# letitiabanana/PnP-OVSS

Measured on AMD Instinct MI355X. Metric: images/sec (336^2, drop_iter=4, blur+CRF), higher is better.
Workload: dtype bf16x3

## Files before the change

### include/pnp_hip.h

```cpp
#ifndef PNP_HIP_H
#define PNP_HIP_H

#include <stddef.h>
#include <stdint.h>

#ifdef __cplusplus
extern "C" {
#endif

typedef struct pnp_engine pnp_engine;

typedef struct pnp_config {
    int32_t img_size, patch, vit_dim, vit_depth, vit_heads, vit_mlp_ratio;
    float vit_ln_eps;
    int32_t txt_hidden, txt_layers, txt_heads, txt_inter;
    float txt_ln_eps;
    int32_t vocab, max_pos, enc_token_id;
    int32_t max_batch;
    int32_t max_text_len;
    int32_t stash_layer;
    int32_t compute_bf16;
    int32_t device;
} pnp_config;

int pnp_create(const pnp_config* cfg, pnp_engine** out);
int pnp_create_shared(const pnp_config* cfg, pnp_engine* donor, pnp_engine** out);
void pnp_destroy(pnp_engine* e);
const char* pnp_last_error(const pnp_engine* e);
size_t pnp_workspace_bytes(const pnp_config* cfg);
size_t pnp_allocated_bytes(const pnp_engine* e);

int pnp_load_weight(pnp_engine* e, const char* name, const float* data, const int64_t* shape, int32_t ndim,
                    int32_t on_device);
int pnp_finalize_weights(pnp_engine* e);

int pnp_vit_forward(pnp_engine* e, const float* d_images, const uint8_t* d_dropped, int32_t B, void* stream);
int pnp_cross_kv(pnp_engine* e, int32_t B, void* stream);
int pnp_text_forward_xattn(pnp_engine* e, const int64_t* d_ids, const int64_t* d_mask, int32_t ld, int32_t B,
                           int32_t L, float* d_logits, void* stream);
int pnp_xattn_grad(pnp_engine* e, int32_t B, int32_t L, void* stream);
int pnp_xattn_grad_layer(pnp_engine* e, int32_t B, int32_t L, int32_t layer, void* stream);
int pnp_gradcam_gather(pnp_engine* e, const int64_t* d_mask, int32_t ld, int32_t B, int32_t L, int32_t head,
                       float* d_out, void* stream);
int pnp_compute_gradcam(pnp_engine* e, const float* d_images, const uint8_t* d_dropped, const int64_t* d_ids,
                        const int64_t* d_mask, int32_t ld, int32_t B, int32_t L, int32_t head, float* d_out,
                        float* d_logits, void* stream);

int pnp_compute_gradcam_layer(pnp_engine* e, const float* d_images, const uint8_t* d_dropped, const int64_t* d_ids,
                              const int64_t* d_mask, int32_t ld, int32_t B, int32_t L, int32_t layer, int32_t head,
                              float* d_out, float* d_logits, void* stream);

int pnp_drop_step(pnp_engine* e, const float* d_gradcam, float* d_g0, float* d_agg, uint8_t* d_dropped,
                  int32_t* d_picks, int32_t iter, int32_t B, int32_t T, int32_t npick, int32_t max_picks,
                  void* stream);
int pnp_drop_loop(pnp_engine* e, const float* d_images, const int64_t* d_ids, const int64_t* d_mask, int32_t ld,
                  int32_t B, int32_t L, int32_t head, int32_t drop_iter, int32_t npick, float* d_g0, float* d_agg,
                  int32_t* d_picks, float* d_logits, void* stream);

int pnp_drop_loop_layer(pnp_engine* e, const float* d_images, const int64_t* d_ids, const int64_t* d_mask, int32_t ld,
                        int32_t B, int32_t L, int32_t layer, int32_t head, int32_t drop_iter, int32_t npick, float* d_g0,
                        float* d_agg, int32_t* d_picks, float* d_logits, void* stream);

typedef struct pnp_post_batch {
    int32_t B;
    const int32_t* H;
    const int32_t* W;
    const int32_t* n_classes;
    const int32_t* has_bg;
    const int32_t* img_cls_off;
    const int32_t* cls_off;
    const int32_t* tok_idx;
    const int32_t* cls_div;
    const int32_t* lut;
    int32_t lut_stride;
    const uint8_t* d_rgb;
    const float* d_gt;
    const double* blur_wts;
    const int32_t* blur_wt_off;
} pnp_post_batch;

int pnp_post_reserve(pnp_engine* e, int32_t max_batch, int64_t max_total_pixels, int32_t max_pixels_per_image,
                     int32_t max_channels, int32_t crf_chunk);
int pnp_post_prepare(pnp_engine* e, const pnp_post_batch* batch, int32_t want_crf, void* stream);
int pnp_merge_tokens(pnp_engine* e, const float* d_gradcam, int32_t T, void* stream);
int pnp_threshold_upsample(pnp_engine* e, float threshold, int32_t scale01, void* stream);
int pnp_blur_minmax(pnp_engine* e, void* stream);
int pnp_densecrf(pnp_engine* e, int32_t iters, float pos_w, float pos_xy, float bi_w, float bi_xy, float bi_rgb,
                 void* stream);
int pnp_remap_hist(pnp_engine* e, int32_t from_crf, uint8_t* d_labels, unsigned long long* d_hist, int32_t n_class,
                   void* stream);
int pnp_postprocess(pnp_engine* e, const float* d_gradcam, int32_t T, float threshold, int32_t scale01, int32_t mode,
                    uint8_t* d_labels, unsigned long long* d_hist, int32_t n_class, void* stream);

int pnp_postprocess_pair(pnp_engine* e, const float* d_gradcam_1drop, const float* d_gradcam_ndrop, int32_t T, float threshold,
                         int32_t scale01_mask, uint8_t* d_labels_1drop, unsigned long long* d_hist_1drop, uint8_t* d_labels_ndrop,
                         unsigned long long* d_hist_ndrop, int32_t n_class, void* stream);

typedef struct pnp_pre_image {
    int64_t src_off;
    int64_t tmp_off;
    int32_t H, W;
    int32_t kx_off, kx_size;
    int32_t ky_off, ky_size;
} pnp_pre_image;
int pnp_preprocess_images(const uint8_t* d_rgb, const pnp_pre_image* d_desc, int32_t B, int32_t S, int32_t max_H,
                          const int32_t* d_coef, uint8_t* d_tmp, const float* mean3, const float* std3, float* d_out,
                          void* stream);

typedef struct pnp_jpeg_image {
    int64_t data_off;
    int64_t coef_off[3];
    int64_t plane_off[3];
    int64_t rgb_off;
    int32_t data_len, H, W, ncomp, hmax, vmax, mcux, mcuy;
    int32_t h[3], v[3], tq[3], td[3], ta[3], bx[3], by[3];
    int32_t tab, pad[2];
} pnp_jpeg_image;
typedef struct pnp_jpeg_tables {
    uint8_t counts[4][16];
    uint8_t vals[4][256];
    int32_t quant[4][64];
} pnp_jpeg_tables;
typedef struct pnp_jpeg_segment {
    int64_t byte_off;
    int64_t clean_off;
    int32_t image, mcu0, nmcu;
    int32_t raw_len;
    int32_t clean_cap;
    int32_t sub_bits;
    int32_t pad[2];
} pnp_jpeg_segment;
int pnp_jpeg_decode(const uint8_t* d_data, const pnp_jpeg_image* d_images, const pnp_jpeg_tables* d_tables,
                    const pnp_jpeg_segment* d_segments, int32_t n_images, int32_t n_segments, uint8_t* d_clean, int32_t* d_seg_bits,
                    int16_t* d_coef, int64_t coef_elems, uint8_t* d_planes, uint8_t* d_rgb, int32_t max_blocks_per_image,
                    int32_t max_pixels_per_image, int32_t* d_err, void* stream);

int pnp_get_buffer(pnp_engine* e, const char* name, void** d_ptr, size_t* bytes);
int pnp_profile_enable(pnp_engine* e, int32_t on);
int pnp_profile_read(pnp_engine* e, int64_t* launches, double* flops, double* ms);
int pnp_profile_read_stage(pnp_engine* e, int32_t stage, int64_t* launches, double* work, double* ms);
int pnp_set_tuning(const char* key, int32_t value);
int pnp_streamk_status(pnp_engine* e, int64_t* launches, uint32_t* gave_up);
int pnp_op_gemm(int32_t bf16, const void* d_A, int32_t lda, const void* d_B, int32_t ldb, int32_t M, int32_t N, int32_t K,
                const float* d_bias, const float* d_resid, int32_t ldr, float* d_out_f32, int32_t ldo, int32_t gelu,
                void* stream);
int pnp_op_gemm_ex(int32_t bf16, const void* d_A, int32_t lda, const void* d_B, int32_t ldb, int32_t M, int32_t N, int32_t K,
                   const float* d_bias, const float* d_resid, int32_t ldr, float* d_out_f32, int32_t ldo, void* d_out_t,
                   int32_t ldo_t, int32_t mode, void* stream);
int pnp_op_gemm_tokcols(int32_t bf16, const void* d_A, int32_t lda, const void* d_B, int32_t ldb, int32_t M, int32_t N,
                        int32_t K, const float* d_bias_rows, void* d_out_t, int32_t ldo_t, int32_t col_div,
                        int32_t col_pad, void* stream);
int pnp_op_split(const float* d_in, void* d_hi, void* d_lo, int64_t n, void* stream);
int pnp_op_gemm_x3(const void* d_A_hi, const void* d_A_lo, int32_t lda, const void* d_B_hi, const void* d_B_lo, int32_t ldb,
                   int32_t M, int32_t N, int32_t K, const float* d_bias, int32_t bias_on_rows, const float* d_resid, int32_t ldr,
                   float* d_out_f32, int32_t ldo, void* d_out_hi, void* d_out_lo, int32_t ldo_t, int32_t gelu, int32_t col_div,
                   int32_t col_pad, void* stream);
int pnp_op_gemm_x3a(const float* d_A, int32_t lda, const void* d_B_hi, const void* d_B_lo, int32_t ldb, int32_t M, int32_t N,
                    int32_t K, const float* d_bias, const float* d_resid, int32_t ldr, float* d_out_f32, int32_t ldo, int32_t mode,
                    float* d_aux, int32_t ld_aux, void* stream);
int pnp_op_vit_attention(int32_t bf16, const void* d_qk, int32_t ld_qk, int32_t D, const void* d_vt, int32_t ld_vt,
                         int32_t n_pad, void* d_ctx, int32_t B, int32_t heads, int32_t N, float scale, void* stream);
int pnp_op_vit_attention_x3(const void* d_qkv_hi, const void* d_qkv_lo, int32_t ld_qkv, int32_t D, void* d_ctx_hi, void* d_ctx_lo,
                            int32_t B, int32_t heads, int32_t N, float scale, void* stream);
int pnp_op_layernorm(const float* d_x, const float* d_w, const float* d_b, float eps, int32_t rows, int32_t D,
                     float* d_y, void* stream);
int pnp_op_xattn(int32_t bf16, int32_t mode, const void* d_nat, int32_t ld_nat, const void* d_tr, int32_t ld_tr,
                 int32_t n_pad, const void* d_x, int32_t ldx, void* d_out, int32_t ldo, float* d_probs, int32_t n_stride,
                 int32_t B, int32_t L, int32_t N, int32_t heads, void* stream);
int pnp_dbg_gemm_stamps(uint64_t* host_out, int32_t max_blocks);
int pnp_op_cast(int32_t to_bf16, const float* d_in, void* d_out, int64_t n, void* stream);
int pnp_op_sort_pairs(uint64_t* d_keys_in, uint64_t* d_keys_out, uint32_t* d_vals_in, uint32_t* d_vals_out, int64_t n,
                      int32_t begin_bit, int32_t end_bit, const size_t* h_seg_off, int32_t n_seg, void* stream);
int pnp_op_scan_i32(const int32_t* d_in, int32_t* d_out, int64_t n, int32_t inclusive, void* stream);

#ifdef __cplusplus
}
#endif
#endif
```

### pnp-ovss_amd/csrc/engine.hip

```cpp
#include <hip/hip_runtime.h>

#include <cmath>
#include <cstdarg>
#include <cstring>
#include <map>
#include <memory>
#include <string>
#include <vector>

#include "../../include/pnp_hip.h"
#include "common.h"
#include "kernels.h"

using namespace pnp;

namespace {

struct Buf {
    void* p = nullptr;
    size_t bytes = 0;
};

struct TextLayerW {
    void *qkv_w = nullptr, *so_w = nullptr, *cq_w = nullptr, *co_w = nullptr, *i_w = nullptr, *o_w = nullptr;
    float *qkv_b = nullptr, *so_b = nullptr, *sln_w = nullptr, *sln_b = nullptr, *cq_b = nullptr, *co_b = nullptr,
          *cln_w = nullptr, *cln_b = nullptr, *i_b = nullptr, *o_b = nullptr, *oln_w = nullptr, *oln_b = nullptr;
    void *o_wT = nullptr, *i_wT = nullptr, *co_wT = nullptr, *cq_wT = nullptr, *so_wT = nullptr, *qkv_wT = nullptr;
};

struct TextLayerA {
    void* qkv = nullptr;
    float* Ps = nullptr;
    float *a_hat = nullptr, *a_rstd = nullptr, *a_out = nullptr;
    void* a_outT = nullptr;
    void* qc = nullptr;
    float* Pc = nullptr;
    float *c_hat = nullptr, *c_rstd = nullptr, *c_out = nullptr;
    void* c_outT = nullptr;
    float* u = nullptr;
    float *o_hat = nullptr, *o_rstd = nullptr, *h_out = nullptr;
    void* h_outT = nullptr;
};

struct VitLayerW {
    float *n1w, *n1b, *n2w, *n2b, *qkv_b, *proj_b, *fc1_b, *fc2_b;
    void *qkv_w, *proj_w, *fc1_w, *fc2_w;
};

struct WeightStore {
    int device = 0;
    std::vector<void*> allocs;
    size_t bytes = 0;
    ~WeightStore() {
        (void)hipSetDevice(device);
        for (void* p : allocs) (void)hipFree(p);
    }
};

}

struct pnp_engine {
    pnp_config c{};
    std::shared_ptr<WeightStore> wstore;
    bool to_store = false;
    bool shares_weights = false;
    int bf = 0;
    int x3 = 0;
    size_t esz = 4;
    int P = 0, PP = 0, N = 0, Npad = 0, D = 0, H = 0, I = 0, TL = 0, nh = 0, Nst = 0, SL = 0;
    char err[512] = {0};
    std::vector<void*> allocs;
    size_t alloc_bytes = 0;
    std::map<std::string, Buf> named;
    std::map<std::string, bool> loaded;
    bool finalized = false;

    float *cls = nullptr, *pos = nullptr, *patch_b = nullptr, *vnorm_w = nullptr, *vnorm_b = nullptr;
    void* patch_w = nullptr;
    std::vector<VitLayerW> vit;
    float *word = nullptr, *tpos = nullptr, *eln_w = nullptr, *eln_b = nullptr, *itm_w = nullptr, *itm_b = nullptr;
    std::vector<TextLayerW> txt;
    void *ck_w = nullptr, *cv_w = nullptr;
    float *ck_b = nullptr, *cv_b = nullptr;
    std::vector<Buf> staging;

    int ldq = 0;
    float* x0 = nullptr;
    struct { const float* images = nullptr; const int64_t* ids = nullptr; const int64_t* mask = nullptr; int B = 0, L = 0, ld = 0;
             bool vit = false, text = false; } reuse;
    void *patches = nullptr, *xn = nullptr, *qk = nullptr, *vt = nullptr, *ctx = nullptr, *h1 = nullptr, *embT = nullptr;
    float *x = nullptr, *emb32 = nullptr;
    void *Knat = nullptr, *Vnat = nullptr, *Kt = nullptr, *Vt = nullptr;
    std::vector<TextLayerA> ta;
    float *temb = nullptr, *h0 = nullptr, *tmp = nullptr;
    void *h0T = nullptr, *ctx_s = nullptr, *ctx_c = nullptr, *g = nullptr;
    float *dh = nullptr, *d_pre = nullptr, *dc = nullptr, *d_cpre = nullptr, *da = nullptr, *d_apre = nullptr,
          *dctx_s = nullptr, *dS = nullptr, *dPc = nullptr;
    void *d_preT = nullptr, *dg = nullptr, *d_cpreT = nullptr, *dctxc = nullptr, *dqc = nullptr, *d_apreT = nullptr,
         *dqkv = nullptr;
    int grad_layer = -1;
    float* G = nullptr;
    uint8_t* dropped = nullptr;
    float* logits_scratch = nullptr;

    struct Post {
        bool reserved = false, prepared = false, has_crf = false;
        int groups_cap = 1;
        int maxB = 0, maxK = 0, max_pix_img = 0, chunk = 0;
        int64_t max_total_pix = 0;
        int B = 0, Cmax = 0, Kmax = 0, maxHW = 0;
        int64_t total_pix = 0;
        std::vector<PostDesc> desc, desc_pair;
        PostDesc* d_desc = nullptr;
        PostDesc* d_desc_pair = nullptr;
        int32_t *d_img_cls_off = nullptr, *d_cls_off = nullptr, *d_tok_idx = nullptr, *d_cls_div = nullptr, *d_lut = nullptr;
        int lut_stride = 0;
        size_t* d_label_off = nullptr;
        double* d_wts = nullptr;
        int32_t* d_wt_off = nullptr;
        float *merged = nullptr, *thr = nullptr, *maps = nullptr, *maps2 = nullptr, *maps3 = nullptr, *stats = nullptr;
        float *unary = nullptr, *Q = nullptr, *va = nullptr, *vb = nullptr, *vga = nullptr, *vgb = nullptr, *norm[2] = {nullptr, nullptr};
        int Kpmax = 0, Kpmax_pair = 0, maxH = 0, maxW = 0, max_radius = 0, maxKp = 0;
        size_t valg_cap = 0;
        std::vector<int> gauss_sig;
        const uint8_t* d_rgb = nullptr;
        const float* d_gt = nullptr;
        CrfLattice lat[2]{};
        uint64_t *keys_a = nullptr, *keys_b = nullptr;
        uint32_t* vals_a = nullptr;
        int *n1k = nullptr, *n2k = nullptr;
        int *head = nullptr, *incl = nullptr, *range_err = nullptr;
        int range_err_host = 0;
        int lat_points[2] = {0, 0};
        std::vector<size_t> h_label_off;
        std::vector<int32_t> h_wt_off;
        std::vector<double> h_wts;
        void* sort_tmp = nullptr;
        size_t sort_tmp_bytes = 0;
        size_t cap[2] = {0, 0};
        size_t val_cap = 0;
        int lut_cap = 0, cls_cap = 0, tok_cap = 0, wts_cap = 0;
        bool maps_in_2 = false;
    } post;

    GemmProfile* gemm_prof = nullptr;
    StreamKWs sk_ws;
    struct StageProfile {
        bool on = false;
        std::vector<hipEvent_t> ev0, ev1;
        int used = 0;
        long long launches = 0;
        double work = 0;
        double lattice = 0;
    } crf_prof;
};

namespace {

int fail(pnp_engine* e, int code, const char* fmt, ...) {
// ... 6 lines not shown

#define HIPCHK(e, call)                                                                      \
    do {                                                                                     \
        hipError_t _s = (call);                                                              \
        if (_s != hipSuccess) return fail(e, PNP_ERR_HIP, "%s: %s", #call, hipGetErrorString(_s)); \
    } while (0)
#define KCHK(e, call)                                                         \
    do {                                                                      \
        int _r = (call);                                                      \
        if (_r != PNP_OK) return fail(e, _r, "%s failed (%d): %s", #call, _r, hipGetErrorString(hipGetLastError())); \
    } while (0)

template <typename T>
int dalloc(pnp_engine* e, T** out, size_t count, bool zero = false) {
    void* p = nullptr;
    const size_t bytes = (count * sizeof(T) + 255) / 256 * 256;
    if (hipMalloc(&p, bytes ? bytes : 256) != hipSuccess) return fail(e, PNP_ERR_NOMEM, "hipMalloc(%zu) failed", bytes);
    if (zero && hipMemset(p, 0, bytes ? bytes : 256) != hipSuccess) return fail(e, PNP_ERR_HIP, "hipMemset failed");
    if (e->to_store && e->wstore) {
        e->wstore->allocs.push_back(p);
        e->wstore->bytes += bytes;
    } else {
        e->allocs.push_back(p);
    }
    e->alloc_bytes += bytes;
    *out = reinterpret_cast<T*>(p);
    return PNP_OK;
}
int dalloc_t(pnp_engine* e, void** out, size_t count, bool zero = false) {
    char* p = nullptr;
    int r = dalloc<char>(e, &p, count * e->esz, zero);
    *out = p;
    return r;
}

bool ends_with(const std::string& s, const char* suf) {
    const size_t n = strlen(suf);
    return s.size() >= n && s.compare(s.size() - n, n, suf) == 0;
}

__global__ void transpose_cast_kernel_f32(const float* __restrict__ in, float* __restrict__ out, int rows, int cols) {
    __shared__ float t[32][33];
    const int bx = blockIdx.x * 32, by = blockIdx.y * 32;
    for (int i = threadIdx.y; i < 32; i += 8) {
        const int r = by + i, c = bx + threadIdx.x;
        t[i][threadIdx.x] = (r < rows && c < cols) ? in[(size_t)r * cols + c] : 0.f;
    }
    __syncthreads();
    for (int i = threadIdx.y; i < 32; i += 8) {
        const int c = bx + i, r = by + threadIdx.x;
        if (r < rows && c < cols) out[(size_t)c * rows + r] = t[threadIdx.x][i];
    }
}

__global__ void feat_to_tok_kernel(const float* __restrict__ src, int ld_src, int n_pad, float* __restrict__ dst, int R, int N) {
    __shared__ float t[32][33];
    const int b = blockIdx.z, r0 = blockIdx.x * 32, t0 = blockIdx.y * 32;
    for (int i = threadIdx.y; i < 32; i += 8) {
        const int r = r0 + i, tok = t0 + threadIdx.x;
        t[i][threadIdx.x] = (r < R && tok < N) ? src[(size_t)r * ld_src + (size_t)b * n_pad + tok] : 0.f;
    }
    __syncthreads();
    for (int i = threadIdx.y; i < 32; i += 8) {
        const int tok = t0 + i, r = r0 + threadIdx.x;
        if (r < R && tok < N) dst[((size_t)b * N + tok) * R + r] = t[threadIdx.x][i];
    }
}
__global__ void tok_to_feat_kernel(const float* __restrict__ src, int ld_src, float* __restrict__ dst, int ld_dst, int n_pad, int R, int N) {
    __shared__ float t[32][33];
    const int b = blockIdx.z, r0 = blockIdx.x * 32, t0 = blockIdx.y * 32;
    for (int i = threadIdx.y; i < 32; i += 8) {
        const int tok = t0 + i, r = r0 + threadIdx.x;
        t[i][threadIdx.x] = (r < R && tok < N) ? src[((size_t)b * N + tok) * ld_src + r] : 0.f;
    }
    __syncthreads();
    for (int i = threadIdx.y; i < 32; i += 8) {
        const int r = r0 + i, tok = t0 + threadIdx.x;
        if (r < R && tok < N) dst[(size_t)r * ld_dst + (size_t)b * n_pad + tok] = t[threadIdx.x][i];
    }
}

__global__ void embed_reuse_kernel(const float* __restrict__ x0, const uint8_t* __restrict__ dropped, const float* __restrict__ bias,
                                   const float* __restrict__ pos, float* __restrict__ x, int rows, int N, int D4) {
    const size_t total = (size_t)rows * D4;
    for (size_t i = (size_t)blockIdx.x * blockDim.x + threadIdx.x; i < total; i += (size_t)gridDim.x * blockDim.x) {
        const int m = (int)(i / D4), c = (int)(i - (size_t)m * D4);
        const int b = m / N, t = m - b * N;
        f32x4 v;
        if (t > 0 && dropped[(size_t)b * (N - 1) + (t - 1)]) {
            const f32x4 bv = reinterpret_cast<const f32x4*>(bias)[c];
            const f32x4 pv = reinterpret_cast<const f32x4*>(pos)[(size_t)t * D4 + c];
#pragma unroll
            for (int e = 0; e < 4; e++) v[e] = __fadd_rn(__fadd_rn(0.0f, bv[e]), pv[e]);
        } else {
            v = reinterpret_cast<const f32x4*>(x0)[i];
        }
        reinterpret_cast<f32x4*>(x)[i] = v;
    }
}

int make_weight(pnp_engine* e, const float* src32, int rows, int cols, bool transpose, void** out, bool split = false) {
    KCHK(e, dalloc_t(e, out, (size_t)rows * cols));
    const float* s = src32;
    float* tmp = nullptr;
    if (transpose) {
        HIPCHK(e, hipMalloc((void**)&tmp, (size_t)rows * cols * 4));
        hipLaunchKernelGGL(transpose_cast_kernel_f32, dim3((cols + 31) / 32, (rows + 31) / 32), dim3(32, 8), 0, 0, src32, tmp,
                           rows, cols);
        s = tmp;
    }
    int r = split ? split_f32(s, *out, (char*)*out + (size_t)rows * cols * 2, (size_t)rows * cols, 0)
                  : cast_f32(e->bf, s, *out, (size_t)rows * cols, 0);
    hipError_t st = hipDeviceSynchronize();
    if (tmp) (void)hipFree(tmp);
    if (r != PNP_OK || st != hipSuccess) return fail(e, PNP_ERR_HIP, "weight conversion failed");
    return PNP_OK;
}

GemmArgs G_(const void* A, int lda, const void* B, int ldb, int M, int N, int K) {
    GemmArgs g;
    g.A = A; g.lda = lda; g.B = B; g.ldb = ldb; g.M = M; g.N = N; g.K = K;
    return g;
}

int egemm(pnp_engine* e, int bf, GemmArgs g, hipStream_t s) {
    g.prof = e->gemm_prof;
    g.sk = e->sk_ws.part ? &e->sk_ws : nullptr;
    return gemm_nt(bf, g, s);
}

int tgemm(pnp_engine* e, GemmArgs g, hipStream_t s) {
    if (e->x3) {
        g.a_f32 = 1;
        g.B_lo = (const char*)g.B + (size_t)g.N * g.K * 2;
    }
    return egemm(e, e->bf, g, s);
}

const char* kVitNames[] = {"norm1.weight", "norm1.bias", "attn.qkv.weight", "attn.qkv.bias", "attn.proj.weight",
                           "attn.proj.bias", "norm2.weight", "norm2.bias", "mlp.fc1.weight", "mlp.fc1.bias",
                           "mlp.fc2.weight", "mlp.fc2.bias"};

}


extern "C" size_t pnp_workspace_bytes(const pnp_config* c) {
    if (!c) return 0;
    const size_t es = c->compute_bf16 == 1 ? 2 : 4;
    const size_t P = c->img_size / c->patch, N = P * P + 1, Npad = (N + 63) / 64 * 64, D = c->vit_dim, H = c->txt_hidden,
                 I = c->txt_inter, TL = c->txt_layers, B = c->max_batch, L = c->max_text_len;
    const size_t M = B * N, R = B * L;
    size_t w = (size_t)c->vit_depth * (12 * D * D) * es + TL * (4 * H * H + 2 * H * D + 2 * H * I) * es * 2 +
               ((size_t)c->vocab + c->max_pos) * H * 4;
    size_t a = M * (768 + D * 2 + 3 * D + 64 + D + 4 * D) * es + M * D * 12 + D * B * Npad * es + M * TL * H * es * 2 +
               2 * TL * H * B * Npad * es;
    size_t t = TL * (R * (3 * H + 2 * H) * es + R * (H * 8 + I) * 4 + B * (H / 64) * L * (L + Npad) * 4) + R * I * (4 + es) * 2 +
               R * H * 64;
    return w + a + t + (64u << 20);
}

extern "C" const char* pnp_last_error(const pnp_engine* e) { return e ? e->err : "null engine"; }

extern "C" void pnp_destroy(pnp_engine* e) {
    if (!e) return;
    (void)hipSetDevice(e->c.device);
    (void)hipDeviceSynchronize();
    for (void* p : e->allocs) (void)hipFree(p);
    for (auto& b : e->staging) if (b.p) (void)hipFree(b.p);
    if (e->gemm_prof) {
        for (int i = 0; i < e->gemm_prof->created; i++) {
            (void)hipEventDestroy(e->gemm_prof->ev0[i]);
            (void)hipEventDestroy(e->gemm_prof->ev1[i]);
        }
        delete e->gemm_prof;
    }
    for (hipEvent_t ev : e->crf_prof.ev0) (void)hipEventDestroy(ev);
    for (hipEvent_t ev : e->crf_prof.ev1) (void)hipEventDestroy(ev);
    streamk_ws_destroy(&e->sk_ws);
    delete e;
}

static int create_impl(const pnp_config* cfg, pnp_engine* donor, pnp_engine** out);
extern "C" int pnp_create(const pnp_config* cfg, pnp_engine** out) { return create_impl(cfg, nullptr, out); }
extern "C" int pnp_create_shared(const pnp_config* cfg, pnp_engine* donor, pnp_engine** out) {
    if (!donor) return PNP_ERR_ARG;
    return create_impl(cfg, donor, out);
}
static int create_impl(const pnp_config* cfg, pnp_engine* donor, pnp_engine** out) {
    if (!cfg || !out) return PNP_ERR_ARG;
    pnp_engine* e = new pnp_engine();
    *out = e;
    e->c = *cfg;
    if (donor) {
        const pnp_config& d = donor->c;
        if (!donor->finalized) return fail(e, PNP_ERR_STATE, "pnp_create_shared: the donor's weights are not finalized");
        if (d.device != cfg->device || d.compute_bf16 != cfg->compute_bf16 || d.img_size != cfg->img_size || d.patch != cfg->patch ||
            d.vit_dim != cfg->vit_dim || d.vit_depth != cfg->vit_depth || d.vit_heads != cfg->vit_heads ||
            d.vit_mlp_ratio != cfg->vit_mlp_ratio || d.txt_hidden != cfg->txt_hidden || d.txt_layers != cfg->txt_layers ||
            d.txt_heads != cfg->txt_heads || d.txt_inter != cfg->txt_inter || d.vocab != cfg->vocab || d.max_pos != cfg->max_pos ||
            d.vit_ln_eps != cfg->vit_ln_eps || d.txt_ln_eps != cfg->txt_ln_eps)
            return fail(e, PNP_ERR_ARG, "pnp_create_shared: device, compute mode and model geometry must equal the donor's");
        if (cfg->stash_layer < d.stash_layer)
            return fail(e, PNP_ERR_ARG, "pnp_create_shared: stash_layer %d below the donor's %d (its transposed backward weights "
                        "exist for layers >= %d only)", cfg->stash_layer, d.stash_layer, d.stash_layer);
    }
    const pnp_config& c = e->c;
    if (c.compute_bf16 < 0 || c.compute_bf16 > 2) return fail(e, PNP_ERR_ARG, "compute_bf16 must be 0 (fp32), 1 (bf16) or 2 (split-bf16)");
    e->bf = c.compute_bf16 == 1 ? 1 : 0;
    e->x3 = c.compute_bf16 == 2 ? 1 : 0;
    e->esz = e->bf ? 2 : 4;
    if (c.patch != 16) return fail(e, PNP_ERR_ARG, "patch must be 16");
    if (c.img_size % 16 || c.img_size <= 0) return fail(e, PNP_ERR_ARG, "img_size must be a positive multiple of 16");
    if (c.vit_dim != c.vit_heads * 64 || c.txt_hidden != c.txt_heads * 64)
        return fail(e, PNP_ERR_ARG, "head_dim must be 64 (vit_dim=%d heads=%d, txt_hidden=%d heads=%d)", c.vit_dim,
                    c.vit_heads, c.txt_hidden, c.txt_heads);
    if (c.vit_dim % 128 || c.txt_hidden % 128 || c.txt_inter % 128 || (c.vit_dim * c.vit_mlp_ratio) % 128)
        return fail(e, PNP_ERR_ARG, "widths must be multiples of 128");
    if (c.vit_dim > 1024 || c.txt_hidden > 1024) return fail(e, PNP_ERR_ARG, "LayerNorm width > 1024 unsupported");
    if (c.max_text_len < 5 || c.max_text_len > 512 || c.max_text_len > c.max_pos)
        return fail(e, PNP_ERR_ARG, "max_text_len must be in [5, min(512, max_pos = %d)]", c.max_pos);
    if (c.stash_layer < 0 || c.stash_layer >= c.txt_layers) return fail(e, PNP_ERR_ARG, "stash_layer out of range");
    if (c.max_batch <= 0) return fail(e, PNP_ERR_ARG, "max_batch must be positive");
    HIPCHK(e, hipSetDevice(c.device));
    e->P = c.img_size / 16;
    e->PP = e->P * e->P;
    e->N = e->PP + 1;
    e->Npad = (e->N + 63) / 64 * 64;
    e->Nst = e->Npad;
    e->D = c.vit_dim;
    e->H = c.txt_hidden;
    e->I = c.txt_inter;
    e->TL = c.txt_layers;
    e->nh = c.txt_heads;
    e->SL = c.stash_layer;
    if ((e->N + 15) / 16 > 160) return fail(e, PNP_ERR_ARG, "too many image tokens (%d) for the cross-attention kernel", e->N);
    const size_t B = c.max_batch, M = B * e->N, D = e->D, H = e->H, I = e->I, L = c.max_text_len, R = B * L, TL = e->TL;
    const size_t ldv = B * e->Npad;
    e->vit.resize(c.vit_depth);
    e->txt.resize(TL);
    e->ta.resize(TL);
    if (e->x3) {
        const int n_cu = device_cu_count();
        if (!n_cu || streamk_ws_create(&e->sk_ws, n_cu) != PNP_OK) return fail(e, PNP_ERR_HIP, "stream-K workspace allocation failed");
        e->alloc_bytes += (size_t)n_cu * 256 * 256 * 4;
    }
    KCHK(e, dalloc_t(e, &e->patches, B * e->PP * 768));
    KCHK(e, dalloc(e, &e->x, M * D));
    KCHK(e, dalloc(e, &e->x0, M * D));
    KCHK(e, dalloc_t(e, &e->xn, M * D));
    e->ldq = 3 * (int)D + 64;
    KCHK(e, dalloc_t(e, &e->qk, M * (size_t)e->ldq));
    KCHK(e, dalloc_t(e, &e->vt, D * ldv, true));
    KCHK(e, dalloc_t(e, &e->ctx, M * D));
    KCHK(e, dalloc_t(e, &e->h1, M * D * c.vit_mlp_ratio));
    KCHK(e, dalloc_t(e, &e->embT, M * D));
    KCHK(e, dalloc(e, &e->emb32, M * D));
    const int nVn = e->TL - e->SL, nKt = e->TL - e->SL - 1;
    KCHK(e, dalloc_t(e, &e->Knat, M * TL * H));
    KCHK(e, dalloc_t(e, &e->Vnat, M * (size_t)nVn * H));
    KCHK(e, dalloc_t(e, &e->Vt, TL * H * ldv, true));
    if (nKt > 0) KCHK(e, dalloc_t(e, &e->Kt, (size_t)nKt * H * ldv, true));
    KCHK(e, dalloc(e, &e->temb, R * H));
    KCHK(e, dalloc(e, &e->h0, R * H));
    KCHK(e, dalloc_t(e, &e->h0T, R * H));
    KCHK(e, dalloc(e, &e->tmp, R * H));
    KCHK(e, dalloc_t(e, &e->ctx_s, R * H));
    KCHK(e, dalloc_t(e, &e->ctx_c, R * H));
    KCHK(e, dalloc_t(e, &e->g, R * I));
    for (size_t i = 0; i < TL; i++) {
        TextLayerA& a = e->ta[i];
        KCHK(e, dalloc_t(e, &a.qkv, R * 3 * H));
        KCHK(e, dalloc(e, &a.a_hat, R * H));
        KCHK(e, dalloc(e, &a.a_rstd, R));
        KCHK(e, dalloc(e, &a.a_out, R * H));
        KCHK(e, dalloc_t(e, &a.a_outT, R * H));
        KCHK(e, dalloc_t(e, &a.qc, R * H));
        KCHK(e, dalloc(e, &a.c_hat, R * H));
        KCHK(e, dalloc(e, &a.c_rstd, R));
        KCHK(e, dalloc(e, &a.c_out, R * H));
        KCHK(e, dalloc_t(e, &a.c_outT, R * H));
        KCHK(e, dalloc(e, &a.u, R * I));
        KCHK(e, dalloc(e, &a.o_hat, R * H));
        KCHK(e, dalloc(e, &a.o_rstd, R));
        KCHK(e, dalloc(e, &a.h_out, R * H));
        KCHK(e, dalloc_t(e, &a.h_outT, R * H));
        if ((int)i >= e->SL) {
            KCHK(e, dalloc(e, &a.Ps, B * e->nh * L * L));
            KCHK(e, dalloc(e, &a.Pc, B * e->nh * L * (size_t)e->Nst, true));
        }
    }
    KCHK(e, dalloc(e, &e->dh, R * H));
    KCHK(e, dalloc(e, &e->d_pre, R * H));
    KCHK(e, dalloc_t(e, &e->d_preT, R * H));
    KCHK(e, dalloc_t(e, &e->dg, R * I));
    KCHK(e, dalloc(e, &e->dc, R * H));
    KCHK(e, dalloc(e, &e->d_cpre, R * H));
    KCHK(e, dalloc_t(e, &e->d_cpreT, R * H));
    KCHK(e, dalloc_t(e, &e->dctxc, R * H));
    KCHK(e, dalloc_t(e, &e->dqc, R * H));
    KCHK(e, dalloc(e, &e->da, R * H));
    KCHK(e, dalloc(e, &e->d_apre, R * H));
    KCHK(e, dalloc_t(e, &e->d_apreT, R * H));
    KCHK(e, dalloc(e, &e->dctx_s, R * H));
    KCHK(e, dalloc(e, &e->dS, B * e->nh * L * L));
    KCHK(e, dalloc(e, &e->dPc, B * e->nh * L * (size_t)e->Nst, true));
    KCHK(e, dalloc_t(e, &e->dqkv, R * 3 * H));
    KCHK(e, dalloc(e, &e->G, B * L * (size_t)e->PP));
    KCHK(e, dalloc(e, &e->dropped, B * (size_t)e->PP, true));
    KCHK(e, dalloc(e, &e->logits_scratch, B * 2));
    if (donor) {
        e->wstore = donor->wstore;
        e->shares_weights = true;
        e->cls = donor->cls; e->pos = donor->pos; e->patch_b = donor->patch_b; e->vnorm_w = donor->vnorm_w; e->vnorm_b = donor->vnorm_b;
        e->word = donor->word; e->tpos = donor->tpos; e->eln_w = donor->eln_w; e->eln_b = donor->eln_b;
        e->itm_w = donor->itm_w; e->itm_b = donor->itm_b; e->ck_b = donor->ck_b; e->cv_b = donor->cv_b;
        e->patch_w = donor->patch_w; e->ck_w = donor->ck_w; e->cv_w = donor->cv_w;
        e->vit = donor->vit;
        e->txt = donor->txt;
        e->finalized = true;
        return PNP_OK;
    }
    e->wstore = std::make_shared<WeightStore>();
    e->wstore->device = c.device;
    e->to_store = true;
    KCHK(e, dalloc(e, &e->cls, D));
    KCHK(e, dalloc(e, &e->pos, (size_t)e->N * D));
    KCHK(e, dalloc(e, &e->patch_b, D));
    KCHK(e, dalloc(e, &e->vnorm_w, D));
    KCHK(e, dalloc(e, &e->vnorm_b, D));
    KCHK(e, dalloc(e, &e->word, (size_t)c.vocab * H));
    KCHK(e, dalloc(e, &e->tpos, (size_t)c.max_pos * H));
    KCHK(e, dalloc(e, &e->eln_w, H));
    KCHK(e, dalloc(e, &e->eln_b, H));
    KCHK(e, dalloc(e, &e->itm_w, 2 * H));
    KCHK(e, dalloc(e, &e->itm_b, 2));
    KCHK(e, dalloc(e, &e->ck_b, TL * H));
    KCHK(e, dalloc(e, &e->cv_b, TL * H));
    for (auto& v : e->vit) {
        KCHK(e, dalloc(e, &v.n1w, D)); KCHK(e, dalloc(e, &v.n1b, D)); KCHK(e, dalloc(e, &v.n2w, D)); KCHK(e, dalloc(e, &v.n2b, D));
        KCHK(e, dalloc(e, &v.qkv_b, 3 * D)); KCHK(e, dalloc(e, &v.proj_b, D));
        KCHK(e, dalloc(e, &v.fc1_b, D * c.vit_mlp_ratio)); KCHK(e, dalloc(e, &v.fc2_b, D));
        v.qkv_w = v.proj_w = v.fc1_w = v.fc2_w = nullptr;
    }
    for (auto& t : e->txt) {
        KCHK(e, dalloc(e, &t.qkv_b, 3 * H)); KCHK(e, dalloc(e, &t.so_b, H)); KCHK(e, dalloc(e, &t.sln_w, H)); KCHK(e, dalloc(e, &t.sln_b, H));
        KCHK(e, dalloc(e, &t.cq_b, H)); KCHK(e, dalloc(e, &t.co_b, H)); KCHK(e, dalloc(e, &t.cln_w, H)); KCHK(e, dalloc(e, &t.cln_b, H));
        KCHK(e, dalloc(e, &t.i_b, I)); KCHK(e, dalloc(e, &t.o_b, H)); KCHK(e, dalloc(e, &t.oln_w, H)); KCHK(e, dalloc(e, &t.oln_b, H));
    }
    e->to_store = false;
    return PNP_OK;
}


namespace {

struct Slot {
    float* small = nullptr;
    size_t small_off = 0;
    bool gemm = false;
    int rows = 0, cols = 0;
};

bool resolve(pnp_engine* e, const std::string& n, Slot& s) {
    const int D = e->D, H = e->H, I = e->I;
    auto small = [&](float* p, int count, size_t off = 0) { s.small = p; s.small_off = off; s.rows = 1; s.cols = count; return true; };
    auto gemm = [&](int r, int c) { s.gemm = true; s.rows = r; s.cols = c; return true; };
    if (n == "visual_encoder.cls_token") return small(e->cls, D);
    if (n == "visual_encoder.pos_embed") return small(e->pos, e->N * D);
    if (n == "visual_encoder.patch_embed.proj.weight") return gemm(D, 768);
    if (n == "visual_encoder.patch_embed.proj.bias") return small(e->patch_b, D);
    if (n == "visual_encoder.norm.weight") return small(e->vnorm_w, D);
    if (n == "visual_encoder.norm.bias") return small(e->vnorm_b, D);
    if (n == "text_encoder.embeddings.word_embeddings.weight") return small(e->word, e->c.vocab * H);
    if (n == "text_encoder.embeddings.position_embeddings.weight") return small(e->tpos, e->c.max_pos * H);
    if (n == "text_encoder.embeddings.LayerNorm.weight") return small(e->eln_w, H);
    if (n == "text_encoder.embeddings.LayerNorm.bias") return small(e->eln_b, H);
    if (n == "itm_head.weight") return small(e->itm_w, 2 * H);
    if (n == "itm_head.bias") return small(e->itm_b, 2);
    int li = -1;
    char rest[128];
    if (sscanf(n.c_str(), "visual_encoder.blocks.%d.%127s", &li, rest) == 2 && li >= 0 && li < e->c.vit_depth) {
        VitLayerW& v = e->vit[li];
        const std::string r(rest);
        const int F = D * e->c.vit_mlp_ratio;
        if (r == "norm1.weight") return small(v.n1w, D);
        if (r == "norm1.bias") return small(v.n1b, D);
        if (r == "norm2.weight") return small(v.n2w, D);
        if (r == "norm2.bias") return small(v.n2b, D);
        if (r == "attn.qkv.bias") return small(v.qkv_b, 3 * D);
        if (r == "attn.proj.bias") return small(v.proj_b, D);
        if (r == "mlp.fc1.bias") return small(v.fc1_b, F);
        if (r == "mlp.fc2.bias") return small(v.fc2_b, D);
        if (r == "attn.qkv.weight") return gemm(3 * D, D);
        if (r == "attn.proj.weight") return gemm(D, D);
        if (r == "mlp.fc1.weight") return gemm(F, D);
        if (r == "mlp.fc2.weight") return gemm(D, F);
        return false;
    }
    if (sscanf(n.c_str(), "text_encoder.encoder.layer.%d.%127s", &li, rest) == 2 && li >= 0 && li < e->TL) {
        TextLayerW& t = e->txt[li];
        const std::string r(rest);
        if (r == "attention.self.query.bias") return small(t.qkv_b, H, 0);
        if (r == "attention.self.key.bias") return small(t.qkv_b, H, H);
        if (r == "attention.self.value.bias") return small(t.qkv_b, H, 2 * H);
        if (r == "attention.output.dense.bias") return small(t.so_b, H);
// ... 47 lines not shown
    }
    e->loaded[name] = true;
    return PNP_OK;
}

extern "C" int pnp_finalize_weights(pnp_engine* e) {
    if (!e) return PNP_ERR_ARG;
    if (e->finalized) return PNP_OK;
    HIPCHK(e, hipSetDevice(e->c.device));
    e->to_store = true;
    struct StoreOff { pnp_engine* e; ~StoreOff() { e->to_store = false; } } store_off{e};
    const int D = e->D, H = e->H, I = e->I, TL = e->TL;
    auto stage = [&](const std::string& n) -> const float* {
        auto it = e->named.find("stage:" + n);
        return it == e->named.end() ? nullptr : (const float*)it->second.p;
    };
#define NEED(ptr, nm)                                                         \
    const float* ptr = stage(nm);                                             \
    if (!ptr) return fail(e, PNP_ERR_STATE, "missing weight %s", std::string(nm).c_str());
    {
        const char* smalls[] = {"visual_encoder.cls_token", "visual_encoder.pos_embed", "visual_encoder.patch_embed.proj.bias",
                                "visual_encoder.norm.weight", "visual_encoder.norm.bias",
                                "text_encoder.embeddings.word_embeddings.weight", "text_encoder.embeddings.position_embeddings.weight",
                                "text_encoder.embeddings.LayerNorm.weight", "text_encoder.embeddings.LayerNorm.bias",
                                "itm_head.weight", "itm_head.bias"};
        for (const char* s : smalls)
            if (!e->loaded.count(s)) return fail(e, PNP_ERR_STATE, "missing weight %s", s);
    }
    {
        NEED(pw, "visual_encoder.patch_embed.proj.weight");
        KCHK(e, make_weight(e, pw, D, 768, false, &e->patch_w));
    }
    const int F = D * e->c.vit_mlp_ratio;
    for (int i = 0; i < e->c.vit_depth; i++) {
        const std::string b = "visual_encoder.blocks." + std::to_string(i) + ".";
        for (const char* k : kVitNames)
            if (!e->loaded.count(b + k)) return fail(e, PNP_ERR_STATE, "missing weight %s%s", b.c_str(), k);
        NEED(w0, b + "attn.qkv.weight");
        NEED(w1, b + "attn.proj.weight");
        NEED(w2, b + "mlp.fc1.weight");
        NEED(w3, b + "mlp.fc2.weight");
        KCHK(e, make_weight(e, w0, 3 * D, D, false, &e->vit[i].qkv_w, e->x3));
        KCHK(e, make_weight(e, w1, D, D, false, &e->vit[i].proj_w, e->x3));
        KCHK(e, make_weight(e, w2, F, D, false, &e->vit[i].fc1_w, e->x3));
        KCHK(e, make_weight(e, w3, D, F, false, &e->vit[i].fc2_w, e->x3));
    }
    KCHK(e, dalloc_t(e, &e->ck_w, (size_t)TL * H * D));
    KCHK(e, dalloc_t(e, &e->cv_w, (size_t)TL * H * D));
    for (int i = 0; i < TL; i++) {
        const std::string b = "text_encoder.encoder.layer." + std::to_string(i) + ".";
        TextLayerW& t = e->txt[i];
        const char* req[] = {"attention.self.query.bias", "attention.self.key.bias", "attention.self.value.bias",
                             "attention.output.dense.bias", "attention.output.LayerNorm.weight", "attention.output.LayerNorm.bias",
                             "crossattention.self.query.bias", "crossattention.self.key.bias", "crossattention.self.value.bias",
                             "crossattention.output.dense.bias", "crossattention.output.LayerNorm.weight",
                             "crossattention.output.LayerNorm.bias", "intermediate.dense.bias", "output.dense.bias",
                             "output.LayerNorm.weight", "output.LayerNorm.bias"};
        for (const char* k : req)
            if (!e->loaded.count(b + k)) return fail(e, PNP_ERR_STATE, "missing weight %s%s", b.c_str(), k);
        NEED(wq, b + "attention.self.query.weight");
        NEED(wk, b + "attention.self.key.weight");
        NEED(wv, b + "attention.self.value.weight");
        NEED(wso, b + "attention.output.dense.weight");
        NEED(wcq, b + "crossattention.self.query.weight");
        NEED(wck, b + "crossattention.self.key.weight");
        NEED(wcv, b + "crossattention.self.value.weight");
        NEED(wco, b + "crossattention.output.dense.weight");
        NEED(wi, b + "intermediate.dense.weight");
        NEED(wo, b + "output.dense.weight");
        float* fused = nullptr;
        HIPCHK(e, hipMalloc((void**)&fused, (size_t)3 * H * H * 4));
        HIPCHK(e, hipMemcpy(fused, wq, (size_t)H * H * 4, hipMemcpyDeviceToDevice));
        HIPCHK(e, hipMemcpy(fused + (size_t)H * H, wk, (size_t)H * H * 4, hipMemcpyDeviceToDevice));
        HIPCHK(e, hipMemcpy(fused + (size_t)2 * H * H, wv, (size_t)H * H * 4, hipMemcpyDeviceToDevice));
        int r = make_weight(e, fused, 3 * H, H, false, &t.qkv_w, e->x3);
        if (r == PNP_OK && i > e->SL) r = make_weight(e, fused, 3 * H, H, true, &t.qkv_wT, e->x3);
        (void)hipFree(fused);
        if (r != PNP_OK) return r;
        KCHK(e, make_weight(e, wso, H, H, false, &t.so_w, e->x3));
        KCHK(e, make_weight(e, wcq, H, H, false, &t.cq_w, e->x3));
        KCHK(e, make_weight(e, wco, H, H, false, &t.co_w, e->x3));
        KCHK(e, make_weight(e, wi, I, H, false, &t.i_w, e->x3));
        KCHK(e, make_weight(e, wo, H, I, false, &t.o_w, e->x3));
        if (e->x3) {
            const size_t half = (size_t)TL * H * D * 2, off = (size_t)i * H * D * 2;
            KCHK(e, split_f32(wck, (char*)e->ck_w + off, (char*)e->ck_w + half + off, (size_t)H * D, 0));
            KCHK(e, split_f32(wcv, (char*)e->cv_w + off, (char*)e->cv_w + half + off, (size_t)H * D, 0));
        } else {
            KCHK(e, cast_f32(e->bf, wck, (char*)e->ck_w + (size_t)i * H * D * e->esz, (size_t)H * D, 0));
            KCHK(e, cast_f32(e->bf, wcv, (char*)e->cv_w + (size_t)i * H * D * e->esz, (size_t)H * D, 0));
        }
        if (i >= e->SL) {
            KCHK(e, make_weight(e, wo, H, I, true, &t.o_wT, e->x3));
            KCHK(e, make_weight(e, wi, I, H, true, &t.i_wT, e->x3));
            KCHK(e, make_weight(e, wco, H, H, true, &t.co_wT, e->x3));
        }
        if (i > e->SL) {
            KCHK(e, make_weight(e, wcq, H, H, true, &t.cq_wT, e->x3));
            KCHK(e, make_weight(e, wso, H, H, true, &t.so_wT, e->x3));
        }
    }
#undef NEED
    HIPCHK(e, hipDeviceSynchronize());
    for (auto& b : e->staging) if (b.p) (void)hipFree(b.p);
    e->staging.clear();
    for (auto it = e->named.begin(); it != e->named.end();) {
        if (it->first.rfind("stage:", 0) == 0) it = e->named.erase(it);
        else ++it;
    }
    e->finalized = true;
    return PNP_OK;
}


static int vit_forward_impl(pnp_engine* e, const float* d_images, const uint8_t* d_dropped, int32_t B, void* stream, int embed);
extern "C" int pnp_vit_forward(pnp_engine* e, const float* d_images, const uint8_t* d_dropped, int32_t B, void* stream) {
    if (e) e->reuse.vit = false;
    return vit_forward_impl(e, d_images, d_dropped, B, stream, 0);
}
static int vit_forward_impl(pnp_engine* e, const float* d_images, const uint8_t* d_dropped, int32_t B, void* stream, int embed) {
    if (!e || !d_images) return PNP_ERR_ARG;
    if (!e->finalized) return fail(e, PNP_ERR_STATE, "weights not finalized");
    if (B <= 0 || B > e->c.max_batch) return fail(e, PNP_ERR_ARG, "batch %d out of range (max %d)", B, e->c.max_batch);
    hipStream_t s = (hipStream_t)stream;
    const int D = e->D, N = e->N, M = B * N, F = D * e->c.vit_mlp_ratio, bf = e->bf;
    const int ldv = e->c.max_batch * e->Npad;
    if (embed == 2 && !(e->reuse.vit && e->reuse.images == d_images && e->reuse.B == B)) embed = 0;
    if (embed == 2 && d_dropped) {
        hipLaunchKernelGGL(embed_reuse_kernel, dim3(2048), dim3(256), 0, s, (const float*)e->x0, d_dropped, (const float*)e->patch_b,
                           (const float*)e->pos, e->x, M, N, D / 4);
        if (hipGetLastError() != hipSuccess) return fail(e, PNP_ERR_HIP, "embed_reuse launch");
    } else {
    KCHK(e, patchify(bf, d_images, d_dropped, e->patches, B, e->c.img_size, e->P, s));
    KCHK(e, cls_rows(e->cls, e->pos, e->x, B, N, D, s));
    {
        GemmArgs g = G_(e->patches, 768, e->patch_w, 768, B * e->PP, D, 768);
        g.bias = e->patch_b; g.resid = e->pos; g.ldr = D; g.out_f32 = e->x; g.ldo = D; g.row_div = e->PP;
        KCHK(e, egemm(e, bf, g, s));
    }
    if (embed == 1) {
        HIPCHK(e, hipMemcpyAsync(e->x0, e->x, (size_t)M * D * sizeof(float), hipMemcpyDeviceToDevice, s));
        e->reuse.images = d_images;
        e->reuse.B = B;
        e->reuse.vit = true;
    }
    }
    const float scale = 1.0f / sqrtf(64.f);
    if (e->x3) {
        const size_t cap = (size_t)e->c.max_batch * N;
        void* const xn_lo = (char*)e->xn + cap * D * 2;
        void* const ctx_lo = (char*)e->ctx + cap * D * 2;
        void* const h1_lo = (char*)e->h1 + cap * F * 2;
        void* const qk_lo = (char*)e->qk + cap * e->ldq * 2;
        for (int l = 0; l < e->c.vit_depth; l++) {
            const VitLayerW& w = e->vit[l];
            const char* const qkv_lo = (const char*)w.qkv_w + (size_t)3 * D * D * 2;
            KCHK(e, layernorm(1, e->x, w.n1w, w.n1b, e->c.vit_ln_eps, M, D, nullptr, e->xn, nullptr, nullptr, s, xn_lo));
            {
                GemmArgs g = G_(e->xn, D, w.qkv_w, D, M, 3 * D, D);
                g.A_lo = xn_lo; g.B_lo = qkv_lo;
                g.bias = w.qkv_b; g.out_t = e->qk; g.out_lo = qk_lo; g.ldo_t = e->ldq;
                KCHK(e, egemm(e, 1, g, s));
            }
            KCHK(e, vit_attention_x3(e->qk, qk_lo, e->ldq, D, e->ctx, ctx_lo, B, e->c.vit_heads, N, scale, s));
            {
                GemmArgs g = G_(e->ctx, D, w.proj_w, D, M, D, D);
                g.A_lo = ctx_lo; g.B_lo = (const char*)w.proj_w + (size_t)D * D * 2;
                g.bias = w.proj_b; g.resid = e->x; g.ldr = D; g.out_f32 = e->x; g.ldo = D;
                KCHK(e, egemm(e, 1, g, s));
            }
            KCHK(e, layernorm(1, e->x, w.n2w, w.n2b, e->c.vit_ln_eps, M, D, nullptr, e->xn, nullptr, nullptr, s, xn_lo));
            {
                GemmArgs g = G_(e->xn, D, w.fc1_w, D, M, F, D);
                g.A_lo = xn_lo; g.B_lo = (const char*)w.fc1_w + (size_t)F * D * 2;
                g.bias = w.fc1_b; g.mode = GEMM_EPI_GELU; g.out_t = e->h1; g.out_lo = h1_lo; g.ldo_t = F;
                KCHK(e, egemm(e, 1, g, s));
            }
            {
                GemmArgs g = G_(e->h1, F, w.fc2_w, F, M, D, F);
                g.A_lo = h1_lo; g.B_lo = (const char*)w.fc2_w + (size_t)D * F * 2;
                g.bias = w.fc2_b; g.resid = e->x; g.ldr = D; g.out_f32 = e->x; g.ldo = D;
                KCHK(e, egemm(e, 1, g, s));
            }
        }
        KCHK(e, layernorm(1, e->x, e->vnorm_w, e->vnorm_b, e->c.vit_ln_eps, M, D, e->emb32, e->embT, nullptr, nullptr, s,
                          (char*)e->embT + cap * D * 2));
        return pnp_cross_kv(e, B, stream);
    }
    for (int l = 0; l < e->c.vit_depth; l++) {
        const VitLayerW& w = e->vit[l];
        KCHK(e, layernorm(bf, e->x, w.n1w, w.n1b, e->c.vit_ln_eps, M, D, nullptr, e->xn, nullptr, nullptr, s));
        if (bf) {
            GemmArgs g = G_(e->xn, D, w.qkv_w, D, M, 3 * D, D);
            g.bias = w.qkv_b; g.out_t = e->qk; g.ldo_t = e->ldq;
            KCHK(e, egemm(e, bf, g, s));
            KCHK(e, vit_attention(bf, e->qk, e->ldq, D, (const char*)e->qk + (size_t)2 * D * e->esz, e->ldq, e->Npad, e->ctx, B,
                                  e->c.vit_heads, N, scale, s));
        } else {
        {
            GemmArgs g = G_(e->xn, D, w.qkv_w, D, M, 2 * D, D);
            g.bias = w.qkv_b; g.out_t = e->qk; g.ldo_t = 2 * D;
            KCHK(e, egemm(e, bf, g, s));
        }
        {
            GemmArgs g = G_((const char*)w.qkv_w + (size_t)2 * D * D * e->esz, D, e->xn, D, D, M, D);
            g.bias = w.qkv_b + 2 * D; g.bias_on_rows = 1; g.out_t = e->vt; g.ldo_t = ldv; g.col_div = N; g.col_pad = e->Npad;
            KCHK(e, egemm(e, bf, g, s));
        }
        KCHK(e, vit_attention(bf, e->qk, 2 * D, D, e->vt, ldv, e->Npad, e->ctx, B, e->c.vit_heads, N, scale, s));
        }
        {
            GemmArgs g = G_(e->ctx, D, w.proj_w, D, M, D, D);
            g.bias = w.proj_b; g.resid = e->x; g.ldr = D; g.out_f32 = e->x; g.ldo = D;
            KCHK(e, egemm(e, bf, g, s));
        }
        KCHK(e, layernorm(bf, e->x, w.n2w, w.n2b, e->c.vit_ln_eps, M, D, nullptr, e->xn, nullptr, nullptr, s));
        {
            GemmArgs g = G_(e->xn, D, w.fc1_w, D, M, F, D);
            g.bias = w.fc1_b; g.mode = GEMM_EPI_GELU; g.out_t = e->h1; g.ldo_t = F;
            KCHK(e, egemm(e, bf, g, s));
        }
        {
            GemmArgs g = G_(e->h1, F, w.fc2_w, F, M, D, F);
            g.bias = w.fc2_b; g.resid = e->x; g.ldr = D; g.out_f32 = e->x; g.ldo = D;
            KCHK(e, egemm(e, bf, g, s));
        }
    }
    KCHK(e, layernorm(bf, e->x, e->vnorm_w, e->vnorm_b, e->c.vit_ln_eps, M, D, e->emb32, e->embT, nullptr, nullptr, s));
    return pnp_cross_kv(e, B, stream);
}

extern "C" int pnp_cross_kv(pnp_engine* e, int32_t B, void* stream) {
    if (!e) return PNP_ERR_ARG;
    if (!e->finalized) return fail(e, PNP_ERR_STATE, "weights not finalized");
    if (B <= 0 || B > e->c.max_batch) return fail(e, PNP_ERR_ARG, "batch %d out of range (max %d)", B, e->c.max_batch);
    hipStream_t s = (hipStream_t)stream;
    const int D = e->D, N = e->N, M = B * N, bf = e->bf;
    const int ldv = e->c.max_batch * e->Npad;
    const int H = e->H, TL = e->TL, SL = e->SL;
    if (e->x3) {
        const size_t cap = (size_t)e->c.max_batch * N, whalf = (size_t)TL * H * D * 2;
        const void* const emb_lo = (const char*)e->embT + cap * D * 2;
        const char *ck = (const char*)e->ck_w, *cv = (const char*)e->cv_w;
        {
            GemmArgs g = G_(e->embT, D, ck, D, M, TL * H, D);
            g.A_lo = emb_lo; g.B_lo = ck + whalf;
            g.bias = e->ck_b; g.out_f32 = (float*)e->Knat; g.ldo = TL * H;
            KCHK(e, egemm(e, 1, g, s));
        }
        {
            GemmArgs g = G_(cv, D, e->embT, D, TL * H, M, D);
            g.A_lo = cv + whalf; g.B_lo = emb_lo;
            g.bias = e->cv_b; g.bias_on_rows = 1; g.out_f32 = (float*)e->Vt; g.ldo = ldv; g.col_div = N; g.col_pad = e->Npad;
            KCHK(e, egemm(e, 1, g, s));
        }
        {
            const int nVn = TL - SL, R = nVn * H;
            hipLaunchKernelGGL(feat_to_tok_kernel, dim3((R + 31) / 32, (N + 31) / 32, B), dim3(32, 8), 0, s,
                               (const float*)e->Vt + (size_t)SL * H * ldv, ldv, e->Npad, (float*)e->Vnat, R, N);
            const int nKt = TL - SL - 1;
            if (nKt > 0)
                hipLaunchKernelGGL(tok_to_feat_kernel, dim3((nKt * H + 31) / 32, (N + 31) / 32, B), dim3(32, 8), 0, s,
                                   (const float*)e->Knat + (size_t)(SL + 1) * H, TL * H, (float*)e->Kt, ldv, e->Npad, nKt * H, N);
            if (hipGetLastError() != hipSuccess) return fail(e, PNP_ERR_HIP, "cross K / V layout kernels failed to launch");
        }
        return PNP_OK;
    }
    {
        GemmArgs g = G_(e->embT, D, e->ck_w, D, M, TL * H, D);
        g.bias = e->ck_b; g.out_t = e->Knat; g.ldo_t = TL * H;
        KCHK(e, egemm(e, bf, g, s));
    }
    {
        GemmArgs g = G_(e->cv_w, D, e->embT, D, TL * H, M, D);
        g.bias = e->cv_b; g.bias_on_rows = 1; g.out_t = e->Vt; g.ldo_t = ldv; g.col_div = N; g.col_pad = e->Npad;
        KCHK(e, egemm(e, bf, g, s));
    }
    {
        const int nVn = TL - SL;
        GemmArgs g = G_(e->embT, D, (const char*)e->cv_w + (size_t)SL * H * D * e->esz, D, M, nVn * H, D);
        g.bias = e->cv_b + (size_t)SL * H; g.out_t = e->Vnat; g.ldo_t = nVn * H;
        KCHK(e, egemm(e, bf, g, s));
    }
    if (TL - SL - 1 > 0) {
        const int nKt = TL - SL - 1;
        GemmArgs g = G_((const char*)e->ck_w + (size_t)(SL + 1) * H * D * e->esz, D, e->embT, D, nKt * H, M, D);
        g.bias = e->ck_b + (size_t)(SL + 1) * H; g.bias_on_rows = 1; g.out_t = e->Kt; g.ldo_t = ldv; g.col_div = N; g.col_pad = e->Npad;
        KCHK(e, egemm(e, bf, g, s));
    }
    return PNP_OK;
}

static int text_forward_impl(pnp_engine* e, const int64_t* d_ids, const int64_t* d_mask, int32_t ld, int32_t B, int32_t L,
                             float* d_logits, void* stream, bool reuse_prefix);
extern "C" int pnp_text_forward_xattn(pnp_engine* e, const int64_t* d_ids, const int64_t* d_mask, int32_t ld, int32_t B,
                                      int32_t L, float* d_logits, void* stream) {
    if (e) e->reuse.text = false;
    return text_forward_impl(e, d_ids, d_mask, ld, B, L, d_logits, stream, false);
}
static int text_forward_impl(pnp_engine* e, const int64_t* d_ids, const int64_t* d_mask, int32_t ld, int32_t B, int32_t L,
                             float* d_logits, void* stream, bool reuse_prefix) {
    if (!e || !d_ids || !d_mask) return PNP_ERR_ARG;
    if (!e->finalized) return fail(e, PNP_ERR_STATE, "weights not finalized");
    if (B <= 0 || B > e->c.max_batch || L < 5 || L > e->c.max_text_len || ld < L)
        return fail(e, PNP_ERR_ARG, "text batch %d x %d (ld %d) out of range (max %d x %d)", B, L, ld, e->c.max_batch, e->c.max_text_len);
    hipStream_t s = (hipStream_t)stream;
    const int H = e->H, I = e->I, TL = e->TL, R = B * L, bf = e->bf, N = e->N, D = e->D;
    const int ldv = e->c.max_batch * e->Npad;
    (void)D;
    if (reuse_prefix && !(e->reuse.text && e->reuse.ids == d_ids && e->reuse.mask == d_mask && e->reuse.B == B && e->reuse.L == L &&
                          e->reuse.ld == ld))
        reuse_prefix = false;
    if (!reuse_prefix) {
        KCHK(e, text_embed(d_ids, ld, e->word, e->tpos, e->temb, B, L, H, e->c.enc_token_id, e->c.vocab, s));
        KCHK(e, layernorm(bf, e->temb, e->eln_w, e->eln_b, e->c.txt_ln_eps, R, H, e->h0, e->h0T, nullptr, nullptr, s));
    }
    const float* h = e->h0;
// ... 579 lines not shown
    lout.lut = p.d_lut;
    lout.lut_stride = p.lut_stride;
    lout.label_off = p.d_label_off;
    int r = crf_iterate(e, p.d_desc_pair, p.Kpmax_pair, 10, 7.0f, 10.0f, s, lout);
    if (r) return r;
    for (int grp = 0; grp < 2; grp++) {
        uint8_t* lab = grp == 0 ? d_labels_1drop : d_labels_ndrop;
        unsigned long long* hist = grp == 0 ? d_hist_1drop : d_hist_ndrop;
        if (hist && p.d_gt) KCHK(e, confusion_hist(lab, p.d_gt, p.d_desc, p.d_label_off, hist, n_class, p.B, p.maxHW, s));
    }
    return PNP_OK;
}


extern "C" int pnp_get_buffer(pnp_engine* e, const char* name, void** d_ptr, size_t* bytes) {
    if (!e || !name || !d_ptr || !bytes) return PNP_ERR_ARG;
    const std::string n(name);
    const size_t B = e->c.max_batch, L = e->c.max_text_len;
    auto& p = e->post;
    auto set = [&](void* ptr, size_t b) { *d_ptr = ptr; *bytes = b; return PNP_OK; };
    if (n == "image_embeds") return set(e->emb32, B * e->N * (size_t)e->D * 4);
    if (n == "image_embeds_t") return set(e->embT, B * e->N * (size_t)e->D * e->esz);
    if (n == "x") return set(e->x, B * e->N * (size_t)e->D * 4);
    if (n == "P") return set(e->ta[e->grad_layer >= 0 ? e->grad_layer : e->SL].Pc, B * e->nh * L * (size_t)e->Nst * 4);
    if (n == "dP") return set(e->dPc, B * e->nh * L * (size_t)e->Nst * 4);
    if (n == "h_last") return set(e->ta[e->TL - 1].h_out, B * L * (size_t)e->H * 4);
    if (n == "dropped") return set(e->dropped, B * (size_t)e->PP);
    if (n == "P_last" && e->ta[e->TL - 1].Pc) return set(e->ta[e->TL - 1].Pc, B * e->nh * L * (size_t)e->Nst * 4);
    if (n == "Kt" && e->Kt) return set(e->Kt, (size_t)(e->TL - e->SL - 1) * e->H * B * e->Npad * e->esz);
    if (n == "Vt") return set(e->Vt, (size_t)e->TL * e->H * B * e->Npad * e->esz);
    if (n == "dq_xattn") return set(e->dqc, B * L * (size_t)e->H * e->esz);
    if (n == "dctx_xattn") return set(e->dctxc, B * L * (size_t)e->H * e->esz);
    if (p.reserved) {
        const size_t mk = (size_t)p.max_total_pix * p.maxK * 4;
        const size_t mq = (size_t)p.max_total_pix * p.maxKp * 4;
        if (n == "merged") return set(p.merged, (size_t)p.maxB * p.maxK * e->PP * 4);
        if (n == "maps") return set(p.maps_in_2 ? p.maps2 : p.maps, mk);
        if (n == "maps_pre_blur") return set(p.maps, mk);
        if (n == "unary") return set(p.unary, mq);
        if (n == "crf_q") return set(p.Q, mq);
        if (n == "crf_idbase_gauss") return set(p.lat[0].idbase, ((size_t)p.maxB + 1) * 4);
        if (n == "crf_idbase_bilateral") return set(p.lat[1].idbase, ((size_t)p.maxB + 1) * 4);
        if (n == "crf_norm_gauss") return set(p.norm[0], (size_t)p.max_total_pix * 4);
        if (n == "crf_norm_bilateral") return set(p.norm[1], (size_t)p.max_total_pix * 4);
        if (n == "crf_offset_gauss") return set(p.lat[0].offset, (size_t)p.max_total_pix * 3 * 4);
        if (n == "crf_offset_bilateral") return set(p.lat[1].offset, (size_t)p.max_total_pix * 6 * 4);
        if (n == "crf_nbr8_gauss") return set(p.lat[0].nbr8, (size_t)(p.lat[0].D1 / 2) * p.lat[0].cap * sizeof(CrfNbr8));
        if (n == "crf_nbr8_bilateral") return set(p.lat[1].nbr8, (size_t)(p.lat[1].D1 / 2) * p.lat[1].cap * sizeof(CrfNbr8));
    }
    return fail(e, PNP_ERR_ARG, "unknown buffer %s", name);
}

extern "C" size_t pnp_allocated_bytes(const pnp_engine* e) { return e ? e->alloc_bytes : 0; }

extern "C" int pnp_profile_enable(pnp_engine* e, int32_t on) {
    if (!e) return PNP_ERR_ARG;
    if (!e->gemm_prof) {
        if (!on) {
            e->crf_prof.on = false;
            return PNP_OK;
        }
        e->gemm_prof = new GemmProfile();
    }
    GemmProfile& pf = *e->gemm_prof;
    pf.on = on != 0;
    pf.period = on > 1 ? on : 1;
    pf.seq = 0;
    pf.used = 0;
    pf.launches = 0;
    pf.flops = 0;
    e->crf_prof.on = on != 0;
    e->crf_prof.used = 0;
    e->crf_prof.launches = 0;
    e->crf_prof.work = 0;
    e->crf_prof.lattice = 0;
    return PNP_OK;
}

extern "C" int pnp_profile_read_stage(pnp_engine* e, int32_t stage, int64_t* launches, double* work, double* ms) {
    if (!e || !launches || !work || !ms) return PNP_ERR_ARG;
    if (stage == 0) return pnp_profile_read(e, launches, work, ms);
    if (stage != 1 && stage != 2) return fail(e, PNP_ERR_ARG, "unknown profile stage %d", stage);
    auto& pf = e->crf_prof;
    double total = 0;
    for (int i = 0; i < pf.used; i++) {
        HIPCHK(e, hipEventSynchronize(pf.ev1[i]));
        float t = 0;
        HIPCHK(e, hipEventElapsedTime(&t, pf.ev0[i], pf.ev1[i]));
        total += t;
    }
    *launches = pf.launches;
    *work = stage == 1 ? pf.work : pf.lattice;
    *ms = total;
    return PNP_OK;
}

extern "C" int pnp_profile_read(pnp_engine* e, int64_t* launches, double* flops, double* ms) {
    if (!e || !launches || !flops || !ms) return PNP_ERR_ARG;
    if (!e->gemm_prof) {
        *launches = 0; *flops = 0; *ms = 0;
        return PNP_OK;
    }
    GemmProfile& pf = *e->gemm_prof;
    double total = 0;
    for (int i = 0; i < pf.used; i++) {
        HIPCHK(e, hipEventSynchronize(pf.ev1[i]));
        float t = 0;
        HIPCHK(e, hipEventElapsedTime(&t, pf.ev0[i], pf.ev1[i]));
        total += t;
    }
    *launches = pf.launches;
    *flops = pf.flops;
    *ms = total;
    return PNP_OK;
}

extern "C" int pnp_op_gemm(int32_t bf, const void* d_A, int32_t lda, const void* d_B, int32_t ldb, int32_t M, int32_t N,
                           int32_t K, const float* d_bias, const float* d_resid, int32_t ldr, float* d_out_f32, int32_t ldo,
                           int32_t gelu, void* stream) {
    GemmArgs g = G_(d_A, lda, d_B, ldb, M, N, K);
    g.bias = d_bias; g.resid = d_resid; g.ldr = ldr; g.out_f32 = d_out_f32; g.ldo = ldo;
    g.mode = gelu ? GEMM_EPI_GELU : GEMM_EPI_LINEAR;
    return gemm_nt(bf, g, (hipStream_t)stream);
}

extern "C" int pnp_op_gemm_ex(int32_t bf, const void* d_A, int32_t lda, const void* d_B, int32_t ldb, int32_t M, int32_t N,
                              int32_t K, const float* d_bias, const float* d_resid, int32_t ldr, float* d_out_f32, int32_t ldo,
                              void* d_out_t, int32_t ldo_t, int32_t mode, void* stream) {
    GemmArgs g = G_(d_A, lda, d_B, ldb, M, N, K);
    g.bias = d_bias; g.resid = d_resid; g.ldr = ldr; g.out_f32 = d_out_f32; g.ldo = ldo; g.out_t = d_out_t; g.ldo_t = ldo_t;
    g.mode = mode ? GEMM_EPI_GELU : GEMM_EPI_LINEAR;
    return gemm_nt(bf, g, (hipStream_t)stream);
}

extern "C" int pnp_op_split(const float* d_in, void* d_hi, void* d_lo, int64_t n, void* stream) {
    if (!d_in || !d_hi || !d_lo || n <= 0) return PNP_ERR_ARG;
    return split_f32(d_in, d_hi, d_lo, (size_t)n, (hipStream_t)stream);
}

extern "C" int pnp_op_gemm_x3(const void* d_A_hi, const void* d_A_lo, int32_t lda, const void* d_B_hi, const void* d_B_lo,
                              int32_t ldb, int32_t M, int32_t N, int32_t K, const float* d_bias, int32_t bias_on_rows,
                              const float* d_resid, int32_t ldr, float* d_out_f32, int32_t ldo, void* d_out_hi, void* d_out_lo,
                              int32_t ldo_t, int32_t gelu, int32_t col_div, int32_t col_pad, void* stream) {
    if (!d_A_hi || !d_A_lo || !d_B_hi || !d_B_lo) return PNP_ERR_ARG;
    GemmArgs g = G_(d_A_hi, lda, d_B_hi, ldb, M, N, K);
    g.A_lo = d_A_lo; g.B_lo = d_B_lo;
    g.bias = d_bias; g.bias_on_rows = bias_on_rows; g.resid = d_resid; g.ldr = ldr; g.out_f32 = d_out_f32; g.ldo = ldo;
    g.out_t = d_out_hi; g.out_lo = d_out_lo; g.ldo_t = ldo_t; g.col_div = col_div; g.col_pad = col_pad;
    g.mode = gelu ? GEMM_EPI_GELU : GEMM_EPI_LINEAR;
    g.sk = streamk_mode() ? streamk_ws_default() : nullptr;
    return gemm_nt(1, g, (hipStream_t)stream);
}

extern "C" int pnp_set_tuning(const char* key, int32_t value) {
    if (!key) return PNP_ERR_ARG;
    if (!strcmp(key, "streamk")) {
        if (value < 0 || value > 2) return PNP_ERR_ARG;
        set_streamk_mode(value);
        return PNP_OK;
    }
    return PNP_ERR_ARG;
}

extern "C" int pnp_streamk_status(pnp_engine* e, int64_t* launches, uint32_t* gave_up) {
    if (!launches || !gave_up) return PNP_ERR_ARG;
    StreamKWs* ws = e ? &e->sk_ws : streamk_ws_default();
    *launches = ws ? ws->launches : 0;
    *gave_up = 0;
    if (!ws || !ws->part) return PNP_OK;
    if (e) HIPCHK(e, hipSetDevice(e->c.device));
    if (hipDeviceSynchronize() != hipSuccess) return PNP_ERR_HIP;
    return streamk_ws_timeouts(ws, gave_up);
}

extern "C" int pnp_op_gemm_x3a(const float* d_A, int32_t lda, const void* d_B_hi, const void* d_B_lo, int32_t ldb, int32_t M,
                               int32_t N, int32_t K, const float* d_bias, const float* d_resid, int32_t ldr, float* d_out_f32,
                               int32_t ldo, int32_t mode, float* d_aux, int32_t ld_aux, void* stream) {
    if (!d_A || !d_B_hi || !d_B_lo || !d_out_f32 || mode < 0 || mode > 2) return PNP_ERR_ARG;
    GemmArgs g = G_(d_A, lda, d_B_hi, ldb, M, N, K);
    g.B_lo = d_B_lo; g.a_f32 = 1;
    g.bias = d_bias; g.resid = d_resid; g.ldr = ldr; g.out_f32 = d_out_f32; g.ldo = ldo;
    g.mode = mode; g.aux = d_aux; g.ld_aux = ld_aux;
    return gemm_nt(0, g, (hipStream_t)stream);
}

extern "C" int pnp_op_gemm_tokcols(int32_t bf, const void* d_A, int32_t lda, const void* d_B, int32_t ldb, int32_t M, int32_t N,
                                   int32_t K, const float* d_bias_rows, void* d_out_t, int32_t ldo_t, int32_t col_div,
                                   int32_t col_pad, void* stream) {
    if (!d_out_t || col_div < 0 || (col_div > 0 && col_pad < col_div)) return PNP_ERR_ARG;
    GemmArgs g = G_(d_A, lda, d_B, ldb, M, N, K);
    g.bias = d_bias_rows; g.bias_on_rows = 1; g.out_t = d_out_t; g.ldo_t = ldo_t; g.col_div = col_div; g.col_pad = col_pad;
    return gemm_nt(bf, g, (hipStream_t)stream);
}

extern "C" int pnp_op_vit_attention(int32_t bf, const void* d_qk, int32_t ld_qk, int32_t D, const void* d_vt, int32_t ld_vt,
                                    int32_t n_pad, void* d_ctx, int32_t B, int32_t heads, int32_t N, float scale, void* stream) {
    if (!d_qk || !d_vt || !d_ctx || B <= 0 || heads <= 0 || N <= 0) return PNP_ERR_ARG;
    return vit_attention(bf, d_qk, ld_qk, D, d_vt, ld_vt, n_pad, d_ctx, B, heads, N, scale, (hipStream_t)stream);
}

extern "C" int pnp_op_vit_attention_x3(const void* d_qkv_hi, const void* d_qkv_lo, int32_t ld_qkv, int32_t D, void* d_ctx_hi,
                                       void* d_ctx_lo, int32_t B, int32_t heads, int32_t N, float scale, void* stream) {
    if (B <= 0 || heads <= 0 || N <= 0 || ld_qkv < 3 * D) return PNP_ERR_ARG;
    return vit_attention_x3(d_qkv_hi, d_qkv_lo, ld_qkv, D, d_ctx_hi, d_ctx_lo, B, heads, N, scale, (hipStream_t)stream);
}

extern "C" int pnp_op_layernorm(const float* d_x, const float* d_w, const float* d_b, float eps, int32_t rows, int32_t D,
                                float* d_y, void* stream) {
    return layernorm(0, d_x, d_w, d_b, eps, rows, D, d_y, nullptr, nullptr, nullptr, (hipStream_t)stream);
}

extern "C" int pnp_op_xattn(int32_t bf16, int32_t mode, const void* d_nat, int32_t ld_nat, const void* d_tr, int32_t ld_tr,
                            int32_t n_pad, const void* d_x, int32_t ldx, void* d_out, int32_t ldo, float* d_probs,
                            int32_t n_stride, int32_t B, int32_t L, int32_t N, int32_t heads, void* stream) {
    if (!d_nat || !d_x || !d_probs || mode < 0 || mode > 2 || (mode != 2 && (!d_tr || !d_out))) return PNP_ERR_ARG;
    if (B <= 0 || L <= 0 || N <= 0 || heads <= 0) return PNP_ERR_ARG;
    return xattn(bf16, mode, d_nat, ld_nat, d_tr, ld_tr, n_pad, d_x, ldx, d_out, ldo, d_probs, n_stride, B, L, N, heads,
                 (hipStream_t)stream);
}

extern "C" int pnp_dbg_gemm_stamps(uint64_t* host_out, int32_t max_blocks) {
    return gemm_read_stamps((unsigned long long*)host_out, max_blocks);
}

extern "C" int pnp_preprocess_images(const uint8_t* d_rgb, const pnp_pre_image* d_desc, int32_t B, int32_t S, int32_t max_H,
                                     const int32_t* d_coef, uint8_t* d_tmp, const float* mean3, const float* std3,
                                     float* d_out, void* stream) {
    if (!d_rgb || !d_desc || !d_coef || !d_tmp || !mean3 || !std3 || !d_out) return PNP_ERR_ARG;
    static_assert(sizeof(pnp_pre_image) == 40, "pnp_pre_image layout is part of the ABI");
    return preprocess_images(d_rgb, d_desc, B, S, max_H, d_coef, d_tmp, mean3, std3, d_out, (hipStream_t)stream);
}

extern "C" int pnp_jpeg_decode(const uint8_t* d_data, const pnp_jpeg_image* d_images, const pnp_jpeg_tables* d_tables,
                               const pnp_jpeg_segment* d_segments, int32_t n_images, int32_t n_segments, uint8_t* d_clean,
                               int32_t* d_seg_bits, int16_t* d_coef, int64_t coef_elems, uint8_t* d_planes, uint8_t* d_rgb,
                               int32_t max_blocks_per_image, int32_t max_pixels_per_image, int32_t* d_err, void* stream) {
    if (!d_data || !d_images || !d_tables || !d_segments || !d_clean || !d_seg_bits || !d_coef || !d_planes || !d_rgb || !d_err ||
        coef_elems <= 0)
        return PNP_ERR_ARG;
    static_assert(sizeof(pnp_jpeg_image) == sizeof(JpegImage) && sizeof(pnp_jpeg_tables) == sizeof(JpegTables) &&
                      sizeof(pnp_jpeg_segment) == sizeof(JpegSegment), "JPEG descriptor layouts are part of the ABI");
    return jpeg_decode(d_data, reinterpret_cast<const JpegImage*>(d_images), reinterpret_cast<const JpegTables*>(d_tables),
                       reinterpret_cast<const JpegSegment*>(d_segments), n_images, n_segments, d_clean, d_seg_bits, d_coef,
                       (size_t)coef_elems, d_planes, d_rgb, max_blocks_per_image, max_pixels_per_image, d_err, (hipStream_t)stream);
}

extern "C" int pnp_op_sort_pairs(uint64_t* d_keys_in, uint64_t* d_keys_out, uint32_t* d_vals_in, uint32_t* d_vals_out, int64_t n,
                                 int32_t begin_bit, int32_t end_bit, const size_t* h_seg_off, int32_t n_seg, void* stream) {
    if (n < 0 || (n && (!d_keys_in || !d_keys_out || !d_vals_in || !d_vals_out))) return PNP_ERR_ARG;
    if (!n) return PNP_OK;
    const size_t tb = sort_temp_bytes((size_t)n);
    void* temp = nullptr;
    if (hipMalloc(&temp, tb) != hipSuccess) return PNP_ERR_NOMEM;
    int r = radix_sort_pairs(d_keys_in, d_keys_out, d_vals_in, d_vals_out, (size_t)n, begin_bit, end_bit, h_seg_off, n_seg, temp, tb, (hipStream_t)stream);
    if (hipStreamSynchronize((hipStream_t)stream) != hipSuccess && r == PNP_OK) r = PNP_ERR_HIP;
    (void)hipFree(temp);
    return r;
}
extern "C" int pnp_op_scan_i32(const int32_t* d_in, int32_t* d_out, int64_t n, int32_t inclusive, void* stream) {
    if (n < 0 || (n && (!d_in || !d_out))) return PNP_ERR_ARG;
    if (!n) return PNP_OK;
    const size_t tb = sort_temp_bytes((size_t)n);
    void* temp = nullptr;
    if (hipMalloc(&temp, tb) != hipSuccess) return PNP_ERR_NOMEM;
    int r = device_scan_i32(d_in, d_out, (size_t)n, inclusive != 0, temp, tb, (hipStream_t)stream);
    if (hipStreamSynchronize((hipStream_t)stream) != hipSuccess && r == PNP_OK) r = PNP_ERR_HIP;
    (void)hipFree(temp);
    return r;
}

extern "C" int pnp_op_cast(int32_t to_bf16, const float* d_in, void* d_out, int64_t n, void* stream) {
    return cast_f32(to_bf16, d_in, d_out, (size_t)n, (hipStream_t)stream);
}
```

### pnp-ovss_amd/csrc/gemm.h

```cpp
#pragma once
#include <hip/hip_runtime.h>

namespace pnp {

enum { GEMM_EPI_LINEAR = 0, GEMM_EPI_GELU = 1, GEMM_EPI_GELU_GRAD = 2 };

struct GemmProfile;

struct StreamKWs {
    float* part = nullptr;
    unsigned* flag = nullptr;
    int wgs = 0;
    long long launches = 0;
};
int streamk_ws_create(StreamKWs* ws, int wgs);
void streamk_ws_destroy(StreamKWs* ws);
int streamk_ws_timeouts(StreamKWs* ws, unsigned* out);
StreamKWs* streamk_ws_default();
void set_streamk_mode(int mode);
int streamk_mode();

struct GemmArgs {
    const void* A = nullptr;
    const void* B = nullptr;
    int M = 0, N = 0, K = 0, lda = 0, ldb = 0;
    int Nvalid = 0;
    int mode = GEMM_EPI_LINEAR;
    const float* bias = nullptr;
    int bias_on_rows = 0;
    const float* resid = nullptr;
    int ldr = 0;
    float* out_f32 = nullptr;
    int ldo = 0;
    void* out_t = nullptr;
    int ldo_t = 0;
    float* aux = nullptr;
    int ld_aux = 0;
    const void* A_lo = nullptr;
    const void* B_lo = nullptr;
    void* out_lo = nullptr;
    int a_f32 = 0;
    int row_div = 0;
    int col_div = 0, col_pad = 0;
    struct GemmProfile* prof = nullptr;
    StreamKWs* sk = nullptr;
    float* sk_part = nullptr;
    unsigned* sk_flag = nullptr;
    unsigned* sk_tmo = nullptr;
    int sk_full = 0, sk_upw = 0;
    unsigned long long* stamps = nullptr;
    int ablate = 0;
};

int gemm_nt(int dtype_bf16, GemmArgs g, hipStream_t s);

struct GemmProfile {
    bool on = false;
    static constexpr int kMax = 8192;
    hipEvent_t ev0[kMax], ev1[kMax];
    int created = 0, used = 0;
    int period = 1;
    long long seq = 0;
    long long launches = 0;
    double flops = 0;
};
int gemm_read_stamps(unsigned long long* host_out, int max_blocks);

}
```

### pnp-ovss_amd/csrc/gemm.hip

```cpp
#include <stdlib.h>

#include <type_traits>

#include "common.h"
#include "gemm.h"
#include "gemm_wide.h"

namespace pnp {

struct RowCtx {
    int orow;
    const float* resid_row;
    float bias_row;
};

__device__ __forceinline__ RowCtx row_ctx(const GemmArgs& g, int m) {
    RowCtx rc;
    rc.orow = m;
    rc.resid_row = nullptr;
    if (g.row_div > 0) {
        const int b = m / g.row_div, p = m - b * g.row_div;
        rc.orow = b * (g.row_div + 1) + 1 + p;
        if (g.resid) rc.resid_row = g.resid + (size_t)(1 + p) * g.ldr;
    } else if (g.resid) {
// ... 471 lines not shown
                if (g.bias && m < g.M) brow[j] = g.bias[m];
            }
        }
        const int next = tile + gridDim.x;
        if (next < ntiles) {
            set_tile(next, m0, n0);
#pragma unroll
            for (int i = 0; i < NDMA; i++) issue_one(0, i);
        }

        if constexpr (EPI == WIDE_TOKCOLS_BF16) {
            constexpr int HROW = 68;
            bf16* const stgh = reinterpret_cast<bf16*>(smem + 65536) + wave * (64 * HROW);
            const bool pairs = (g.col_div & 1) == 0;
            const int tl0 = pairs ? 2 * l32 : lane;
            const int tok = en0 + wn * 64 + tl0;
            size_t ocol = tok;
            if (g.col_div > 0) {
                const int b = tok / g.col_div;
                int tl = tok - b * g.col_div;
                ocol = (size_t)b * g.col_pad + tl;
            }
            bf16* const ocolp = reinterpret_cast<bf16*>(g.out_t) + ocol;
            const bool tv = tok < g.Nvalid;
#pragma unroll
            for (int half = 0; half < 2; half++) {
                const int mbase = em0 + wm * 128 + half * 64;
#pragma unroll
                for (int jj = 0; jj < 2; jj++)
#pragma unroll
                    for (int i = 0; i < TN; i++)
#pragma unroll
                        for (int gq = 0; gq < 4; gq++) {
                            const f32x16& a = acc[i][half * 2 + jj];
                            const float br = brow[half * 2 + jj];
                            const bf16x4 pk = {(bf16)(a[gq * 4] + br), (bf16)(a[gq * 4 + 1] + br), (bf16)(a[gq * 4 + 2] + br),
                                               (bf16)(a[gq * 4 + 3] + br)};
                            *reinterpret_cast<bf16x4*>(stgh + (jj * 32 + l32) * HROW + i * 32 + gq * 8 + hi * 4) = pk;
                        }
                if (pairs) {
                    uint32_t sv[32];
#pragma unroll
                    for (int it = 0; it < 32; it++) sv[it] = *reinterpret_cast<const uint32_t*>(stgh + (it * 2 + hi) * HROW + tl0);
#pragma unroll
                    for (int it = 0; it < 32; it++) {
                        const int m = mbase + it * 2 + hi;
                        if (tv && m < g.M) *reinterpret_cast<uint32_t*>(ocolp + (size_t)m * g.ldo_t) = sv[it];
                    }
                } else {
#pragma unroll 8
                    for (int row = 0; row < 64; row++) {
                        const bf16 v = stgh[row * HROW + lane];
                        if (tv && mbase + row < g.M) ocolp[(size_t)(mbase + row) * g.ldo_t] = v;
                    }
                }
            }
        } else if constexpr (EPI == WIDE_BF16 || EPI == WIDE_GELU_BF16) {
            constexpr int HROW = 68;
            bf16* const stgh = reinterpret_cast<bf16*>(smem + 65536) + wave * (64 * HROW);
            const bool full = (em0 + BM <= g.M) && (en0 + BN <= g.Nvalid);
            bf16* const obase = reinterpret_cast<bf16*>(g.out_t) + (size_t)(em0 + wm * 128 + (lane >> 4)) * g.ldo_t + n;
#pragma unroll
            for (int half = 0; half < 2; half++) {
#pragma unroll
                for (int jj = 0; jj < 2; jj++)
#pragma unroll
                    for (int i = 0; i < TN; i++)
#pragma unroll
                        for (int gq = 0; gq < 4; gq++) {
                            const f32x16& a = acc[i][half * 2 + jj];
                            f32x4 v = {a[gq * 4], a[gq * 4 + 1], a[gq * 4 + 2], a[gq * 4 + 3]};
                            v += bacc[i][gq];
                            if constexpr (EPI == WIDE_GELU_BF16) {
#pragma unroll
                                for (int e = 0; e < 4; e++) v[e] = gelu_logistic_fit(v[e]);
                            }
                            const bf16x4 pk = {(bf16)v[0], (bf16)v[1], (bf16)v[2], (bf16)v[3]};
                            *reinterpret_cast<bf16x4*>(stgh + (jj * 32 + l32) * HROW + i * 32 + gq * 8 + hi * 4) = pk;
                        }
                bf16x4 sv[16];
#pragma unroll
                for (int it = 0; it < 16; it++)
                    sv[it] = *reinterpret_cast<const bf16x4*>(stgh + (it * 4 + (lane >> 4)) * HROW + (lane & 15) * 4);
                if (full) {
#pragma unroll
                    for (int it = 0; it < 16; it++)
                        *reinterpret_cast<bf16x4*>(obase + (size_t)(half * 64 + it * 4) * g.ldo_t) = sv[it];
                } else {
#pragma unroll
                    for (int it = 0; it < 16; it++) {
                        const int m = em0 + wm * 128 + half * 64 + it * 4 + (lane >> 4);
                        if (m < g.M && nv) *reinterpret_cast<bf16x4*>(obase + (size_t)(half * 64 + it * 4) * g.ldo_t) = sv[it];
                    }
                }
            }
        } else {
            constexpr bool kResid = EPI == WIDE_RESID_F32;
            const bool full = (em0 + BM <= g.M) && (en0 + BN <= g.Nvalid);
            const float* const rbase = kResid ? g.resid + (size_t)(em0 + wm * 128 + (lane >> 4)) * g.ldr + n : nullptr;
            float* const obase = g.out_f32 + (size_t)(em0 + wm * 128 + (lane >> 4)) * g.ldo + n;
            f32x4 rw[8];
#pragma unroll
            for (int qd = 0; qd < 4; qd++) {
                f32x4* const rcur = (qd & 1) ? rw : rv;
                f32x4* const rnxt = (qd & 1) ? rv : rw;
#pragma unroll
                for (int i = 0; i < TN; i++)
#pragma unroll
                    for (int gq = 0; gq < 4; gq++) {
                        const f32x16& a = acc[i][qd];
                        const f32x4 v = {a[gq * 4], a[gq * 4 + 1], a[gq * 4 + 2], a[gq * 4 + 3]};
                        *reinterpret_cast<f32x4*>(stg + l32 * SROW + i * 32 + gq * 8 + hi * 4) = v;
                    }
                if (kResid && qd < 3) {
#pragma unroll
                    for (int it = 0; it < 8; it++) {
                        const int m = em0 + wm * 128 + (qd + 1) * 32 + it * 4 + (lane >> 4);
                        rnxt[it] = (full || (m < g.M && nv)) ? *reinterpret_cast<const f32x4*>(rbase + (size_t)((qd + 1) * 32 + it * 4) * g.ldr) : bv;
                    }
                }
                f32x4 sv[8];
#pragma unroll
                for (int it = 0; it < 8; it++)
                    sv[it] = *reinterpret_cast<const f32x4*>(stg + (it * 4 + (lane >> 4)) * SROW + (lane & 15) * 4);
#pragma unroll
                for (int it = 0; it < 8; it++) {
                    f32x4 v = sv[it] + bv;
                    if constexpr (kResid) v += rcur[it];
                    const int m = em0 + wm * 128 + qd * 32 + it * 4 + (lane >> 4);
                    if (full || (m < g.M && nv)) *reinterpret_cast<f32x4*>(obase + (size_t)(qd * 32 + it * 4) * g.ldo) = v;
                }
            }
        }
        if (tile == (int)blockIdx.x) stamp(1);
        if (next >= ntiles) break;
        tile = next;
        drain32 = EPI != WIDE_TOKCOLS_BF16 && (em0 + BM <= g.M) && (en0 + BN <= g.Nvalid);
    }
    if (g.stamps) {
        asm volatile("s_waitcnt vmcnt(0)" ::: "memory");
        stamp(3);
    }
}

static int wide_epilogue_kind(const GemmArgs& g) {
    if (g.aux || g.row_div) return -1;
    if (g.A_lo || g.B_lo) {
        if (!g.A_lo || !g.B_lo) return -1;
        if (g.mode == GEMM_EPI_LINEAR && !g.resid && g.out_f32 && !g.out_t && (g.bias_on_rows || !g.bias) && (g.col_div > 0 || g.bias_on_rows))
            return WIDE_TOKCOLS_F32;
        if (g.col_div || g.bias_on_rows || (g.Nvalid & 3)) return -1;
        if (g.mode == GEMM_EPI_LINEAR && g.resid && g.out_f32 && !g.out_t) return WIDE_RESID_F32;
        if (g.mode == GEMM_EPI_LINEAR && !g.resid && g.out_f32 && !g.out_t) return WIDE_BIAS_F32;
        if (g.mode == GEMM_EPI_GELU && !g.resid && g.out_t && g.out_lo && !g.out_f32) return WIDE_GELU_SPLIT;
        if (g.mode == GEMM_EPI_LINEAR && !g.resid && g.out_t && g.out_lo && !g.out_f32) return WIDE_SPLIT;
        return -1;
    }
    if (g.mode == GEMM_EPI_LINEAR && !g.resid && g.out_t && !g.out_f32 && (g.bias_on_rows || !g.bias) && (g.col_div > 0 || g.bias_on_rows))
        return WIDE_TOKCOLS_BF16;
    if (g.col_div || g.bias_on_rows || (g.Nvalid & 3)) return -1;
    if (g.mode == GEMM_EPI_LINEAR && !g.resid && g.out_t && !g.out_f32) return WIDE_BF16;
    if (g.mode == GEMM_EPI_GELU && !g.resid && g.out_t && !g.out_f32) return WIDE_GELU_BF16;
    if (g.mode == GEMM_EPI_LINEAR && g.resid && g.out_f32 && !g.out_t) return WIDE_RESID_F32;
    return -1;
}

template <int EPI>
static int launch_wide(const GemmArgs& g, hipStream_t s) {
    const int nbm = (g.M + 255) / 256, nbn = g.N / 256;
    const int n_cu = device_cu_count();
    if (!n_cu) return PNP_ERR_HIP;
    static std::atomic<uint32_t> opted{0};
    if (lds_opt_in(opted, reinterpret_cast<const void*>(gemm_nt_wide_kernel<EPI>), kWideSmem) != PNP_OK) return PNP_ERR_HIP;
    const int ntiles = nbm * nbn;
    int cap = n_cu;
#ifdef PNP_DEV
    if (getenv("PNP_GEMM_GRID")) cap = atoi(getenv("PNP_GEMM_GRID"));
#endif
    const int grid = ntiles > cap ? cap : ntiles;
    hipLaunchKernelGGL((gemm_nt_wide_kernel<EPI>), dim3(grid), dim3(512), kWideSmem, s, g);
    return hipGetLastError() == hipSuccess ? PNP_OK : PNP_ERR_HIP;
}

template <int NW, int KS, int NS = 4>
__global__ __launch_bounds__(NW * 64) void gemm_nt_small_x3_kernel(const GemmArgs g) {
    constexpr int BM = 64, BN = 64, ROWB = 64 * KS, ARR = 64 * ROWB, SLOT = 4 * ARR;
    constexpr int LEAD = NS - 1;
    static_assert(NS == 3 || NS == 4, "ring depth");
    constexpr int WN = NW / 2, TN = 2 / (NW / 4);
    constexpr int EPT = 32 * KS / NW;
    constexpr int PROWS = 1024 / ROWB;
    constexpr int BP = 2 * (64 / PROWS) / NW;
    constexpr int VMI = (EPT + 3) / 4 + BP;
    extern __shared__ __attribute__((aligned(16))) char smem[];
    const int tid = threadIdx.x;
    const int lane = tid & 63, wave = __builtin_amdgcn_readfirstlane(tid >> 6);
    const int r = lane & 15, q = lane >> 4;
    const int wm = wave / WN, wn = wave % WN;
    const int nbm = (g.M + BM - 1) / BM, nbn = g.N / BN;
    int bm, bn;
    tile_coords<16>(blockIdx.x, nbm, nbn, bm, bn);
    const int m0 = bm * BM, n0 = bn * BN;
    const int nk = g.K / (32 * KS);
    auto swz = [](int row) { return KS == 1 ? ((-(row >> 2)) & 3) : ((row >> 1) & 7); };

    const int a_row = tid / NW, a_e = (tid % NW) * EPT;
    int a_gr = m0 + a_row;
    a_gr = a_gr < g.M ? a_gr : g.M - 1;
    const float* a_src = reinterpret_cast<const float*>(g.A) + (size_t)a_gr * g.lda + a_e;
    const char* Bh = reinterpret_cast<const char*>(g.B);
    const char* Bl = reinterpret_cast<const char*>(g.B_lo);
    constexpr int PPA = 64 / PROWS, LPR = ROWB / 16;
    uint32_t b_off[BP];
#pragma unroll
    for (int i = 0; i < BP; i++) {
        const int p = wave * BP + i;
        const int row = (p % PPA) * PROWS + lane / LPR;
        int gr = n0 + row;
        gr = gr < g.Nvalid ? gr : g.Nvalid - 1;
        const int c = (lane % LPR) ^ swz(row);
        b_off[i] = (uint32_t)gr * (uint32_t)g.ldb * 2 + c * 16;
    }
    auto issue_b = [&](int kt) {
        char* st = smem + (kt % NS) * SLOT + 2 * ARR;
        const uint32_t koff = (uint32_t)kt * ROWB;
#pragma unroll
        for (int i = 0; i < BP; i++) {
            const int p = wave * BP + i;
            const char* base = p < PPA ? Bh : Bl;
            __builtin_amdgcn_global_load_lds((const __attribute__((address_space(1))) void*)(base + (size_t)(b_off[i] + koff)),
                                             (__attribute__((address_space(3))) void*)(st + (p / PPA) * ARR + (p % PPA) * 1024), 16, 0, 0);
        }
    };
    typedef __attribute__((ext_vector_type(EPT))) float fvec;
    fvec ra[2];
    auto load_a = [&](int kt) { ra[kt & 1] = *reinterpret_cast<const fvec*>(a_src + (size_t)kt * (32 * KS)); };
    auto store_a = [&](int kt) {
        char* st = smem + (kt % NS) * SLOT + a_row * ROWB;
        if constexpr (EPT >= 8) {
#pragma unroll
            for (int c8 = 0; c8 < EPT / 8; c8++) {
                bf16x8 h, l;
#pragma unroll
                for (int e = 0; e < 8; e++) {
                    h[e] = (bf16)ra[kt & 1][c8 * 8 + e];
                    l[e] = (bf16)(ra[kt & 1][c8 * 8 + e] - (float)h[e]);
                }
                const int off = (((a_e >> 3) + c8) ^ swz(a_row)) << 4;
                *reinterpret_cast<bf16x8*>(st + off) = h;
                *reinterpret_cast<bf16x8*>(st + ARR + off) = l;
            }
        } else {
            bf16x4 h, l;
#pragma unroll
            for (int e = 0; e < 4; e++) {
                h[e] = (bf16)ra[kt & 1][e];
                l[e] = (bf16)(ra[kt & 1][e] - (float)h[e]);
            }
            const int off = (((a_e >> 3) ^ swz(a_row)) << 4) + (a_e & 7) * 2;
            *reinterpret_cast<bf16x4*>(st + off) = h;
            *reinterpret_cast<bf16x4*>(st + ARR + off) = l;
        }
    };

    f32x4 acc[TN][2];
#pragma unroll
    for (int i = 0; i < TN; i++)
#pragma unroll
        for (int j = 0; j < 2; j++) acc[i][j] = f32x4{0.f, 0.f, 0.f, 0.f};

    const int fa_row = (wm * 32 + r) * ROWB, fb_row = 2 * ARR + (wn * 16 * TN + r) * ROWB;
    const int fsw = swz(r);

    load_a(0);
    issue_b(0);
    store_a(0);
    if (nk > 1) {
        load_a(1);
        issue_b(1);
    }
    if (LEAD > 2 && nk > 2) {
        load_a(2);
        issue_b(2);
    }
    auto iter = [&](int kt, auto rest) {
        constexpr int REST = decltype(rest)::value;
        if constexpr (REST >= 2 && LEAD == 3) PNP_WAIT_VM_LGKM(BP + VMI);
        else if constexpr (REST >= 1) PNP_WAIT_VM_LGKM(BP);
        else PNP_WAIT_VM_LGKM(0);
        __builtin_amdgcn_s_barrier();
        const char* st = smem + (kt % NS) * SLOT;
        bf16x8 ah[KS][2], al[KS][2], bh[KS][TN], bl[KS][TN];
#pragma unroll
        for (int ks = 0; ks < KS; ks++) {
            const int co = ((ks * 4 + q) ^ fsw) << 4;
#pragma unroll
            for (int j = 0; j < 2; j++) {
                ah[ks][j] = *reinterpret_cast<const bf16x8*>(st + fa_row + j * 16 * ROWB + co);
                al[ks][j] = *reinterpret_cast<const bf16x8*>(st + ARR + fa_row + j * 16 * ROWB + co);
            }
#pragma unroll
            for (int i = 0; i < TN; i++) {
                bh[ks][i] = *reinterpret_cast<const bf16x8*>(st + fb_row + i * 16 * ROWB + co);
                bl[ks][i] = *reinterpret_cast<const bf16x8*>(st + ARR + fb_row + i * 16 * ROWB + co);
            }
        }
// ... 295 lines not shown
```

### pnp-ovss_amd/csrc/gemm_wide.h

```cpp
#pragma once
#include "common.h"
#include "gemm.h"

namespace pnp {

template <int GM>
__device__ __forceinline__ void tile_coords(int bid, int nbm, int nbn, int& bm, int& bn) {
    const int nwg = nbm * nbn;
    const int qd = nwg >> 3, rm = nwg & 7, x = bid & 7, i = bid >> 3;
    const int id = (x < rm ? x * (qd + 1) : rm * (qd + 1) + (x - rm) * qd) + i;
    const int per_group = GM * nbn;
    const int rg = id / per_group, rem = id - rg * per_group;
    const int rows = (nbm - rg * GM) < GM ? (nbm - rg * GM) : GM;
    bn = rem / rows;
    bm = rg * GM + (rem - bn * rows);
}

__device__ __forceinline__ void tile_coords_rt(int gm, int bid, int nbm, int nbn, int& bm, int& bn) {
    const int nwg = nbm * nbn;
    const int qd = nwg >> 3, rm = nwg & 7, x = bid & 7, i = bid >> 3;
    const int id = (x < rm ? x * (qd + 1) : rm * (qd + 1) + (x - rm) * qd) + i;
    const int per_group = gm * nbn;
    const int rg = id / per_group, rem = id - rg * per_group;
    const int rows = (nbm - rg * gm) < gm ? (nbm - rg * gm) : gm;
    bn = rem / rows;
    bm = rg * gm + (rem - bn * rows);
}

#define PNP_WAIT_VM_LGKM(n) asm volatile("s_waitcnt vmcnt(%0) lgkmcnt(0)" ::"n"(n) : "memory")
#define PNP_WAIT_VM(n) asm volatile("s_waitcnt vmcnt(%0)" ::"n"(n) : "memory")

enum { WIDE_BF16 = 0, WIDE_GELU_BF16 = 1, WIDE_RESID_F32 = 2, WIDE_TOKCOLS_BF16 = 3, WIDE_BIAS_F32 = 4, WIDE_TOKCOLS_F32 = 5,
       WIDE_GELU_SPLIT = 6, WIDE_SPLIT = 7 };
constexpr int kWideStageRow = 68;
constexpr int kWideStageBytes = 8 * 32 * kWideStageRow * 4;
constexpr int kWideSmem = 65536 + kWideStageBytes;

int launch_x3_wide(int epi, const GemmArgs& g, hipStream_t s);

}
```

### pnp-ovss_amd/csrc/gemm_x3.hip

```cpp
#include <stdlib.h>

#include <mutex>
#include <type_traits>

#include "common.h"
#include "gemm.h"
#include "gemm_wide.h"

#ifdef PNP_EPI_NT
#define PNP_EPI_STORE(ptr, val) __builtin_nontemporal_store((val), (ptr))
#else
#define PNP_EPI_STORE(ptr, val) (*(ptr) = (val))
#endif

namespace pnp {

typedef __attribute__((ext_vector_type(4))) uint32_t frag16;

__device__ __forceinline__ void x3_half(f32x4& c0, f32x4& c1, const frag16& ah, const frag16& al, const frag16& bh0, const frag16& bh1,
                                        const frag16& bl0, const frag16& bl1) {
    asm volatile(
        "v_mfma_f32_16x16x32_bf16 %0, %6, %2, %0\n\t"
        "v_mfma_f32_16x16x32_bf16 %1, %7, %2, %1\n\t"
        "v_mfma_f32_16x16x32_bf16 %0, %4, %3, %0\n\t"
        "v_mfma_f32_16x16x32_bf16 %1, %5, %3, %1\n\t"
        "v_mfma_f32_16x16x32_bf16 %0, %4, %2, %0\n\t"
        "v_mfma_f32_16x16x32_bf16 %1, %5, %2, %1"
        : "+v"(c0), "+v"(c1)
        : "v"(ah), "v"(al), "v"(bh0), "v"(bh1), "v"(bl0), "v"(bl1));
}

typedef __attribute__((ext_vector_type(4))) uint32_t u32x4;
typedef __attribute__((address_space(1))) uint32_t gu32;
#ifdef PNP_SK_PLAIN
#define PNP_SK_AUX 0
#else
#define PNP_SK_AUX 16
#endif

template <int EPI, bool SK>
__global__ __launch_bounds__(512) void gemm_nt_x3_kernel(const GemmArgs g) {
    constexpr int BM = 256, BN = 256, SLOT = 65536, ARR = 16384;
    constexpr int JM = 8, IN = 4;
    constexpr int NDMA = 8;
    constexpr int kDrain = (EPI == WIDE_GELU_SPLIT || EPI == WIDE_SPLIT) ? 32 : 24;
    constexpr int SROW = kWideStageRow;
    extern __shared__ __attribute__((aligned(16))) char smem[];

    const int tid = threadIdx.x;
    const int lane = tid & 63, wave = __builtin_amdgcn_readfirstlane(tid >> 6);
    const int r = lane & 15, q = lane >> 4;
    const int wm = wave >> 2, wn = wave & 3;
    const int nbm = (g.M + BM - 1) / BM, nbn = g.N / BN;
    const int ntiles = nbm * nbn;
    const int nk = g.K / 32;
    const char* Ab = reinterpret_cast<const char*>(g.A);
    const char* Bb = reinterpret_cast<const char*>(g.B);
    const char* Alo = reinterpret_cast<const char*>(g.A_lo);
    const char* Blo = reinterpret_cast<const char*>(g.B_lo);

    uint32_t soff[4];
    auto set_tile = [&](int tile, int& m0, int& n0, int lane) {
        int bm, bn;
#ifdef PNP_DEV
        if (g.ablate >= 100) {
            if (g.ablate == 100) {
                bm = tile / nbn;
                bn = tile - bm * nbn;
            } else {
                tile_coords_rt(g.ablate - 100, tile, nbm, nbn, bm, bn);
            }
        } else
#endif
        tile_coords<4>(tile, nbm, nbn, bm, bn);
        m0 = bm * BM;
        n0 = bn * BN;
        const uint32_t lda_b = (uint32_t)g.lda * 2, ldb_b = (uint32_t)g.ldb * 2;
        const int c = (lane & 3) ^ ((-(lane >> 4)) & 3);
#pragma unroll
        for (int i = 0; i < 2; i++) {
            const int row = (wave * 2 + i) * 16 + (lane >> 2);
            int gr = m0 + row;
            gr = gr < g.M ? gr : g.M - 1;
            soff[i] = (uint32_t)gr * lda_b + c * 16;
            gr = n0 + row;
            gr = gr < g.Nvalid ? gr : g.Nvalid - 1;
            soff[2 + i] = (uint32_t)gr * ldb_b + c * 16;
        }
    };
    auto issue_one = [&](int kt, int i, uint32_t on) {
#ifdef PNP_X3_ABLATE
        if (kt >= 2) return;
#endif
        const int op = i >> 2, rg = (i >> 1) & 1, lo = i & 1;
        const char* base = op ? (lo ? Blo : Bb) : (lo ? Alo : Ab);
        const int d = (kt & 1) * SLOT + op * (2 * ARR) + lo * ARR + (wave * 2 + rg) * 1024;
        const uint32_t lds = (uint32_t)(uintptr_t)(__attribute__((address_space(3))) char*)(smem + d);
        uint32_t voff;
        uint64_t saved;
        asm volatile(
            "s_mov_b64 %1, exec\n\t"
            "s_cmp_lg_u32 %6, 0\n\t"
            "s_cselect_b64 exec, exec, 0\n\t"
            "v_add_u32 %0, %3, %2\n\t"
            "s_mov_b32 m0, %5\n\t"
            "s_nop 0\n\t"
            "global_load_lds_dwordx4 %0, %4\n\t"
            "s_mov_b64 exec, %1"
            : "=&v"(voff), "=&s"(saved)
            : "v"(soff[op * 2 + rg]), "s"((uint32_t)kt * 64), "s"(base), "s"(lds), "s"(on)
            : "memory", "scc");
    };
    auto stamp_sk = [&](int slot) {
        if (g.stamps && tid == 0) {
            g.stamps[((size_t)gridDim.x + blockIdx.x) * 8 + slot] = __builtin_readcyclecounter();
            g.stamps[((size_t)gridDim.x + blockIdx.x) * 8 + 4 + slot] = wall_clock64();
        }
    };
    auto stamp = [&](int slot) {
        if (g.stamps && tid == 0) {
            g.stamps[(size_t)blockIdx.x * 8 + slot] = __builtin_readcyclecounter();
            g.stamps[(size_t)blockIdx.x * 8 + 4 + slot] = wall_clock64();
        }
    };

    const int fo = r * 64 + ((q ^ ((-(r >> 2)) & 3)) << 4);
    int fa_off[2], fb_off[2];
    fa_off[0] = wm * (128 * 64) + fo;
    fb_off[0] = 2 * ARR + wn * (64 * 64) + fo;
    fa_off[1] = fa_off[0] + SLOT;
    fb_off[1] = fb_off[0] + SLOT;
    asm volatile("" : "+v"(fa_off[1]), "+v"(fb_off[1]));
    float* const stg = reinterpret_cast<float*>(smem + SLOT) + wave * (32 * SROW);

    const int bid = blockIdx.x;
    enum { kWhole = 0, kProduce = 1, kOwn = 2 };
    auto get_work = [&](int wi, int& t, int& k0, int& k1, int& kind) {
        const int grid = gridDim.x;
        const int full = SK ? g.sk_full : ntiles;
        t = bid + wi * grid;
        if (t < full) {
            k0 = 0;
            k1 = nk;
            kind = kWhole;
            return true;
        }
        if constexpr (SK) {
            const int j = wi - g.sk_full / grid;
            const int nk2 = nk >> 1;
            const int T = (ntiles - full) * nk2;
            const int u0 = bid * g.sk_upw;
            const int u1 = u0 + g.sk_upw < T ? u0 + g.sk_upw : T;
            if (u0 >= u1 || j > 1) return false;
            const int ta = u0 / nk2, bnd = (ta + 1) * nk2;
            const bool owns = u1 >= bnd, two = u1 > bnd;
            if (j == 0 && (two || !owns)) {
                t = full + ta + (two ? 1 : 0);
                k0 = two ? 0 : 2 * (u0 - ta * nk2);
                k1 = 2 * (u1 - (two ? bnd : ta * nk2));
                kind = kProduce;
                return true;
            }
            if (owns && (j == 0 || two)) {
                t = full + ta;
                k0 = 2 * (u0 - ta * nk2);
                k1 = nk;
                kind = k0 ? kOwn : kWhole;
                return true;
            }
        }
        return false;
    };
    int wi = 0, tile, k0, k1, kind;
    if (!get_work(0, tile, k0, k1, kind)) return;
    int m0, n0;
    bool drain32 = false;
    stamp(0);
    set_tile(tile, m0, n0, lane);
#pragma unroll
    for (int i = 0; i < NDMA; i++) issue_one(k0, i, 1u);

    for (;;) {
        f32x4 acc[JM][IN];
#pragma unroll
        for (int j = 0; j < JM; j++)
#pragma unroll
            for (int i = 0; i < IN; i++) acc[j][i] = f32x4{0.f, 0.f, 0.f, 0.f};

        frag16 ah[4], al[4], bh[2][IN], bl[2][IN];
        auto rd_a = [&](int slot, int s, int jm) {
#if defined(PNP_X3_ABLATE) && PNP_X3_ABLATE >= 4
            return;
#endif
            const char* p = smem + fa_off[s] + jm * 1024;
            ah[slot] = *reinterpret_cast<const frag16*>(p);
            al[slot] = *reinterpret_cast<const frag16*>(p + ARR);
        };
        auto rd_b = [&](int set, int s, int in) {
// ... 11 lines not shown
#pragma unroll
        for (int i = 0; i < NDMA; i++) issue_one(k0 + 1, i, 1u);
        rd_a(0, 0, 0);
        rd_a(1, 0, 1);
        rd_a(2, 0, 2);
#pragma unroll
        for (int i = 0; i < IN; i++) rd_b(0, 0, i);

        auto slab = [&](int kt, auto par) {
            constexpr int S = decltype(par)::value;
            const uint32_t head = __builtin_amdgcn_readfirstlane((kt >= k0 + 1 && kt + 1 < k1) ? 1 : 0);
            const uint32_t tail = __builtin_amdgcn_readfirstlane((kt + 2 < k1) ? 1 : 0);
#pragma unroll
            for (int j = 0; j < JM; j++) {
                x3_half(acc[j][0], acc[j][1], ah[j & 3], al[j & 3], bh[S][0], bh[S][1], bl[S][0], bl[S][1]);
                if (j + 3 < JM) {
                    rd_a((j + 3) & 3, S, j + 3);
                    if (j < 2) issue_one(kt + 1, 4 + 2 * j, head);
                } else {
                    if (j == JM - 3) {
#if !defined(PNP_X3_ABLATE) || PNP_X3_ABLATE < 3
                        __builtin_amdgcn_s_waitcnt(0x0070);
                        __builtin_amdgcn_s_barrier();
#endif
                    }
                    rd_a((j + 3) & 3, S ^ 1, j + 3 - JM);
                    if (j == JM - 2) rd_b(S ^ 1, S ^ 1, 1);
                    if (j == JM - 1) rd_b(S ^ 1, S ^ 1, 3);
                    if (j == JM - 3) issue_one(kt + 2, 0, tail);
                    if (j == JM - 2) issue_one(kt + 2, 2, tail);
                }
                x3_half(acc[j][2], acc[j][3], ah[j & 3], al[j & 3], bh[S][2], bh[S][3], bl[S][2], bl[S][3]);
                if (j < 2) issue_one(kt + 1, 5 + 2 * j, head);
                if (j == JM - 3) {
                    rd_b(S ^ 1, S ^ 1, 0);
                    issue_one(kt + 2, 1, tail);
                }
                if (j == JM - 2) {
                    rd_b(S ^ 1, S ^ 1, 2);
                    issue_one(kt + 2, 3, tail);
                }
            }
        };
        constexpr std::integral_constant<int, 0> s0{};
        constexpr std::integral_constant<int, 1> s1{};
        for (int kt = k0; kt < k1; kt += 2) {
            slab(kt, s0);
            slab(kt + 1, s1);
        }
        asm volatile("s_nop 15\n\ts_nop 15" ::: "memory");
        if (wi == 0) stamp(2);

        __syncthreads();
        int ntile, nk0, nk1, nkind;
        const bool have_next = get_work(wi + 1, ntile, nk0, nk1, nkind);
        auto request_next = [&]() {
            if (have_next) {
                set_tile(ntile, m0, n0, lane);
#pragma unroll
                for (int i = 0; i < NDMA; i++) issue_one(nk0, i, 1u);
            }
        };
        if constexpr (SK) {
            if (kind == kProduce) {
                stamp_sk(0);
                request_next();
                const __amdgpu_buffer_rsrc_t rs = __builtin_amdgcn_make_buffer_rsrc(g.sk_part + (size_t)bid * (BM * BN), 0, BM * BN * 4, 0x00020000);
#if !defined(PNP_SK_ABLATE) || PNP_SK_ABLATE < 1 || PNP_SK_ABLATE == 3
                {
                    int voff = tid * 16;
#pragma unroll
                    for (int j = 0; j < JM; j++)
#pragma unroll
                        for (int i = 0; i < IN; i++) {
                            __builtin_amdgcn_raw_buffer_store_b128(__builtin_bit_cast(u32x4, acc[j][i]), rs, voff, 0, PNP_SK_AUX);
                            voff += 8192;
                            asm volatile("" : "+v"(voff));
                        }
                }
#endif
#ifdef PNP_SK_PLAIN
                asm volatile("s_waitcnt vmcnt(0)" ::: "memory");
                __syncthreads();
                if (tid == 0) {
                    __builtin_amdgcn_fence(__ATOMIC_RELEASE, "agent");
                    asm volatile("s_waitcnt vmcnt(0)" ::: "memory");
                }
#endif
                asm volatile("s_waitcnt vmcnt(0)" ::: "memory");
                __syncthreads();
                if (tid == 0) __hip_atomic_store((gu32*)(g.sk_flag + bid), 1u, __ATOMIC_RELAXED, __HIP_MEMORY_SCOPE_AGENT);
                stamp_sk(1);
            }
            if (kind == kOwn) {
                const int np = ((k0 >> 1) + g.sk_upw - 1) / g.sk_upw;
                stamp_sk(2);
                for (int pj = 1; pj <= np; pj++) {
                    const int src = bid - pj;
                    if (wave == 0) {
                        gu32* const fl = (gu32*)(g.sk_flag + src);
                        uint32_t spins = 0;
#if defined(PNP_SK_ABLATE) && PNP_SK_ABLATE >= 2
                        while (false) {
#else
                        while (__hip_atomic_load(fl, __ATOMIC_RELAXED, __HIP_MEMORY_SCOPE_AGENT) != 1u) {
#endif
                            __builtin_amdgcn_s_sleep(8);
                            if (++spins > (1u << 22)) {
                                if (lane == 0) __hip_atomic_store((gu32*)g.sk_tmo, 1u + (uint32_t)bid, __ATOMIC_RELAXED, __HIP_MEMORY_SCOPE_AGENT);
                                break;
                            }
                        }
                        if (lane == 0) __hip_atomic_store(fl, 0u, __ATOMIC_RELAXED, __HIP_MEMORY_SCOPE_AGENT);
                    }
                    __syncthreads();
                    const __amdgpu_buffer_rsrc_t rs = __builtin_amdgcn_make_buffer_rsrc(g.sk_part + (size_t)src * (BM * BN), 0, BM * BN * 4, 0x00020000);
#ifdef PNP_SK_PLAIN
                    if (tid == 0) {
                        __builtin_amdgcn_fence(__ATOMIC_ACQUIRE, "agent");
                        asm volatile("s_waitcnt vmcnt(0)" ::: "memory");
                    }
                    __syncthreads();
#endif
#if !defined(PNP_SK_ABLATE) || PNP_SK_ABLATE < 1 || PNP_SK_ABLATE == 4
                    int voff = tid * 16;
#pragma unroll
                    for (int grp = 0; grp < 4; grp++) {
                        u32x4 t[8];
#pragma unroll
                        for (int x = 0; x < 8; x++) {
                            t[x] = __builtin_amdgcn_raw_buffer_load_b128(rs, voff, 0, PNP_SK_AUX);
                            voff += 8192;
                            asm volatile("" : "+v"(voff));
                        }
#pragma unroll
                        for (int x = 0; x < 8; x++) acc[(grp * 8 + x) / IN][(grp * 8 + x) % IN] += __builtin_bit_cast(f32x4, t[x]);
                    }
#endif
                }
                stamp_sk(3);
            }
        }
        bool next_drain = false;
        if (!SK || kind != kProduce) {
        int etid = tid;
        asm volatile("" : "+v"(etid));
        const int lane = etid & 63, r = lane & 15, q = lane >> 4;
        const int em0 = m0, en0 = n0;
        const int n = en0 + wn * 64 + (lane & 15) * 4;
        const bool nv = n < g.Nvalid;
        f32x4 bv = {0.f, 0.f, 0.f, 0.f};
        f32x4 rv[8];
        f32x4 bacc[IN];
        if constexpr (EPI == WIDE_GELU_SPLIT || EPI == WIDE_SPLIT) {
#pragma unroll
            for (int i = 0; i < IN; i++) {
                const int nn = en0 + wn * 64 + i * 16 + q * 4;
                bacc[i] = (g.bias && nn < g.Nvalid) ? *reinterpret_cast<const f32x4*>(g.bias + nn) : bv;
            }
        }
        if constexpr (EPI == WIDE_BIAS_F32 || EPI == WIDE_RESID_F32) {
            if (g.bias && nv) bv = *reinterpret_cast<const f32x4*>(g.bias + n);
        }
        if constexpr (EPI == WIDE_RESID_F32) {
            const int mrow0 = em0 + wm * 128 + (lane >> 4);
#pragma unroll
            for (int it = 0; it < 8; it++) {
                const int m = mrow0 + it * 4;
                rv[it] = (m < g.M && nv) ? *reinterpret_cast<const f32x4*>(g.resid + (size_t)m * g.ldr + n) : bv;
            }
        }
        float brow[JM] = {0.f, 0.f, 0.f, 0.f, 0.f, 0.f, 0.f, 0.f};
        if constexpr (EPI == WIDE_TOKCOLS_F32) {
#pragma unroll
            for (int j = 0; j < JM; j++) {
                const int m = em0 + wm * 128 + j * 16 + r;
                if (g.bias && m < g.M) brow[j] = g.bias[m];
            }
        }

        if constexpr (EPI == WIDE_TOKCOLS_F32) {
            const int l32 = lane & 31, hi = lane >> 5;
            const bool pairs = (g.col_div & 1) == 0;
            const int tl0 = pairs ? 2 * l32 : lane;
            const int tok = en0 + wn * 64 + tl0;
            size_t ocol = tok;
            if (g.col_div > 0) {
                const int b = tok / g.col_div;
                const int tl = tok - b * g.col_div;
                ocol = (size_t)b * g.col_pad + tl;
            }
            float* const ocolp = g.out_f32 + ocol;
            const bool tv = tok < g.Nvalid;
#pragma unroll
            for (int qd = 0; qd < 4; qd++) {
                const int mbase = em0 + wm * 128 + qd * 32;
#pragma unroll
                for (int j2 = 0; j2 < 2; j2++)
#pragma unroll
                    for (int i = 0; i < IN; i++) {
                        const float br = brow[qd * 2 + j2];
                        const f32x4 v = acc[qd * 2 + j2][i] + br;
                        *reinterpret_cast<f32x4*>(stg + (j2 * 16 + r) * SROW + i * 16 + q * 4) = v;
                    }
                if (qd == 0) request_next();
                if (pairs) {
                    f32x2 sv[16];
#pragma unroll
                    for (int it = 0; it < 16; it++) sv[it] = *reinterpret_cast<const f32x2*>(stg + (it * 2 + hi) * SROW + tl0);
#pragma unroll
                    for (int it = 0; it < 16; it++) {
                        const int m = mbase + it * 2 + hi;
                        if (tv && m < g.M) *reinterpret_cast<f32x2*>(ocolp + (size_t)m * g.ldo) = sv[it];
                    }
                } else {
#pragma unroll 8
                    for (int row = 0; row < 32; row++) {
                        const float v = stg[row * SROW + lane];
                        if (tv && mbase + row < g.M) ocolp[(size_t)(mbase + row) * g.ldo] = v;
                    }
                }
            }
        } else if constexpr (EPI == WIDE_GELU_SPLIT || EPI == WIDE_SPLIT) {
            constexpr int HROW = 68;
            bf16* const stgh = reinterpret_cast<bf16*>(smem + SLOT) + wave * (64 * HROW);
            const bool full = (em0 + BM <= g.M) && (en0 + BN <= g.Nvalid);
#pragma unroll
            for (int half = 0; half < 2; half++) {
#pragma unroll
                for (int j4 = 0; j4 < 4; j4++)
#pragma unroll
                    for (int i = 0; i < IN; i++)
#pragma unroll
                        for (int e = 0; e < 4; e += 2) {
                            f32x4& a = acc[half * 4 + j4][i];
                            pnp_f32x2 v = {a[e] + bacc[i][e], a[e + 1] + bacc[i][e + 1]};
                            if constexpr (EPI == WIDE_GELU_SPLIT) v = gelu_erf_fast2(v);
                            a[e] = v[0];
                            a[e + 1] = v[1];
                        }
                if (half == 0) request_next();
#pragma unroll
                for (int part = 0; part < 2; part++) {
                    bf16* const obase = reinterpret_cast<bf16*>(part ? g.out_lo : g.out_t) + (size_t)(em0 + wm * 128 + (lane >> 4)) * g.ldo_t + n;
#pragma unroll
                    for (int j4 = 0; j4 < 4; j4++)
#pragma unroll
                        for (int i = 0; i < IN; i++) {
                            const f32x4& a = acc[half * 4 + j4][i];
                            bf16x4 pk;
#pragma unroll
                            for (int e = 0; e < 4; e++) {
                                const float v = a[e];
                                const bf16 h = (bf16)v;
                                pk[e] = part ? (bf16)(v - (float)h) : h;
                            }
                            *reinterpret_cast<bf16x4*>(stgh + (j4 * 16 + r) * HROW + i * 16 + q * 4) = pk;
                        }
                    bf16x4 sv[16];
#pragma unroll
                    for (int it = 0; it < 16; it++)
                        sv[it] = *reinterpret_cast<const bf16x4*>(stgh + (it * 4 + (lane >> 4)) * HROW + (lane & 15) * 4);
#pragma unroll
                    for (int it = 0; it < 16; it++) {
                        const int m = em0 + wm * 128 + half * 64 + it * 4 + (lane >> 4);
                        if (full || (m < g.M && nv)) PNP_EPI_STORE(reinterpret_cast<bf16x4*>(obase + (size_t)(half * 64 + it * 4) * g.ldo_t), sv[it]);
                    }
                }
            }
        } else {
            constexpr bool kResid = EPI == WIDE_RESID_F32;
            const bool full = (em0 + BM <= g.M) && (en0 + BN <= g.Nvalid);
            const float* const rbase = kResid ? g.resid + (size_t)(em0 + wm * 128 + (lane >> 4)) * g.ldr + n : nullptr;
            float* const obase = g.out_f32 + (size_t)(em0 + wm * 128 + (lane >> 4)) * g.ldo + n;
            f32x4 rw[8];
#pragma unroll
            for (int qd = 0; qd < 4; qd++) {
                f32x4* const rcur = (qd & 1) ? rw : rv;
                f32x4* const rnxt = (qd & 1) ? rv : rw;
#pragma unroll
                for (int j2 = 0; j2 < 2; j2++)
#pragma unroll
                    for (int i = 0; i < IN; i++)
                        *reinterpret_cast<f32x4*>(stg + (j2 * 16 + r) * SROW + i * 16 + q * 4) = acc[qd * 2 + j2][i];
                if (kResid && qd < 3) {
#pragma unroll
                    for (int it = 0; it < 8; it++) {
                        const int m = em0 + wm * 128 + (qd + 1) * 32 + it * 4 + (lane >> 4);
                        rnxt[it] = (full || (m < g.M && nv)) ? *reinterpret_cast<const f32x4*>(rbase + (size_t)((qd + 1) * 32 + it * 4) * g.ldr) : bv;
                    }
                }
                f32x4 sv[8];
#pragma unroll
                for (int it = 0; it < 8; it++)
                    sv[it] = *reinterpret_cast<const f32x4*>(stg + (it * 4 + (lane >> 4)) * SROW + (lane & 15) * 4);
#pragma unroll
                for (int it = 0; it < 8; it++) {
                    f32x4 v = sv[it] + bv;
                    if constexpr (kResid) v += rcur[it];
                    const int m = em0 + wm * 128 + qd * 32 + it * 4 + (lane >> 4);
                    if (full || (m < g.M && nv)) PNP_EPI_STORE(reinterpret_cast<f32x4*>(obase + (size_t)(qd * 32 + it * 4) * g.ldo), v);
                }
                if (qd == 0) request_next();
            }
        }
        next_drain = (EPI != WIDE_TOKCOLS_F32) && (em0 + BM <= g.M) && (en0 + BN <= g.Nvalid);
        }
        if (wi == 0) stamp(1);
        if (!have_next) break;
        wi++;
        tile = ntile;
        k0 = nk0;
        k1 = nk1;
        kind = nkind;
        drain32 = next_drain;
    }
    if (g.stamps) {
        asm volatile("s_waitcnt vmcnt(0)" ::: "memory");
        stamp(3);
    }
}

static std::atomic<int> g_streamk_mode{1};
void set_streamk_mode(int m) { g_streamk_mode.store(m, std::memory_order_relaxed); }
int streamk_mode() { return g_streamk_mode.load(std::memory_order_relaxed); }
static bool streamk_pays(int tail, int cap, int nk2, int upw, int np) {
    const double x = (double)tail / cap;
    const double whole = (nk2 + 2.0) * (x <= 0.6 ? 0.75 : 0.75 + (x - 0.6) * 0.857);
    const double sk = 1.05 * upw + 4.0 + (tail <= 64 ? 1.0 : 4.5) + 0.75 * np + 1.5;
    return sk * 1.05 + 0.5 < whole;
}

template <int EPI>
static int launch_x3(GemmArgs g, hipStream_t s) {
    const int nbm = (g.M + 255) / 256, nbn = g.N / 256;
    const int n_cu = device_cu_count();
    if (!n_cu) return PNP_ERR_HIP;
    static std::atomic<uint32_t> opted{0}, opted_sk{0};
    const int ntiles = nbm * nbn;
    int cap = n_cu;
#ifdef PNP_DEV
    if (getenv("PNP_GEMM_GRID")) cap = atoi(getenv("PNP_GEMM_GRID"));
#endif
    const int mode = streamk_mode();
    StreamKWs* const ws = g.sk;
    if (mode && ws && ws->part && ws->wgs >= cap) {
        const int rounds = ntiles / cap, tail = ntiles - rounds * cap, nk2 = g.K / 64;
        if (tail > 0) {
            const int upw = (int)(((long)tail * nk2 + cap - 1) / cap);
            const int np = (nk2 - 1 + upw - 1) / upw;
            hipStreamCaptureStatus cap_st = hipStreamCaptureStatusNone;
            const bool capturing = hipStreamIsCapturing(s, &cap_st) == hipSuccess && cap_st != hipStreamCaptureStatusNone;
            if (!capturing && (mode == 2 || streamk_pays(tail, cap, nk2, upw, np))) {
                if (lds_opt_in(opted_sk, reinterpret_cast<const void*>(gemm_nt_x3_kernel<EPI, true>), kWideSmem) != PNP_OK) return PNP_ERR_HIP;
                g.sk_part = ws->part;
                g.sk_flag = ws->flag;
                g.sk_tmo = ws->flag + ws->wgs;
                g.sk_full = rounds * cap;
                g.sk_upw = upw;
                ws->launches++;
                static std::mutex mu;
                static hipEvent_t last[kMaxDevices];
                const int d = current_device();
                if (d < 0) return PNP_ERR_HIP;
                std::lock_guard<std::mutex> lk(mu);
                if (!last[d]) {
                    if (hipEventCreateWithFlags(&last[d], hipEventDisableTiming) != hipSuccess) return PNP_ERR_HIP;
                } else if (hipStreamWaitEvent(s, last[d], 0) != hipSuccess) {
                    return PNP_ERR_HIP;
                }
                hipLaunchKernelGGL((gemm_nt_x3_kernel<EPI, true>), dim3(cap), dim3(512), kWideSmem, s, g);
                const bool ok = hipGetLastError() == hipSuccess && hipEventRecord(last[d], s) == hipSuccess;
                return ok ? PNP_OK : PNP_ERR_HIP;
            }
        }
    }
    if (lds_opt_in(opted, reinterpret_cast<const void*>(gemm_nt_x3_kernel<EPI, false>), kWideSmem) != PNP_OK) return PNP_ERR_HIP;
    const int grid = ntiles > cap ? cap : ntiles;
    hipLaunchKernelGGL((gemm_nt_x3_kernel<EPI, false>), dim3(grid), dim3(512), kWideSmem, s, g);
    return hipGetLastError() == hipSuccess ? PNP_OK : PNP_ERR_HIP;
}

int streamk_ws_create(StreamKWs* ws, int wgs) {
    if (!ws || wgs <= 0) return PNP_ERR_ARG;
    const size_t fbytes = ((size_t)(wgs + 1) * 4 + 15) / 16 * 16;
    if (hipMalloc(&ws->part, (size_t)wgs * 256 * 256 * 4) != hipSuccess) return PNP_ERR_HIP;
    if (hipMalloc(&ws->flag, fbytes) != hipSuccess || hipMemset(ws->flag, 0, fbytes) != hipSuccess) {
        (void)hipFree(ws->part);
        ws->part = nullptr;
        return PNP_ERR_HIP;
    }
    ws->wgs = wgs;
    return PNP_OK;
}

void streamk_ws_destroy(StreamKWs* ws) {
    if (!ws) return;
    if (ws->part) (void)hipFree(ws->part);
    if (ws->flag) (void)hipFree(ws->flag);
    *ws = StreamKWs();
}

int streamk_ws_timeouts(StreamKWs* ws, unsigned* out) {
    if (!ws || !out) return PNP_ERR_ARG;
    *out = 0;
    if (!ws->flag) return PNP_OK;
    return hipMemcpy(out, ws->flag + ws->wgs, 4, hipMemcpyDeviceToHost) == hipSuccess ? PNP_OK : PNP_ERR_HIP;
}

StreamKWs* streamk_ws_default() {
    static StreamKWs ws[kMaxDevices];
    static std::mutex mu;
    const int d = current_device();
    if (d < 0) return nullptr;
    std::lock_guard<std::mutex> lk(mu);
    if (!ws[d].part) {
        const int n = device_cu_count();
        if (!n || streamk_ws_create(&ws[d], n) != PNP_OK) return nullptr;
    }
    return &ws[d];
}

int launch_x3_wide(int epi, const GemmArgs& g, hipStream_t s) {
    switch (epi) {
        case WIDE_RESID_F32: return launch_x3<WIDE_RESID_F32>(g, s);
        case WIDE_BIAS_F32: return launch_x3<WIDE_BIAS_F32>(g, s);
        case WIDE_GELU_SPLIT: return launch_x3<WIDE_GELU_SPLIT>(g, s);
        case WIDE_SPLIT: return launch_x3<WIDE_SPLIT>(g, s);
        case WIDE_TOKCOLS_F32: return launch_x3<WIDE_TOKCOLS_F32>(g, s);
    }
    return PNP_ERR_ARG;
}

}
```

### pnp-ovss_amd/csrc/kernels.h

```cpp
#pragma once
#include <hip/hip_runtime.h>
#include <stdint.h>
#include <stddef.h>
#include "gemm.h"

namespace pnp {

struct PostDesc {
    int H, W, K, C, has_bg, pix0;
    int Kp;
    int G, Kg;
    size_t off;
    size_t qoff;
    size_t voff[2];
};

struct alignas(16) CrfEntry {
    uint32_t pixel;
    float w;
    float nr;
    uint32_t pad;
};

struct alignas(16) CrfNbr8 {
    int ia, id;
    int pa, pd;
    int aa, ad;
    int da, dd;
};

struct CrfLattice {
    int D1;
    int which;
    size_t cap;
    float* bary;
    uint32_t* vals;
    CrfEntry* ent;
    int* offset;
    int* seg_start;
    int* seg_lo;
    int* seg_hi;
    uint64_t* ukeys;
    int* idbase;
    int* n1;
    int* n2;
    CrfNbr8* nbr8;
};

int patchify(int bf, const float* img, const uint8_t* dropped, void* out, int B, int S, int P, hipStream_t s);
int cls_rows(const float* cls, const float* pos, float* x, int B, int N, int D, hipStream_t s);
int layernorm(int bf, const float* x, const float* w, const float* b, float eps, int rows, int D, float* y, void* yt,
              float* xhat, float* rstd, hipStream_t s, void* yt_lo = nullptr);
int vit_attention(int bf, const void* qk, int ld_qk, int D, const void* vt, int ld_vt, int Npad, void* ctx, int B,
                  int H, int N, float scale, hipStream_t s, void* ctx_lo = nullptr);

int vit_attention_x3(const void* qkv_hi, const void* qkv_lo, int ld_qk, int D, void* ctx_hi, void* ctx_lo, int B, int H, int N,
                     float scale, hipStream_t s);

int text_embed(const int64_t* ids, int ld_ids, const float* word, const float* pos, float* out, int B, int L, int H,
               int enc_id, int vocab, hipStream_t s);
int text_self_attn(int bf, const void* qkv, const int64_t* mask, int ld_mask, void* ctx, float* probs, float* scratch, int B, int L,
                   int H, hipStream_t s);
int text_self_attn_bwd(int bf, const void* qkv, const float* dctx, const float* probs, float* ds_scratch, void* dqkv,
                       int B, int L, int H, hipStream_t s);
int xattn(int bf, int mode, const void* a1, int ld1, const void* a2t, int ld2, int Npad, const void* x, int ldx,
          void* out, int ldo, float* pbuf, int Nst, int B, int L, int N, int nheads, hipStream_t s);
int layernorm_bwd(int bf, const float* dy, const float* w, const float* xhat, const float* rstd, int rows, int D,
                  float* dx, void* dxt, hipStream_t s);
int itm_head(const float* hlast, const float* w, const float* bias, float* logits, int B, int L, int H, hipStream_t s);
int itm_grad_seed(const float* w, float* dh, int B, int L, int H, hipStream_t s);
int cast_f32(int bf, const float* in, void* out, size_t n, hipStream_t s);
int split_f32(const float* in, void* hi, void* lo, size_t n, hipStream_t s);

int gradcam_gather(const float* P, const float* dP, const int64_t* mask, int ld_mask, float* out, int B, int nheads,
                   int head, int L, int Nst, int PP, hipStream_t s);
int drop_step(const float* G, float* g0, float* agg, uint8_t* dropped, int32_t* picks, int iter, int B, int T, int PP,
              int npick, int max_picks, hipStream_t s);
int merge_tokens(const float* src, const int32_t* cls_off, const int32_t* tok_idx, const int32_t* cls_div,
                 const int32_t* img_cls_off, float* out, int B, int T, int PP, int Cmax, hipStream_t s);
int threshold_maps(const float* merged, const int32_t* img_cls_off, float* out, float threshold, int B, int PP, int Cmax,
                   hipStream_t s);
int upsample_maps(const float* src, const PostDesc* desc, float* maps, int B, int P, int Cmax, int maxHW, hipStream_t s);
int minmax_normalize(float* maps, const PostDesc* desc, float* stats, int B, int Kmax, int maxHW, int class_channels_only,
                     hipStream_t s);
int background_channel(float* maps, const PostDesc* desc, int B, int maxHW, hipStream_t s);
int blur_maps(const float* in, float* tmp, float* out, const PostDesc* desc, const double* wts, const int32_t* wt_off,
              int B, int Kmax, int maxH, int maxW, int max_radius, hipStream_t s);
int preprocess_images(const uint8_t* rgb, const void* desc, int B, int S, int max_H, const int32_t* coef, uint8_t* tmp,
                      const float* mean3, const float* std3, float* out, hipStream_t s);
int unary_from_maps(const float* maps, const PostDesc* desc, float* unary, int B, int maxHW, int max_kp, int group, hipStream_t s);
int argmax_remap(const float* q, const PostDesc* desc, const int32_t* lut, int lut_stride, uint8_t* labels,
                 const size_t* label_off, int pixel_major, int group, int B, int maxHW, hipStream_t s);
int confusion_hist(const uint8_t* labels, const float* gt, const PostDesc* desc, const size_t* label_off,
                   unsigned long long* hist, int n_class, int B, int maxHW, hipStream_t s);

struct JpegImage {
    int64_t data_off;
    int64_t coef_off[3];
    int64_t plane_off[3];
    int64_t rgb_off;
    int32_t data_len, H, W, ncomp, hmax, vmax, mcux, mcuy;
    int32_t h[3], v[3], tq[3], td[3], ta[3], bx[3], by[3];
    int32_t tab, pad[2];
};
struct JpegTables {
    uint8_t counts[4][16];
    uint8_t vals[4][256];
    int32_t quant[4][64];
};
struct JpegSegment {
    int64_t byte_off;
    int64_t clean_off;
    int32_t image, mcu0, nmcu;
    int32_t raw_len;
    int32_t clean_cap;
    int32_t sub_bits;
    int32_t pad[2];
};
int jpeg_decode(const uint8_t* d_data, const JpegImage* d_imgs, const JpegTables* d_tabs, const JpegSegment* d_segs, int n_images,
                int n_segments, uint8_t* d_clean, int* d_seg_bits, int16_t* d_coef, size_t coef_elems, uint8_t* d_planes, uint8_t* d_rgb,
                int max_blocks, int max_pixels, int* d_err, hipStream_t s);

size_t sort_temp_bytes(size_t n);
int radix_sort_pairs(uint64_t* keys_in, uint64_t* keys_out, uint32_t* vals_in, uint32_t* vals_out, size_t n, int begin_bit, int end_bit,
                     const size_t* seg_off, int nseg, void* temp, size_t temp_bytes, hipStream_t s);
int device_scan_i32(const int* in, int* out, size_t n, bool inclusive, void* temp, size_t temp_bytes, hipStream_t s);
size_t crf_sort_temp_bytes(size_t max_entries, int max_images);
int crf_build_lattice(int D, const CrfLattice& L, const PostDesc* d_imgs, const PostDesc* h_imgs, const uint8_t* d_rgb, float sxy, float srgb,
                      int B, size_t ent_total, int max_pixels,
                      uint64_t* keys_a, uint64_t* keys_b, uint32_t* vals_a, int* head, int* incl, int* n1k, int* n2k,
                      void* temp, size_t temp_bytes, int* d_range_err, int* h_range_err, int* h_points, hipStream_t s);
int crf_lattice_norm(const CrfLattice& L, const PostDesc* d_imgs, int B, int max_pixels, size_t ent_total, float* va, float* vb,
                     float* norm_out, hipStream_t s);
int crf_filter(const CrfLattice& L, const PostDesc* d_imgs, int img0, int nimg, const float* Q,
               float* va, float* vb, const float** result, int max_kp, hipStream_t s);
struct CrfLabelOut {
    uint8_t* lab[2] = {nullptr, nullptr};
    const int32_t* lut = nullptr;
    int lut_stride = 0;
    const size_t* label_off = nullptr;
};
int crf_update(const CrfLattice& Lg, const CrfLattice& Lb, const PostDesc* d_imgs, int img0, int nimg, const float* vg,
               const float* vb, const float* norm_g, const float* norm_b, const float* unary, float* Q, float w_g,
               float w_b, int pairwise, int max_pixels, int max_kp, int groups, hipStream_t s, const CrfLabelOut& labels = CrfLabelOut());

}
```

### pnp-ovss_amd/csrc/vit_kernels.hip

```cpp
#include <stdlib.h>

#include "common.h"
#include "kernels.h"

namespace pnp {

template <typename T>
__global__ void patchify_kernel(const float* __restrict__ img, const uint8_t* __restrict__ dropped,
                                T* __restrict__ out, int B, int S, int P) {
    const int idx = blockIdx.x * blockDim.x + threadIdx.x;
    const int total = B * P * P * 3 * 16;
    if (idx >= total) return;
    const int i = idx & 15;
    const int c = (idx >> 4) % 3;
    const int m = idx / 48;
    const int b = m / (P * P), p = m - b * P * P;
    const int py = p / P, px = p - py * P;
    T* o = out + (size_t)m * 768 + c * 256 + i * 16;
    const bool drop = dropped && dropped[m];
    const float* src = img + (((size_t)b * 3 + c) * S + (py * 16 + i)) * S + px * 16;
#pragma unroll
    for (int v = 0; v < 4; v++) {
        f32x4 x = drop ? f32x4{0.f, 0.f, 0.f, 0.f} : *reinterpret_cast<const f32x4*>(src + v * 4);
#pragma unroll
// ... 220 lines not shown
    const int b = blockIdx.z, h = blockIdx.y;
    const size_t row0 = (size_t)b * N;
    const int qw = blockIdx.x * nwaves + wave;
    int qrow = qw * 32 + l32;
    const bool q_valid = qw < nqw && qrow < N;
    qrow = qrow < N ? qrow : N - 1;

    bf16x8 fq[4];
    {
        const bf16* qp = qk + (row0 + qrow) * ld_qk + h * 64 + hi * 8;
#pragma unroll
        for (int ks = 0; ks < 4; ks++) fq[ks] = *reinterpret_cast<const bf16x8*>(qp + ks * 16);
    }

    const char* kbase = reinterpret_cast<const char*>(qk + row0 * ld_qk + D + h * 64);
    const char* vbase = reinterpret_cast<const char*>(vt + row0 * ld_vt + h * 64);
    const int prow = lane >> 3, pc = lane & 7;
    auto issue_tile = [&](int t) {
        char* dst = ring[t & 1];
        for (int p = wave; p < 16; p += nwaves) {
            const int row = (p & 7) * 8 + prow;
            const int sc = pc ^ ((row >> 1) & 7);
            int key = t * 64 + row;
            key = key < N ? key : N - 1;
            const char* src = p < 8 ? kbase + (size_t)key * ld_qk * 2 + sc * 16 : vbase + (size_t)key * ld_vt * 2 + sc * 16;
            __builtin_amdgcn_global_load_lds((const __attribute__((address_space(1))) void*)src,
                                             (__attribute__((address_space(3))) void*)(dst + p * 1024), 16, 0, 0);
        }
    };

    f32x16 o[2];
#pragma unroll
    for (int i = 0; i < 2; i++)
#pragma unroll
        for (int e = 0; e < 16; e++) o[i][e] = 0.f;
    float m_run = -INFINITY, l_run = 0.f;
    const float c = scale * 1.4426950408889634f;
    const int sw = (l32 >> 1) & 7;
    const int ntiles = (N + 63) / 64;

    issue_tile(0);
    for (int t = 0; t < ntiles; t++) {
        asm volatile("s_waitcnt vmcnt(0)" ::: "memory");
        __builtin_amdgcn_s_barrier();
        if (t + 1 < ntiles) issue_tile(t + 1);
        const char* Ks = ring[t & 1];
        const char* Vs = Ks + TILE;

        bf16x8 fk[2][4];
#pragma unroll
        for (int kt = 0; kt < 2; kt++)
#pragma unroll
            for (int ks = 0; ks < 4; ks++)
                fk[kt][ks] = *reinterpret_cast<const bf16x8*>(Ks + (kt * 32 + l32) * ROWB + (((ks * 2 + hi) ^ sw) << 4));
        f32x16 s[2];
        const f32x16 zero16 = {0.f, 0.f, 0.f, 0.f, 0.f, 0.f, 0.f, 0.f, 0.f, 0.f, 0.f, 0.f, 0.f, 0.f, 0.f, 0.f};
#pragma unroll
        for (int kt = 0; kt < 2; kt++) {
            s[kt] = __builtin_amdgcn_mfma_f32_32x32x16_bf16(fk[kt][0], fq[0], zero16, 0, 0, 0);
#pragma unroll
            for (int ks = 1; ks < 4; ks++) s[kt] = __builtin_amdgcn_mfma_f32_32x32x16_bf16(fk[kt][ks], fq[ks], s[kt], 0, 0, 0);
        }
        if (t == ntiles - 1 && (N & 63)) {
#pragma unroll
            for (int kt = 0; kt < 2; kt++)
#pragma unroll
                for (int e = 0; e < 16; e++) {
                    const int key = t * 64 + kt * 32 + (e >> 2) * 8 + hi * 4 + (e & 3);
                    if (key >= N) s[kt][e] = -INFINITY;
                }
        }
        float mx;
        asm("v_max3_f32 %0, %1, %2, %3" : "=v"(mx) : "v"(s[0][0]), "v"(s[0][1]), "v"(s[0][2]));
#pragma unroll
        for (int e = 3; e + 1 < 16; e += 2) asm("v_max3_f32 %0, %1, %2, %3" : "=v"(mx) : "v"(mx), "v"(s[0][e]), "v"(s[0][e + 1]));
        asm("v_max3_f32 %0, %1, %2, %3" : "=v"(mx) : "v"(mx), "v"(s[0][15]), "v"(s[1][0]));
#pragma unroll
        for (int e = 1; e + 1 < 16; e += 2) asm("v_max3_f32 %0, %1, %2, %3" : "=v"(mx) : "v"(mx), "v"(s[1][e]), "v"(s[1][e + 1]));
        asm("v_max3_f32 %0, %1, %2, %3" : "=v"(mx) : "v"(mx), "v"(s[1][15]), "v"(m_run));
        const float m_new = fmaxf(mx, __shfl_xor(mx, 32, 64));
        {
            const float alpha = __builtin_amdgcn_exp2f((m_run - m_new) * c);
#pragma unroll
            for (int i = 0; i < 2; i++) o[i] *= alpha;
            l_run *= alpha;
            m_run = m_new;
        }
        const float mc = -m_run * c;
        bf16x8 fp[4];
#pragma unroll
        for (int kt = 0; kt < 2; kt++)
#pragma unroll
            for (int e = 0; e < 16; e++) {
                const float p = __builtin_amdgcn_exp2f(fmaf(s[kt][e], c, mc));
                l_run += p;
                fp[kt * 2 + (e >> 3)][e & 7] = (bf16)p;
            }
        const int grp_d = ((lane >> 4) & 1) * 16, tq = (lane >> 2) & 3, tp = lane & 3;
#pragma unroll
        for (int j = 0; j < 4; j++)
#pragma unroll
            for (int dt = 0; dt < 2; dt++) {
                typedef __attribute__((ext_vector_type(4))) short s16x4;
                s16x4 part[2];
#pragma unroll
                for (int u = 0; u < 2; u++) {
                    const int key = 16 * j + 8 * u + 4 * hi + tq;
                    const int col = dt * 32 + grp_d + 4 * tp;
                    const char* a = Vs + key * ROWB + ((((col >> 3)) ^ ((key >> 1) & 7)) << 4) + (col & 7) * 2;
                    part[u] = __builtin_amdgcn_ds_read_tr16_b64_v4i16((__attribute__((address_space(3))) s16x4*)a);
                }
                const bf16x4 lo = __builtin_bit_cast(bf16x4, part[0]), hh = __builtin_bit_cast(bf16x4, part[1]);
                const bf16x8 fv = {lo[0], lo[1], lo[2], lo[3], hh[0], hh[1], hh[2], hh[3]};
                o[dt] = __builtin_amdgcn_mfma_f32_32x32x16_bf16(fv, fp[j], o[dt], 0, 0, 0);
            }
    }
    l_run += __shfl_xor(l_run, 32, 64);
    if (q_valid) {
        const float inv = 1.0f / l_run;
        bf16* op = ctx + (row0 + qrow) * D + h * 64 + hi * 4;
#pragma unroll
        for (int dt = 0; dt < 2; dt++)
#pragma unroll
            for (int g4 = 0; g4 < 4; g4++) {
                const bf16x4 pk = {(bf16)(o[dt][g4 * 4] * inv), (bf16)(o[dt][g4 * 4 + 1] * inv), (bf16)(o[dt][g4 * 4 + 2] * inv),
                                   (bf16)(o[dt][g4 * 4 + 3] * inv)};
                *reinterpret_cast<bf16x4*>(op + dt * 32 + g4 * 8) = pk;
            }
    }
}

#ifdef PNP_DEV
__device__ unsigned long long* g_attn_stamps = nullptr;
__device__ int g_attn_ablate = 0;
extern "C" int pnp_dev_attn_ablate(int on) {
    return hipMemcpyToSymbol(HIP_SYMBOL(g_attn_ablate), &on, sizeof(on)) == hipSuccess ? PNP_OK : PNP_ERR_HIP;
}
extern "C" int pnp_dev_attn_stamps(unsigned long long* d_buf) {
    return hipMemcpyToSymbol(HIP_SYMBOL(g_attn_stamps), &d_buf, sizeof(d_buf)) == hipSuccess ? PNP_OK : PNP_ERR_HIP;
}
#define PNP_ATTN_STAMP(k)                                                                                       \
    do {                                                                                                        \
        if (stamps && lane == 0) {                                                                              \
            __builtin_amdgcn_sched_barrier(0);                                                                  \
            stamps[((size_t)wave * ntiles + t) * 6 + (k)] = __builtin_readcyclecounter();                       \
            __builtin_amdgcn_sched_barrier(0);                                                                  \
        }                                                                                                       \
    } while (0)
#else
#define PNP_ATTN_STAMP(k) do {} while (0)
#endif

__global__ __launch_bounds__(768) void vit_attn32_x3_kernel(const bf16* __restrict__ qk, const bf16* __restrict__ qk_lo, int ld_qk, int D,
                                                            const bf16* __restrict__ vt, const bf16* __restrict__ vt_lo, int ld_vt,
                                                            bf16* __restrict__ ctx, bf16* __restrict__ ctx_lo, int N, float scale, int nqw) {
    constexpr int ROWB = 128, TILE = 64 * ROWB;
    __shared__ __attribute__((aligned(16))) char ring[2][4 * TILE];

    const int tid = threadIdx.x, lane = tid & 63, wave = __builtin_amdgcn_readfirstlane(tid >> 6);
    const int nwaves = blockDim.x >> 6;
    const int l32 = lane & 31, hi = lane >> 5;
    const int b = blockIdx.z, h = blockIdx.y;
    const size_t row0 = (size_t)b * N;
    const int qw = blockIdx.x * nwaves + wave;
    int qrow = qw * 32 + l32;
    const bool q_valid = qw < nqw && qrow < N;
    qrow = qrow < N ? qrow : N - 1;

    bf16x8 fq[4], fql[4];
    {
        const size_t off = (row0 + qrow) * ld_qk + h * 64 + hi * 8;
#pragma unroll
        for (int ks = 0; ks < 4; ks++) {
            fq[ks] = *reinterpret_cast<const bf16x8*>(qk + off + ks * 16);
            fql[ks] = *reinterpret_cast<const bf16x8*>(qk_lo + off + ks * 16);
        }
    }
    const size_t koff = (row0 * ld_qk + D + h * 64) * 2, voff = (row0 * ld_vt + h * 64) * 2;
    const uint64_t k0 = reinterpret_cast<uint64_t>(qk) + koff;
    const uint64_t d_klo = reinterpret_cast<uint64_t>(qk_lo) + koff - k0;
    const uint64_t d_v = reinterpret_cast<uint64_t>(vt) + voff - k0;
    const uint64_t d_vlo = reinterpret_cast<uint64_t>(vt_lo) + voff - k0;
    const int prow = lane >> 3, pc = lane & 7;
    const uint32_t sc_even = (uint32_t)(pc ^ ((prow >> 1) & 7)) << 4, sc_odd = (uint32_t)(pc ^ ((4 + (prow >> 1)) & 7)) << 4;
    auto issue_tile = [&](int t) {
        for (int p = wave; p < 32; p += nwaves) {
            const uint64_t m_v = 0ull - (uint64_t)((p >> 3) & 1), m_lo = 0ull - (uint64_t)(p >> 4);
            const uint64_t d = (m_v & m_lo & d_vlo) | (m_v & ~m_lo & d_v) | (~m_v & m_lo & d_klo);
            const uint32_t ld2 = ((uint32_t)ld_qk + ((uint32_t)m_v & (uint32_t)(ld_vt - ld_qk))) * 2u;
            int rs = t * 64 + (p & 7) * 8;
#ifdef PNP_DEV
            if (g_attn_ablate) rs = (p & 7) * 8;
#endif
            rs = rs < N - 1 ? rs : N - 1;
            const char* const sbase = reinterpret_cast<const char*>(k0 + d + (uint64_t)((uint32_t)rs * ld2));
            int lr = rs + prow;
            lr = (lr < N ? lr : N - 1) - rs;
            const uint32_t loff = (uint32_t)lr * ld2 + ((p & 1) ? sc_odd : sc_even);
            const uint32_t lds = (uint32_t)(uintptr_t)(__attribute__((address_space(3))) char*)(ring[t & 1] + p * 1024);
            const uint64_t sb = reinterpret_cast<uint64_t>(sbase);
            const uint64_t sbu = ((uint64_t)(uint32_t)__builtin_amdgcn_readfirstlane((int)(sb >> 32)) << 32) |
                                 (uint32_t)__builtin_amdgcn_readfirstlane((int)(uint32_t)sb);
            asm volatile("s_mov_b32 m0, %2\n\ts_nop 0\n\tglobal_load_lds_dwordx4 %0, %1" ::"v"(loff), "s"(sbu),
                         "s"(__builtin_amdgcn_readfirstlane((int)lds))
                         : "memory");
        }
    };

    f32x16 o[2];
#pragma unroll
    for (int i = 0; i < 2; i++)
#pragma unroll
        for (int e = 0; e < 16; e++) o[i][e] = 0.f;
    float m_run = -INFINITY, l_run = 0.f;
    const float c = scale * 1.4426950408889634f;
    const int sw = (l32 >> 1) & 7;
    const int ntiles = (N + 63) / 64;

#ifdef PNP_DEV
    unsigned long long* const stamps = (blockIdx.x | blockIdx.y | blockIdx.z) == 0 ? g_attn_stamps : nullptr;
#endif
    issue_tile(0);
    for (int t = 0; t < ntiles; t++) {
        PNP_ATTN_STAMP(0);
        asm volatile("s_waitcnt vmcnt(0)" ::: "memory");
        __builtin_amdgcn_s_barrier();
        PNP_ATTN_STAMP(1);
        if (t + 1 < ntiles) issue_tile(t + 1);
        PNP_ATTN_STAMP(2);
        const char* Ks = ring[t & 1];
        const char* Vs = Ks + TILE;
        const char* Kl = Ks + 2 * TILE;
        const char* Vl = Ks + 3 * TILE;

        f32x16 s[2];
        const f32x16 zero16 = {0.f, 0.f, 0.f, 0.f, 0.f, 0.f, 0.f, 0.f, 0.f, 0.f, 0.f, 0.f, 0.f, 0.f, 0.f, 0.f};
#pragma unroll
        for (int kt = 0; kt < 2; kt++) {
            s[kt] = zero16;
#pragma unroll
            for (int ks = 0; ks < 4; ks++) {
                const int a = (kt * 32 + l32) * ROWB + (((ks * 2 + hi) ^ sw) << 4);
                const bf16x8 kl = *reinterpret_cast<const bf16x8*>(Kl + a);
                const bf16x8 kh = *reinterpret_cast<const bf16x8*>(Ks + a);
                s[kt] = __builtin_amdgcn_mfma_f32_32x32x16_bf16(kl, fq[ks], s[kt], 0, 0, 0);
                s[kt] = __builtin_amdgcn_mfma_f32_32x32x16_bf16(kh, fql[ks], s[kt], 0, 0, 0);
                s[kt] = __builtin_amdgcn_mfma_f32_32x32x16_bf16(kh, fq[ks], s[kt], 0, 0, 0);
            }
        }
        PNP_ATTN_STAMP(3);
        if (t == ntiles - 1 && (N & 63)) {
#pragma unroll
            for (int kt = 0; kt < 2; kt++)
#pragma unroll
                for (int e = 0; e < 16; e++) {
                    const int key = t * 64 + kt * 32 + (e >> 2) * 8 + hi * 4 + (e & 3);
                    if (key >= N) s[kt][e] = -INFINITY;
                }
        }
        float mx = m_run;
#pragma unroll
        for (int kt = 0; kt < 2; kt++)
#pragma unroll
            for (int e = 0; e < 16; e++) mx = fmaxf(mx, s[kt][e]);
        const float m_new = fmaxf(mx, __shfl_xor(mx, 32, 64));
        {
            const float alpha = __builtin_amdgcn_exp2f((m_run - m_new) * c);
#pragma unroll
            for (int i = 0; i < 2; i++) o[i] *= alpha;
            l_run *= alpha;
            m_run = m_new;
        }
        const float mc = -m_run * c;
        bf16x8 fp[4], fpl[4];
#pragma unroll
        for (int kt = 0; kt < 2; kt++)
#pragma unroll
            for (int e = 0; e < 16; e++) {
                const float p = __builtin_amdgcn_exp2f(fmaf(s[kt][e], c, mc));
                l_run += p;
                const bf16 ph = (bf16)p;
                fp[kt * 2 + (e >> 3)][e & 7] = ph;
                fpl[kt * 2 + (e >> 3)][e & 7] = (bf16)(p - (float)ph);
            }
        PNP_ATTN_STAMP(4);
        const int grp_d = ((lane >> 4) & 1) * 16, tq = (lane >> 2) & 3, tp = lane & 3;
#pragma unroll
        for (int j = 0; j < 4; j++)
#pragma unroll
            for (int dt = 0; dt < 2; dt++) {
                typedef __attribute__((ext_vector_type(4))) short s16x4;
                bf16x8 fv[2];
#pragma unroll
                for (int part = 0; part < 2; part++) {
                    const char* V = part ? Vl : Vs;
                    s16x4 pr[2];
#pragma unroll
                    for (int u = 0; u < 2; u++) {
                        const int key = 16 * j + 8 * u + 4 * hi + tq;
                        const int col = dt * 32 + grp_d + 4 * tp;
                        const char* a = V + key * ROWB + ((((col >> 3)) ^ ((key >> 1) & 7)) << 4) + (col & 7) * 2;
                        pr[u] = __builtin_amdgcn_ds_read_tr16_b64_v4i16((__attribute__((address_space(3))) s16x4*)a);
                    }
                    const bf16x4 lo = __builtin_bit_cast(bf16x4, pr[0]), hh = __builtin_bit_cast(bf16x4, pr[1]);
                    fv[part] = bf16x8{lo[0], lo[1], lo[2], lo[3], hh[0], hh[1], hh[2], hh[3]};
                }
                o[dt] = __builtin_amdgcn_mfma_f32_32x32x16_bf16(fv[1], fp[j], o[dt], 0, 0, 0);
                o[dt] = __builtin_amdgcn_mfma_f32_32x32x16_bf16(fv[0], fpl[j], o[dt], 0, 0, 0);
                o[dt] = __builtin_amdgcn_mfma_f32_32x32x16_bf16(fv[0], fp[j], o[dt], 0, 0, 0);
            }
        PNP_ATTN_STAMP(5);
    }
    l_run += __shfl_xor(l_run, 32, 64);
    if (q_valid) {
        const float inv = 1.0f / l_run;
        const size_t off = (row0 + qrow) * D + h * 64 + hi * 4;
#pragma unroll
        for (int dt = 0; dt < 2; dt++)
#pragma unroll
            for (int g4 = 0; g4 < 4; g4++) {
                bf16x4 ph, pl;
#pragma unroll
                for (int e = 0; e < 4; e++) {
                    const float v = o[dt][g4 * 4 + e] * inv;
                    ph[e] = (bf16)v;
                    pl[e] = (bf16)(v - (float)ph[e]);
                }
                *reinterpret_cast<bf16x4*>(ctx + off + dt * 32 + g4 * 8) = ph;
                *reinterpret_cast<bf16x4*>(ctx_lo + off + dt * 32 + g4 * 8) = pl;
            }
    }
}

int vit_attention(int bf, const void* qk, int ld_qk, int D, const void* vt, int ld_vt, int Npad, void* ctx, int B,
                  int H, int N, float scale, hipStream_t s, void* ctx_lo) {
    if (D != H * 64 || Npad % 64 || Npad < N) return PNP_ERR_ARG;
    if (bf) {
        if (ctx_lo) return PNP_ERR_ARG;
        const int nqw = (N + 31) / 32;
        const int max_wpb = 8;
        const int nblk = (nqw + max_wpb - 1) / max_wpb, wpb = (nqw + nblk - 1) / nblk;
        hipLaunchKernelGGL(vit_attn32_kernel, dim3(nblk, H, B), dim3(wpb * 64), 0, s, (const bf16*)qk, ld_qk, D,
                           (const bf16*)vt, ld_vt, Npad, (bf16*)ctx, N, scale, nqw);
        return hipGetLastError() == hipSuccess ? PNP_OK : PNP_ERR_HIP;
    }
    dim3 grid((N + 63) / 64, H, B);
    hipLaunchKernelGGL((vit_attn_kernel<float>), grid, dim3(256), 0, s, (const float*)qk, ld_qk, D, (const float*)vt, ld_vt,
                       Npad, ctx_lo ? nullptr : (float*)ctx, N, scale, ctx_lo ? (bf16*)ctx : nullptr, (bf16*)ctx_lo);
    return hipGetLastError() == hipSuccess ? PNP_OK : PNP_ERR_HIP;
}

int vit_attention_x3(const void* qkv_hi, const void* qkv_lo, int ld_qk, int D, void* ctx_hi, void* ctx_lo, int B, int H, int N,
                     float scale, hipStream_t s) {
    if (D != H * 64 || !qkv_hi || !qkv_lo || !ctx_hi || !ctx_lo) return PNP_ERR_ARG;
    const int nqw = (N + 31) / 32;
    int max_wpb = nqw > 24 ? 12 : 8;
#ifdef PNP_DEV
    if (getenv("PNP_ATTN_WPB")) max_wpb = atoi(getenv("PNP_ATTN_WPB"));
#endif
    const int nblk = (nqw + max_wpb - 1) / max_wpb, wpb = (nqw + nblk - 1) / nblk;
    const bf16 *qh = (const bf16*)qkv_hi, *ql = (const bf16*)qkv_lo;
    hipLaunchKernelGGL(vit_attn32_x3_kernel, dim3(nblk, H, B), dim3(wpb * 64), 0, s, qh, ql, ld_qk, D, qh + 2 * D, ql + 2 * D, ld_qk,
                       (bf16*)ctx_hi, (bf16*)ctx_lo, N, scale, nqw);
    return hipGetLastError() == hipSuccess ? PNP_OK : PNP_ERR_HIP;
}

int patchify(int bf, const float* img, const uint8_t* dropped, void* out, int B, int S, int P, hipStream_t s) {
    const int total = B * P * P * 48;
    const int nb = (total + 255) / 256;
    if (bf) hipLaunchKernelGGL((patchify_kernel<bf16>), dim3(nb), dim3(256), 0, s, img, dropped, (bf16*)out, B, S, P);
    else hipLaunchKernelGGL((patchify_kernel<float>), dim3(nb), dim3(256), 0, s, img, dropped, (float*)out, B, S, P);
    return hipGetLastError() == hipSuccess ? PNP_OK : PNP_ERR_HIP;
}

int cls_rows(const float* cls, const float* pos, float* x, int B, int N, int D, hipStream_t s) {
    hipLaunchKernelGGL(cls_rows_kernel, dim3((B * D + 255) / 256), dim3(256), 0, s, cls, pos, x, B, N, D);
    return hipGetLastError() == hipSuccess ? PNP_OK : PNP_ERR_HIP;
}

int layernorm(int bf, const float* x, const float* w, const float* b, float eps, int rows, int D, float* y, void* yt,
              float* xhat, float* rstd, hipStream_t s, void* yt_lo) {
    if (D > 1024 || D % 4) return PNP_ERR_ARG;
    if (yt_lo && !bf) return PNP_ERR_ARG;
    const int nb = (rows + 3) / 4;
    if (bf) hipLaunchKernelGGL((layernorm_kernel<bf16>), dim3(nb), dim3(256), 0, s, x, w, b, eps, rows, D, y, (bf16*)yt, xhat, rstd, (bf16*)yt_lo);
    else hipLaunchKernelGGL((layernorm_kernel<float>), dim3(nb), dim3(256), 0, s, x, w, b, eps, rows, D, y, (float*)yt, xhat, rstd, (bf16*)nullptr);
    return hipGetLastError() == hipSuccess ? PNP_OK : PNP_ERR_HIP;
}

}
```

### pnp-ovss_amd/pnp_ovss/hip.py

```python
import ctypes as C
import os

import numpy as np
import torch

_HERE = os.path.dirname(os.path.abspath(__file__))
LIB_PATH = os.environ.get("PNP_HIP_LIB") or os.path.join(_HERE, "libpnp_hip.so")


class PnpConfig(C.Structure):
    _fields_ = [(n, C.c_int32) for n in ("img_size", "patch", "vit_dim", "vit_depth", "vit_heads", "vit_mlp_ratio")] + \
               [("vit_ln_eps", C.c_float)] + \
               [(n, C.c_int32) for n in ("txt_hidden", "txt_layers", "txt_heads", "txt_inter")] + \
               [("txt_ln_eps", C.c_float)] + \
               [(n, C.c_int32) for n in ("vocab", "max_pos", "enc_token_id", "max_batch", "max_text_len",
                                         "stash_layer", "compute_bf16", "device")]


class PnpPostBatch(C.Structure):
    _fields_ = [("B", C.c_int32),
                ("H", C.POINTER(C.c_int32)), ("W", C.POINTER(C.c_int32)),
                ("n_classes", C.POINTER(C.c_int32)), ("has_bg", C.POINTER(C.c_int32)),
                ("img_cls_off", C.POINTER(C.c_int32)), ("cls_off", C.POINTER(C.c_int32)),
                ("tok_idx", C.POINTER(C.c_int32)), ("cls_div", C.POINTER(C.c_int32)),
                ("lut", C.POINTER(C.c_int32)), ("lut_stride", C.c_int32),
                ("d_rgb", C.c_void_p), ("d_gt", C.c_void_p),
                ("blur_wts", C.POINTER(C.c_double)), ("blur_wt_off", C.POINTER(C.c_int32))]


_lib = None


def load_library():
    global _lib
    if _lib is not None:
        return _lib
    if not os.path.exists(LIB_PATH):
        raise RuntimeError(f"{LIB_PATH} not built: run `python -c 'import __graft_entry__ as g; g.build()'` "
                           f"or `make -C pnp-ovss_amd/csrc` (there is no CPU fallback)")
    lib = C.CDLL(LIB_PATH)
    vp, i32, i64, f32 = C.c_void_p, C.c_int32, C.c_int64, C.c_float
    sig = {
        "pnp_create": (i32, [C.POINTER(PnpConfig), C.POINTER(vp)]),
        "pnp_create_shared": (i32, [C.POINTER(PnpConfig), vp, C.POINTER(vp)]),
        "pnp_destroy": (None, [vp]),
        "pnp_last_error": (C.c_char_p, [vp]),
        "pnp_workspace_bytes": (C.c_size_t, [C.POINTER(PnpConfig)]),
        "pnp_allocated_bytes": (C.c_size_t, [vp]),
        "pnp_load_weight": (i32, [vp, C.c_char_p, vp, C.POINTER(i64), i32, i32]),
        "pnp_finalize_weights": (i32, [vp]),
        "pnp_vit_forward": (i32, [vp, vp, vp, i32, vp]),
        "pnp_cross_kv": (i32, [vp, i32, vp]),
        "pnp_text_forward_xattn": (i32, [vp, vp, vp, i32, i32, i32, vp, vp]),
        "pnp_xattn_grad": (i32, [vp, i32, i32, vp]),
        "pnp_xattn_grad_layer": (i32, [vp, i32, i32, i32, vp]),
        "pnp_compute_gradcam_layer": (i32, [vp, vp, vp, vp, vp, i32, i32, i32, i32, i32, vp, vp, vp]),
        "pnp_drop_loop_layer": (i32, [vp, vp, vp, vp, i32, i32, i32, i32, i32, i32, i32, vp, vp, vp, vp, vp]),
        "pnp_gradcam_gather": (i32, [vp, vp, i32, i32, i32, i32, vp, vp]),
        "pnp_compute_gradcam": (i32, [vp, vp, vp, vp, vp, i32, i32, i32, i32, vp, vp, vp]),
        "pnp_drop_step": (i32, [vp, vp, vp, vp, vp, vp, i32, i32, i32, i32, i32, vp]),
        "pnp_drop_loop": (i32, [vp, vp, vp, vp, i32, i32, i32, i32, i32, i32, vp, vp, vp, vp, vp]),
        "pnp_post_reserve": (i32, [vp, i32, i64, i32, i32, i32]),
        "pnp_post_prepare": (i32, [vp, C.POINTER(PnpPostBatch), i32, vp]),
        "pnp_merge_tokens": (i32, [vp, vp, i32, vp]),
        "pnp_threshold_upsample": (i32, [vp, f32, i32, vp]),
        "pnp_blur_minmax": (i32, [vp, vp]),
        "pnp_densecrf": (i32, [vp, i32, f32, f32, f32, f32, f32, vp]),
        "pnp_remap_hist": (i32, [vp, i32, vp, vp, i32, vp]),
        "pnp_postprocess": (i32, [vp, vp, i32, f32, i32, i32, vp, vp, i32, vp]),
        "pnp_postprocess_pair": (i32, [vp, vp, vp, i32, f32, i32, vp, vp, vp, vp, i32, vp]),
        "pnp_get_buffer": (i32, [vp, C.c_char_p, C.POINTER(vp), C.POINTER(C.c_size_t)]),
        "pnp_profile_enable": (i32, [vp, i32]),
        "pnp_profile_read": (i32, [vp, C.POINTER(i64), C.POINTER(C.c_double), C.POINTER(C.c_double)]),
        "pnp_profile_read_stage": (i32, [vp, i32, C.POINTER(i64), C.POINTER(C.c_double), C.POINTER(C.c_double)]),
        "pnp_op_gemm": (i32, [i32, vp, i32, vp, i32, i32, i32, i32, vp, vp, i32, vp, i32, i32, vp]),
        "pnp_op_gemm_ex": (i32, [i32, vp, i32, vp, i32, i32, i32, i32, vp, vp, i32, vp, i32, vp, i32, i32, vp]),
        "pnp_op_gemm_tokcols": (i32, [i32, vp, i32, vp, i32, i32, i32, i32, vp, vp, i32, i32, i32, vp]),
        "pnp_op_vit_attention": (i32, [i32, vp, i32, i32, vp, i32, i32, vp, i32, i32, i32, f32, vp]),
        "pnp_op_vit_attention_x3": (i32, [vp, vp, i32, i32, vp, vp, i32, i32, i32, f32, vp]),
        "pnp_preprocess_images": (i32, [vp, vp, i32, i32, i32, vp, vp, C.POINTER(C.c_float), C.POINTER(C.c_float), vp, vp]),
        "pnp_op_layernorm": (i32, [vp, vp, vp, f32, i32, i32, vp, vp]),
        "pnp_op_cast": (i32, [i32, vp, vp, i64, vp]),
        "pnp_jpeg_decode": (i32, [vp, vp, vp, vp, i32, i32, vp, vp, vp, i64, vp, vp, i32, i32, vp, vp]),
        "pnp_op_split": (i32, [vp, vp, vp, i64, vp]),
        "pnp_op_gemm_x3": (i32, [vp, vp, i32, vp, vp, i32, i32, i32, i32, vp, i32, vp, i32, vp, i32, vp, vp, i32, i32, i32, i32, vp]),
        "pnp_op_gemm_x3a": (i32, [vp, i32, vp, vp, i32, i32, i32, i32, vp, vp, i32, vp, i32, i32, vp, i32, vp]),
        "pnp_dbg_gemm_stamps": (i32, [vp, i32]),
        "pnp_op_xattn": (i32, [i32, i32, vp, i32, vp, i32, i32, vp, i32, vp, i32, vp, i32, i32, i32, i32, i32, vp]),
        "pnp_op_sort_pairs": (i32, [vp, vp, vp, vp, i64, i32, i32, vp, i32, vp]),
        "pnp_op_scan_i32": (i32, [vp, vp, i64, i32, vp]),
        "pnp_set_tuning": (i32, [C.c_char_p, i32]),
        "pnp_streamk_status": (i32, [vp, C.POINTER(i64), C.POINTER(C.c_uint32)]),
    }
    for name, (res, args) in sig.items():
        fn = getattr(lib, name)
        fn.restype = res
        fn.argtypes = args
    _lib = lib
    return lib


EXPORTED = ["pnp_create", "pnp_create_shared", "pnp_destroy", "pnp_last_error", "pnp_workspace_bytes", "pnp_load_weight",
            "pnp_finalize_weights", "pnp_vit_forward", "pnp_text_forward_xattn", "pnp_xattn_grad",
            "pnp_gradcam_gather", "pnp_compute_gradcam", "pnp_drop_step", "pnp_drop_loop", "pnp_post_reserve",
            "pnp_post_prepare", "pnp_merge_tokens", "pnp_threshold_upsample", "pnp_blur_minmax", "pnp_densecrf",
            "pnp_remap_hist", "pnp_postprocess", "pnp_postprocess_pair", "pnp_get_buffer", "pnp_profile_enable", "pnp_profile_read", "pnp_op_gemm", "pnp_op_gemm_ex", "pnp_op_layernorm", "pnp_op_cast", "pnp_op_xattn", "pnp_dbg_gemm_stamps", "pnp_op_gemm_tokcols", "pnp_op_vit_attention", "pnp_preprocess_images",
            "pnp_cross_kv", "pnp_profile_read_stage", "pnp_op_split", "pnp_op_gemm_x3", "pnp_op_gemm_x3a",
            "pnp_xattn_grad_layer", "pnp_compute_gradcam_layer", "pnp_drop_loop_layer", "pnp_allocated_bytes",
            "pnp_op_vit_attention_x3", "pnp_jpeg_decode", "pnp_op_sort_pairs", "pnp_op_scan_i32", "pnp_set_tuning",
            "pnp_streamk_status"]


class _DevView:

    def __init__(self, ptr, shape, typestr):
        self.__cuda_array_interface__ = {"shape": tuple(shape), "typestr": typestr, "data": (int(ptr), False),
                                         "version": 2, "strides": None}


def _stream():
    return C.c_void_p(torch.cuda.current_stream().cuda_stream)


def _ptr(t):
    if t is None:
        return None
    assert t.is_cuda and t.is_contiguous(), "device-contiguous tensor required"
    return C.c_void_p(t.data_ptr())


def _i32p(a):
    return a.ctypes.data_as(C.POINTER(C.c_int32))


class PnpPreImage(C.Structure):
    _fields_ = [("src_off", C.c_int64), ("tmp_off", C.c_int64), ("H", C.c_int32), ("W", C.c_int32),
                ("kx_off", C.c_int32), ("kx_size", C.c_int32), ("ky_off", C.c_int32), ("ky_size", C.c_int32)]


_RESAMPLE_CACHE = {}


def resample_table(in_size, out_size, filt="bicubic"):
    key = (int(in_size), int(out_size), filt)
    if filt not in ("bicubic", "bilinear"):
        raise ValueError(f"unknown resampling filter {filt!r}")
    if key in _RESAMPLE_CACHE:
        return _RESAMPLE_CACHE[key]
    scale = filterscale = float(in_size) / out_size
    if filterscale < 1.0:
        filterscale = 1.0
    support = (2.0 if filt == "bicubic" else 1.0) * filterscale
    ksize = int(np.ceil(support)) * 2 + 1
    tab = np.zeros((out_size, 2 + ksize), dtype=np.int32)
    ss = 1.0 / filterscale
    a = -0.5
    for xx in range(out_size):
        center = (xx + 0.5) * scale
        xmin = max(int(center - support + 0.5), 0)
        xmax = min(int(center + support + 0.5), in_size) - xmin
        x = np.abs((np.arange(xmax) + xmin - center + 0.5) * ss)
        if filt == "bicubic":
            w = np.where(x < 1.0, ((a + 2.0) * x - (a + 3.0)) * x * x + 1, np.where(x < 2.0, (((x - 5) * x + 8) * x - 4) * a, 0.0))
        else:
            w = np.where(x < 1.0, 1.0 - x, 0.0)
        ww = 0.0
        for v in w:
            ww += float(v)
        if ww != 0.0:
            w = w / ww
        tab[xx, 0], tab[xx, 1] = xmin, xmax
        tab[xx, 2:2 + xmax] = [int(-0.5 + float(v) * (1 << 22)) if v < 0 else int(0.5 + float(v) * (1 << 22)) for v in w]
    _RESAMPLE_CACHE[key] = (tab, ksize)
    return tab, ksize


def preprocess_images(images, S, mean=(0.0, 0.0, 0.0), std=(1.0, 1.0, 1.0), device=None, filt="bicubic"):
    if not torch.cuda.is_available():
        raise RuntimeError("pnp_ovss.hip.preprocess_images needs a HIP device (no CPU fallback)")
    lib = load_library()
    dev = torch.device("cuda", torch.cuda.current_device()) if device is None else torch.device(device)
    B = len(images)
    desc = (PnpPreImage * B)()
    coef_parts, coef_off, cache = [], 0, {}
    src_off = tmp_off = 0
    for i, im in enumerate(images):
        H, W = int(im.shape[0]), int(im.shape[1])
        for axis, n in (("x", W), ("y", H)):
            if (n, S) not in cache:
                tab, ks = resample_table(n, S, filt)
                cache[(n, S)] = (coef_off, ks)
                coef_parts.append(tab.reshape(-1))
                coef_off += tab.size
        kx, ky = cache[(W, S)], cache[(H, S)]
        desc[i] = PnpPreImage(src_off, tmp_off, H, W, kx[0], kx[1], ky[0], ky[1])
        src_off += H * W * 3
        tmp_off += H * S * 3
    if all(isinstance(im, torch.Tensor) for im in images):
        rgb = torch.cat([im.reshape(-1) for im in images]) if len(images) > 1 else images[0].reshape(-1)
        assert rgb.is_cuda and rgb.dtype == torch.uint8
    else:
        rgb = torch.from_numpy(np.concatenate([np.ascontiguousarray(im.cpu().numpy() if isinstance(im, torch.Tensor) else im,
                                                                    dtype=np.uint8).reshape(-1) for im in images])).to(dev)
    coef = torch.from_numpy(np.concatenate(coef_parts)).to(dev)
    d_desc = torch.frombuffer(bytearray(bytes(desc)), dtype=torch.uint8).to(dev)
    tmp = torch.empty(tmp_off, dtype=torch.uint8, device=dev)
    out = torch.empty(B, 3, S, S, dtype=torch.float32, device=dev)
    m3 = (C.c_float * 3)(*[float(np.float32(v)) for v in mean])
    s3 = (C.c_float * 3)(*[float(np.float32(v)) for v in std])
    r = lib.pnp_preprocess_images(rgb.data_ptr(), d_desc.data_ptr(), B, S, max(int(im.shape[0]) for im in images), coef.data_ptr(),
                                  tmp.data_ptr(), m3, s3, out.data_ptr(), torch.cuda.current_stream().cuda_stream)
    if r != 0:
        raise RuntimeError(f"pnp_preprocess_images failed ({r})")
    return out


def jpeg_decode_batch(files, device=None):
    if not torch.cuda.is_available():
        raise RuntimeError("pnp_ovss.hip.jpeg_decode_batch needs a HIP device (no CPU fallback)")
    from . import jpeg as J
    lib = load_library()
    dev = torch.device("cuda", torch.cuda.current_device()) if device is None else torch.device(device)
    data, imgs, tabs, segs, sizes, tot = J.pack_batch(files)

    def up(buf):
        return torch.frombuffer(bytearray(bytes(buf)), dtype=torch.uint8).to(dev)
    d_data = torch.from_numpy(data).to(dev)
    d_imgs, d_tabs, d_segs = up(imgs), up(tabs), up(segs)
    d_clean = torch.empty(tot["clean_bytes"], dtype=torch.uint8, device=dev)
    d_bits = torch.empty(len(segs), dtype=torch.int32, device=dev)
    d_coef = torch.empty(tot["coef_elems"], dtype=torch.int16, device=dev)
    d_planes = torch.empty(tot["plane_bytes"], dtype=torch.uint8, device=dev)
    d_rgb = torch.empty(tot["rgb_bytes"], dtype=torch.uint8, device=dev)
    d_err = torch.zeros(1, dtype=torch.int32, device=dev)
    r = lib.pnp_jpeg_decode(d_data.data_ptr(), d_imgs.data_ptr(), d_tabs.data_ptr(), d_segs.data_ptr(), len(files), len(segs),
                            d_clean.data_ptr(), d_bits.data_ptr(), d_coef.data_ptr(), tot["coef_elems"], d_planes.data_ptr(), d_rgb.data_ptr(), tot["max_blocks"],
                            tot["max_pixels"], d_err.data_ptr(), torch.cuda.current_stream().cuda_stream)
    if r != 0:
        raise RuntimeError(f"pnp_jpeg_decode failed ({r})")
    if int(d_err.item()):
        raise RuntimeError("pnp_jpeg_decode: corrupt entropy-coded data")
    out, o = [], 0
    for h, w in sizes:
        out.append(d_rgb[o:o + h * w * 3].view(h, w, 3))
        o += h * w * 3
    return out


def gaussian_taps(H, W, scale=0.05, truncate=4.0):
    sigma = scale * max(H, W)
    radius = int(truncate * float(sigma) + 0.5)
    x = np.arange(-radius, radius + 1)
    phi = np.exp(-0.5 / (sigma * sigma) * x ** 2)
    phi = phi / phi.sum()
    return np.ascontiguousarray(phi[radius:][: radius + 1])


class Engine:

    MODES = {"f32": 0, "bf16": 1, "bf16x3": 2}

    def __init__(self, cfg, max_batch, max_text_len=64, stash_layer=7, bf16=False, device=0, mode=None, share_weights_with=None):
        if not torch.cuda.is_available():
# ... 270 lines not shown
```

Baseline: 215.4.

## Write ViT K/V as per-head contiguous panels from QKV GEMM epilogue

The x3 QKV GEMM gains a new epilogue variant that, besides writing Q, scatters the K and V hi/lo parts into per-(image, head) contiguous 64-wide panels padded to Npad tokens. The attention kernel now streams K/V tiles from these panels with simple contiguous addressing instead of strided rows of the fused QKV buffer with clamping logic. This is meant to make attention's async LDS loads cheaper and better coalesced. In exchange, the vt buffer doubles in size, the GEMM epilogue does extra scattered stores, and the padding rows of the panels are never written by the epilogue, so they hold whatever was there before.

```diff
diff --git a/include/pnp_hip.h b/include/pnp_hip.h
--- a/include/pnp_hip.h
+++ b/include/pnp_hip.h
@@ -162,6 +162,14 @@
                          int32_t n_pad, void* d_ctx, int32_t B, int32_t heads, int32_t N, float scale, void* stream);
 int pnp_op_vit_attention_x3(const void* d_qkv_hi, const void* d_qkv_lo, int32_t ld_qkv, int32_t D, void* d_ctx_hi, void* d_ctx_lo,
                             int32_t B, int32_t heads, int32_t N, float scale, void* stream);
+int pnp_op_vit_attention_x3_panels(const void* d_q_hi, const void* d_q_lo, int32_t ld_q, int32_t D, const void* d_kv,
+                                   int64_t kv_stride, int32_t n_pad, void* d_ctx_hi, void* d_ctx_lo, int32_t B, int32_t heads,
+                                   int32_t N, float scale, void* stream);
+int pnp_op_vit_kv_panels(const void* d_qkv_hi, const void* d_qkv_lo, int32_t ld_qkv, int32_t D, void* d_kv, int64_t kv_stride,
+                         int32_t n_pad, int32_t B, int32_t heads, int32_t N, void* stream);
+int pnp_op_gemm_x3_kv(const void* d_A_hi, const void* d_A_lo, int32_t lda, const void* d_B_hi, const void* d_B_lo, int32_t ldb,
+                      int32_t M, int32_t D, int32_t K, const float* d_bias, void* d_q_hi, void* d_q_lo, int32_t ldq, void* d_kv,
+                      int64_t kv_stride, int32_t tokens, int32_t n_pad, void* stream);
 int pnp_op_layernorm(const float* d_x, const float* d_w, const float* d_b, float eps, int32_t rows, int32_t D,
                      float* d_y, void* stream);
 int pnp_op_xattn(int32_t bf16, int32_t mode, const void* d_nat, int32_t ld_nat, const void* d_tr, int32_t ld_tr,
diff --git a/pnp-ovss_amd/csrc/engine.hip b/pnp-ovss_amd/csrc/engine.hip
--- a/pnp-ovss_amd/csrc/engine.hip
+++ b/pnp-ovss_amd/csrc/engine.hip
@@ -5,6 +5,7 @@
 #include <cstring>
 #include <map>
 #include <memory>
+#include <mutex>
 #include <string>
 #include <vector>
 
@@ -317,8 +318,8 @@
     const size_t M = B * N, R = B * L;
     size_t w = (size_t)c->vit_depth * (12 * D * D) * es + TL * (4 * H * H + 2 * H * D + 2 * H * I) * es * 2 +
                ((size_t)c->vocab + c->max_pos) * H * 4;
-    size_t a = M * (768 + D * 2 + 3 * D + 64 + D + 4 * D) * es + M * D * 12 + D * B * Npad * es + M * TL * H * es * 2 +
-               2 * TL * H * B * Npad * es;
+    size_t a = M * (768 + D * 2 + 3 * D + 64 + D + 4 * D) * es + M * D * 12 + D * B * Npad * es * (c->compute_bf16 == 2 ? 2 : 1) +
+               M * TL * H * es * 2 + 2 * TL * H * B * Npad * es;
     size_t t = TL * (R * (3 * H + 2 * H) * es + R * (H * 8 + I) * 4 + B * (H / 64) * L * (L + Npad) * 4) + R * I * (4 + es) * 2 +
                R * H * 64;
     return w + a + t + (64u << 20);
@@ -415,7 +416,7 @@
     KCHK(e, dalloc_t(e, &e->xn, M * D));
     e->ldq = 3 * (int)D + 64;
     KCHK(e, dalloc_t(e, &e->qk, M * (size_t)e->ldq));
-    KCHK(e, dalloc_t(e, &e->vt, D * ldv, true));
+    KCHK(e, dalloc_t(e, &e->vt, D * ldv * (e->x3 ? 2 : 1), true));
     KCHK(e, dalloc_t(e, &e->ctx, M * D));
     KCHK(e, dalloc_t(e, &e->h1, M * D * c.vit_mlp_ratio));
     KCHK(e, dalloc_t(e, &e->embT, M * D));
@@ -769,6 +770,7 @@
         void* const ctx_lo = (char*)e->ctx + cap * D * 2;
         void* const h1_lo = (char*)e->h1 + cap * F * 2;
         void* const qk_lo = (char*)e->qk + cap * e->ldq * 2;
+        const size_t kv_stride = (size_t)ldv * D;
         for (int l = 0; l < e->c.vit_depth; l++) {
             const VitLayerW& w = e->vit[l];
             const char* const qkv_lo = (const char*)w.qkv_w + (size_t)3 * D * D * 2;
@@ -777,9 +779,10 @@
                 GemmArgs g = G_(e->xn, D, w.qkv_w, D, M, 3 * D, D);
                 g.A_lo = xn_lo; g.B_lo = qkv_lo;
                 g.bias = w.qkv_b; g.out_t = e->qk; g.out_lo = qk_lo; g.ldo_t = e->ldq;
+                g.kv_panels = e->vt; g.kv_stride = kv_stride; g.kv_col0 = D; g.kv_tokens = N; g.kv_npad = e->Npad;
                 KCHK(e, egemm(e, 1, g, s));
             }
-            KCHK(e, vit_attention_x3(e->qk, qk_lo, e->ldq, D, e->ctx, ctx_lo, B, e->c.vit_heads, N, scale, s));
+            KCHK(e, vit_attention_x3(e->qk, qk_lo, e->ldq, D, e->vt, kv_stride, e->Npad, e->ctx, ctx_lo, B, e->c.vit_heads, N, scale, s));
             {
                 GemmArgs g = G_(e->ctx, D, w.proj_w, D, M, D, D);
                 g.A_lo = ctx_lo; g.B_lo = (const char*)w.proj_w + (size_t)D * D * 2;
@@ -1665,6 +1668,18 @@
     return gemm_nt(1, g, (hipStream_t)stream);
 }
 
+extern "C" int pnp_op_gemm_x3_kv(const void* d_A_hi, const void* d_A_lo, int32_t lda, const void* d_B_hi, const void* d_B_lo,
+                                 int32_t ldb, int32_t M, int32_t D, int32_t K, const float* d_bias, void* d_q_hi, void* d_q_lo,
+                                 int32_t ldq, void* d_kv, int64_t kv_stride, int32_t tokens, int32_t n_pad, void* stream) {
+    if (!d_A_hi || !d_A_lo || !d_B_hi || !d_B_lo || !d_q_hi || !d_q_lo || !d_kv || kv_stride <= 0 || tokens <= 0) return PNP_ERR_ARG;
+    GemmArgs g = G_(d_A_hi, lda, d_B_hi, ldb, M, 3 * D, K);
+    g.A_lo = d_A_lo; g.B_lo = d_B_lo;
+    g.bias = d_bias; g.out_t = d_q_hi; g.out_lo = d_q_lo; g.ldo_t = ldq;
+    g.kv_panels = d_kv; g.kv_stride = (size_t)kv_stride; g.kv_col0 = D; g.kv_tokens = tokens; g.kv_npad = n_pad;
+    g.sk = streamk_mode() ? streamk_ws_default() : nullptr;
+    return gemm_nt(1, g, (hipStream_t)stream);
+}
+
 extern "C" int pnp_set_tuning(const char* key, int32_t value) {
     if (!key) return PNP_ERR_ARG;
     if (!strcmp(key, "streamk")) {
@@ -1714,8 +1729,40 @@
 
 extern "C" int pnp_op_vit_attention_x3(const void* d_qkv_hi, const void* d_qkv_lo, int32_t ld_qkv, int32_t D, void* d_ctx_hi,
                                        void* d_ctx_lo, int32_t B, int32_t heads, int32_t N, float scale, void* stream) {
-    if (B <= 0 || heads <= 0 || N <= 0 || ld_qkv < 3 * D) return PNP_ERR_ARG;
-    return vit_attention_x3(d_qkv_hi, d_qkv_lo, ld_qkv, D, d_ctx_hi, d_ctx_lo, B, heads, N, scale, (hipStream_t)stream);
+    if (B <= 0 || heads <= 0 || N <= 0 || ld_qkv < 3 * D || D != heads * 64) return PNP_ERR_ARG;
+    static std::mutex mu;
+    static void* ws[kMaxDevices];
+    static size_t ws_bytes[kMaxDevices];
+    const int dev = current_device();
+    if (dev < 0) return PNP_ERR_HIP;
+    const int Npad = (N + 63) / 64 * 64;
+    const size_t stride = (size_t)B * D * Npad, bytes = 4 * stride * 2;
+    std::lock_guard<std::mutex> lk(mu);
+    if (ws_bytes[dev] < bytes) {
+        if (ws[dev] && hipFree(ws[dev]) != hipSuccess) return PNP_ERR_HIP;
+        ws[dev] = nullptr;
+        ws_bytes[dev] = 0;
+        if (hipMalloc(&ws[dev], bytes) != hipSuccess) return PNP_ERR_NOMEM;
+        ws_bytes[dev] = bytes;
+    }
+    hipStream_t s = (hipStream_t)stream;
+    const int r = vit_kv_panels(d_qkv_hi, d_qkv_lo, ld_qkv, D, ws[dev], stride, Npad, B, heads, N, s);
+    if (r != PNP_OK) return r;
+    return vit_attention_x3(d_qkv_hi, d_qkv_lo, ld_qkv, D, ws[dev], stride, Npad, d_ctx_hi, d_ctx_lo, B, heads, N, scale, s);
+}
+
+extern "C" int pnp_op_vit_kv_panels(const void* d_qkv_hi, const void* d_qkv_lo, int32_t ld_qkv, int32_t D, void* d_kv,
+                                    int64_t kv_stride, int32_t n_pad, int32_t B, int32_t heads, int32_t N, void* stream) {
+    if (B <= 0 || heads <= 0 || N <= 0 || kv_stride <= 0) return PNP_ERR_ARG;
+    return vit_kv_panels(d_qkv_hi, d_qkv_lo, ld_qkv, D, d_kv, (size_t)kv_stride, n_pad, B, heads, N, (hipStream_t)stream);
+}
+
+extern "C" int pnp_op_vit_attention_x3_panels(const void* d_q_hi, const void* d_q_lo, int32_t ld_q, int32_t D, const void* d_kv,
+                                              int64_t kv_stride, int32_t n_pad, void* d_ctx_hi, void* d_ctx_lo, int32_t B,
+                                              int32_t heads, int32_t N, float scale, void* stream) {
+    if (B <= 0 || heads <= 0 || N <= 0 || kv_stride <= 0) return PNP_ERR_ARG;
+    return vit_attention_x3(d_q_hi, d_q_lo, ld_q, D, d_kv, (size_t)kv_stride, n_pad, d_ctx_hi, d_ctx_lo, B, heads, N, scale,
+                            (hipStream_t)stream);
 }
 
 extern "C" int pnp_op_layernorm(const float* d_x, const float* d_w, const float* d_b, float eps, int32_t rows, int32_t D,
diff --git a/pnp-ovss_amd/csrc/gemm.h b/pnp-ovss_amd/csrc/gemm.h
--- a/pnp-ovss_amd/csrc/gemm.h
+++ b/pnp-ovss_amd/csrc/gemm.h
@@ -42,6 +42,9 @@
     int a_f32 = 0;
     int row_div = 0;
     int col_div = 0, col_pad = 0;
+    void* kv_panels = nullptr;
+    size_t kv_stride = 0;
+    int kv_col0 = 0, kv_tokens = 0, kv_npad = 0;
     struct GemmProfile* prof = nullptr;
     StreamKWs* sk = nullptr;
     float* sk_part = nullptr;
diff --git a/pnp-ovss_amd/csrc/gemm.hip b/pnp-ovss_amd/csrc/gemm.hip
--- a/pnp-ovss_amd/csrc/gemm.hip
+++ b/pnp-ovss_amd/csrc/gemm.hip
@@ -647,6 +647,14 @@
         if (g.col_div || g.bias_on_rows || (g.Nvalid & 3)) return -1;
         if (g.mode == GEMM_EPI_LINEAR && g.resid && g.out_f32 && !g.out_t) return WIDE_RESID_F32;
         if (g.mode == GEMM_EPI_LINEAR && !g.resid && g.out_f32 && !g.out_t) return WIDE_BIAS_F32;
+        if (g.kv_panels) {
+            const bool ok = g.mode == GEMM_EPI_LINEAR && !g.resid && g.out_t && g.out_lo && !g.out_f32 && g.kv_col0 > 0 &&
+                            g.kv_col0 % 64 == 0 && g.Nvalid == 3 * g.kv_col0 && g.kv_tokens >= 4 && g.kv_npad % 64 == 0 &&
+                            g.kv_npad >= g.kv_tokens && g.M % g.kv_tokens == 0 &&
+                            (size_t)(g.M / g.kv_tokens) * g.kv_npad * g.kv_col0 <= g.kv_stride &&
+                            (size_t)(g.M / g.kv_tokens + 1) * g.kv_npad * g.kv_col0 < (1ull << 31);
+            return ok ? WIDE_SPLIT_KV : -1;
+        }
         if (g.mode == GEMM_EPI_GELU && !g.resid && g.out_t && g.out_lo && !g.out_f32) return WIDE_GELU_SPLIT;
         if (g.mode == GEMM_EPI_LINEAR && !g.resid && g.out_t && g.out_lo && !g.out_f32) return WIDE_SPLIT;
         return -1;
diff --git a/pnp-ovss_amd/csrc/gemm_wide.h b/pnp-ovss_amd/csrc/gemm_wide.h
--- a/pnp-ovss_amd/csrc/gemm_wide.h
+++ b/pnp-ovss_amd/csrc/gemm_wide.h
@@ -31,7 +31,7 @@
 #define PNP_WAIT_VM(n) asm volatile("s_waitcnt vmcnt(%0)" ::"n"(n) : "memory")
 
 enum { WIDE_BF16 = 0, WIDE_GELU_BF16 = 1, WIDE_RESID_F32 = 2, WIDE_TOKCOLS_BF16 = 3, WIDE_BIAS_F32 = 4, WIDE_TOKCOLS_F32 = 5,
-       WIDE_GELU_SPLIT = 6, WIDE_SPLIT = 7 };
+       WIDE_GELU_SPLIT = 6, WIDE_SPLIT = 7, WIDE_SPLIT_KV = 8 };
 constexpr int kWideStageRow = 68;
 constexpr int kWideStageBytes = 8 * 32 * kWideStageRow * 4;
 constexpr int kWideSmem = 65536 + kWideStageBytes;
diff --git a/pnp-ovss_amd/csrc/gemm_x3.hip b/pnp-ovss_amd/csrc/gemm_x3.hip
--- a/pnp-ovss_amd/csrc/gemm_x3.hip
+++ b/pnp-ovss_amd/csrc/gemm_x3.hip
@@ -43,7 +43,8 @@
     constexpr int BM = 256, BN = 256, SLOT = 65536, ARR = 16384;
     constexpr int JM = 8, IN = 4;
     constexpr int NDMA = 8;
-    constexpr int kDrain = (EPI == WIDE_GELU_SPLIT || EPI == WIDE_SPLIT) ? 32 : 24;
+    constexpr bool kSplit = EPI == WIDE_GELU_SPLIT || EPI == WIDE_SPLIT || EPI == WIDE_SPLIT_KV;
+    constexpr int kDrain = kSplit ? 32 : 24;
     constexpr int SROW = kWideStageRow;
     extern __shared__ __attribute__((aligned(16))) char smem[];
 
@@ -361,7 +362,7 @@
         f32x4 bv = {0.f, 0.f, 0.f, 0.f};
         f32x4 rv[8];
         f32x4 bacc[IN];
-        if constexpr (EPI == WIDE_GELU_SPLIT || EPI == WIDE_SPLIT) {
+        if constexpr (kSplit) {
 #pragma unroll
             for (int i = 0; i < IN; i++) {
                 const int nn = en0 + wn * 64 + i * 16 + q * 4;
@@ -430,10 +431,30 @@
                     }
                 }
             }
-        } else if constexpr (EPI == WIDE_GELU_SPLIT || EPI == WIDE_SPLIT) {
+        } else if constexpr (kSplit) {
             constexpr int HROW = 68;
             bf16* const stgh = reinterpret_cast<bf16*>(smem + SLOT) + wave * (64 * HROW);
             const bool full = (em0 + BM <= g.M) && (en0 + BN <= g.Nvalid);
+            const int ns = en0 + wn * 64;
+            const bool kvs = EPI == WIDE_SPLIT_KV && ns >= g.kv_col0 && ns < g.Nvalid;
+            bf16* kvb[2] = {nullptr, nullptr};
+            int kv_m0 = 0, kv_t0[2] = {0, 0};
+            uint32_t kv_o0[2] = {0u, 0u}, kv_jump = 0u;
+            if (EPI == WIDE_SPLIT_KV && kvs) {
+                const int c = ns - g.kv_col0, op = c >= g.kv_col0, h = (c - op * g.kv_col0) >> 6;
+                bf16* const pb = reinterpret_cast<bf16*>(g.kv_panels) + (size_t)h * g.kv_npad * 64 + (lane & 15) * 4;
+                kvb[0] = pb + (size_t)op * g.kv_stride;
+                kvb[1] = pb + (size_t)(op + 2) * g.kv_stride;
+                const uint32_t img = (uint32_t)g.kv_npad * (uint32_t)g.kv_col0;
+                kv_jump = 256u + img - 64u * (uint32_t)g.kv_tokens;
+                kv_m0 = em0 + wm * 128 + (lane >> 4);
+#pragma unroll
+                for (int hf = 0; hf < 2; hf++) {
+                    const int m = kv_m0 + hf * 64, b = m / g.kv_tokens;
+                    kv_t0[hf] = m - b * g.kv_tokens;
+                    kv_o0[hf] = (uint32_t)b * img + 64u * (uint32_t)kv_t0[hf];
+                }
+            }
 #pragma unroll
             for (int half = 0; half < 2; half++) {
 #pragma unroll
@@ -470,6 +491,20 @@
 #pragma unroll
                     for (int it = 0; it < 16; it++)
                         sv[it] = *reinterpret_cast<const bf16x4*>(stgh + (it * 4 + (lane >> 4)) * HROW + (lane & 15) * 4);
+                    if (EPI == WIDE_SPLIT_KV && kvs) {
+                        int m = kv_m0 + half * 64, t = kv_t0[half];
+                        uint32_t o = kv_o0[half];
+#pragma unroll
+                        for (int it = 0; it < 16; it++) {
+                            if (full || m < g.M) PNP_EPI_STORE(reinterpret_cast<bf16x4*>(kvb[part] + o), sv[it]);
+                            m += 4;
+                            t += 4;
+                            const bool wrap = t >= g.kv_tokens;
+                            t = wrap ? t - g.kv_tokens : t;
+                            o += wrap ? kv_jump : 256u;
+                        }
+                        continue;
+                    }
 #pragma unroll
                     for (int it = 0; it < 16; it++) {
                         const int m = em0 + wm * 128 + half * 64 + it * 4 + (lane >> 4);
@@ -636,6 +671,7 @@
         case WIDE_BIAS_F32: return launch_x3<WIDE_BIAS_F32>(g, s);
         case WIDE_GELU_SPLIT: return launch_x3<WIDE_GELU_SPLIT>(g, s);
         case WIDE_SPLIT: return launch_x3<WIDE_SPLIT>(g, s);
+        case WIDE_SPLIT_KV: return launch_x3<WIDE_SPLIT_KV>(g, s);
         case WIDE_TOKCOLS_F32: return launch_x3<WIDE_TOKCOLS_F32>(g, s);
     }
     return PNP_ERR_ARG;
diff --git a/pnp-ovss_amd/csrc/kernels.h b/pnp-ovss_amd/csrc/kernels.h
--- a/pnp-ovss_amd/csrc/kernels.h
+++ b/pnp-ovss_amd/csrc/kernels.h
@@ -54,8 +54,10 @@
 int vit_attention(int bf, const void* qk, int ld_qk, int D, const void* vt, int ld_vt, int Npad, void* ctx, int B,
                   int H, int N, float scale, hipStream_t s, void* ctx_lo = nullptr);
 
-int vit_attention_x3(const void* qkv_hi, const void* qkv_lo, int ld_qk, int D, void* ctx_hi, void* ctx_lo, int B, int H, int N,
-                     float scale, hipStream_t s);
+int vit_attention_x3(const void* q_hi, const void* q_lo, int ld_q, int D, const void* kv, size_t kv_stride, int Npad, void* ctx_hi,
+                     void* ctx_lo, int B, int H, int N, float scale, hipStream_t s);
+int vit_kv_panels(const void* qkv_hi, const void* qkv_lo, int ld, int D, void* kv, size_t kv_stride, int Npad, int B, int H, int N,
+                  hipStream_t s);
 
 int text_embed(const int64_t* ids, int ld_ids, const float* word, const float* pos, float* out, int B, int L, int H,
                int enc_id, int vocab, hipStream_t s);
diff --git a/pnp-ovss_amd/csrc/vit_kernels.hip b/pnp-ovss_amd/csrc/vit_kernels.hip
--- a/pnp-ovss_amd/csrc/vit_kernels.hip
+++ b/pnp-ovss_amd/csrc/vit_kernels.hip
@@ -396,7 +396,7 @@
 #endif
 
 __global__ __launch_bounds__(768) void vit_attn32_x3_kernel(const bf16* __restrict__ qk, const bf16* __restrict__ qk_lo, int ld_qk, int D,
-                                                            const bf16* __restrict__ vt, const bf16* __restrict__ vt_lo, int ld_vt,
+                                                            const bf16* __restrict__ kv, size_t kv_stride, int Npad,
                                                             bf16* __restrict__ ctx, bf16* __restrict__ ctx_lo, int N, float scale, int nqw) {
     constexpr int ROWB = 128, TILE = 64 * ROWB;
     __shared__ __attribute__((aligned(16))) char ring[2][4 * TILE];
@@ -420,29 +420,20 @@
             fql[ks] = *reinterpret_cast<const bf16x8*>(qk_lo + off + ks * 16);
         }
     }
-    const size_t koff = (row0 * ld_qk + D + h * 64) * 2, voff = (row0 * ld_vt + h * 64) * 2;
-    const uint64_t k0 = reinterpret_cast<uint64_t>(qk) + koff;
-    const uint64_t d_klo = reinterpret_cast<uint64_t>(qk_lo) + koff - k0;
-    const uint64_t d_v = reinterpret_cast<uint64_t>(vt) + voff - k0;
-    const uint64_t d_vlo = reinterpret_cast<uint64_t>(vt_lo) + voff - k0;
+    const uint64_t k0 = reinterpret_cast<uint64_t>(kv) + ((size_t)b * gridDim.y + h) * (size_t)Npad * ROWB;
+    const uint64_t opb = (uint64_t)kv_stride * 2;
     const int prow = lane >> 3, pc = lane & 7;
-    const uint32_t sc_even = (uint32_t)(pc ^ ((prow >> 1) & 7)) << 4, sc_odd = (uint32_t)(pc ^ ((4 + (prow >> 1)) & 7)) << 4;
+    const uint32_t loff_even = prow * ROWB + ((uint32_t)(pc ^ ((prow >> 1) & 7)) << 4);
+    const uint32_t loff_odd = prow * ROWB + ((uint32_t)(pc ^ ((4 + (prow >> 1)) & 7)) << 4);
     auto issue_tile = [&](int t) {
         for (int p = wave; p < 32; p += nwaves) {
-            const uint64_t m_v = 0ull - (uint64_t)((p >> 3) & 1), m_lo = 0ull - (uint64_t)(p >> 4);
-            const uint64_t d = (m_v & m_lo & d_vlo) | (m_v & ~m_lo & d_v) | (~m_v & m_lo & d_klo);
-            const uint32_t ld2 = ((uint32_t)ld_qk + ((uint32_t)m_v & (uint32_t)(ld_vt - ld_qk))) * 2u;
             int rs = t * 64 + (p & 7) * 8;
 #ifdef PNP_DEV
             if (g_attn_ablate) rs = (p & 7) * 8;
 #endif
-            rs = rs < N - 1 ? rs : N - 1;
-            const char* const sbase = reinterpret_cast<const char*>(k0 + d + (uint64_t)((uint32_t)rs * ld2));
-            int lr = rs + prow;
-            lr = (lr < N ? lr : N - 1) - rs;
-            const uint32_t loff = (uint32_t)lr * ld2 + ((p & 1) ? sc_odd : sc_even);
+            const uint64_t sb = k0 + (uint64_t)(p >> 3) * opb + (uint32_t)rs * (uint32_t)ROWB;
+            const uint32_t loff = (p & 1) ? loff_odd : loff_even;
             const uint32_t lds = (uint32_t)(uintptr_t)(__attribute__((address_space(3))) char*)(ring[t & 1] + p * 1024);
-            const uint64_t sb = reinterpret_cast<uint64_t>(sbase);
             const uint64_t sbu = ((uint64_t)(uint32_t)__builtin_amdgcn_readfirstlane((int)(sb >> 32)) << 32) |
                                  (uint32_t)__builtin_amdgcn_readfirstlane((int)(uint32_t)sb);
             asm volatile("s_mov_b32 m0, %2\n\ts_nop 0\n\tglobal_load_lds_dwordx4 %0, %1" ::"v"(loff), "s"(sbu),
@@ -594,18 +585,50 @@
     return hipGetLastError() == hipSuccess ? PNP_OK : PNP_ERR_HIP;
 }
 
-int vit_attention_x3(const void* qkv_hi, const void* qkv_lo, int ld_qk, int D, void* ctx_hi, void* ctx_lo, int B, int H, int N,
-                     float scale, hipStream_t s) {
-    if (D != H * 64 || !qkv_hi || !qkv_lo || !ctx_hi || !ctx_lo) return PNP_ERR_ARG;
+__global__ void kv_panels_kernel(const bf16* __restrict__ qkv_hi, const bf16* __restrict__ qkv_lo, int ld, int D,
+                                 bf16* __restrict__ kv, size_t kv_stride, int Npad, int B, int H, int N) {
+    const size_t per_op = (size_t)B * H * Npad * 8;
+    const size_t idx = (size_t)blockIdx.x * blockDim.x + threadIdx.x;
+    if (idx >= 4 * per_op) return;
+    const int op = (int)(idx / per_op);
+    size_t rem = idx - op * per_op;
+    const int ch = (int)(rem & 7);
+    rem >>= 3;
+    const int t = (int)(rem % Npad);
+    rem /= Npad;
+    const int h = (int)(rem % H), b = (int)(rem / H);
+    bf16x8 v = {};
+    if (t < N) {
+        const bf16* src = (op & 2) ? qkv_lo : qkv_hi;
+        v = *reinterpret_cast<const bf16x8*>(src + ((size_t)b * N + t) * ld + (1 + (op & 1)) * D + h * 64 + ch * 8);
+    }
+    *reinterpret_cast<bf16x8*>(kv + op * kv_stride + (((size_t)b * H + h) * Npad + t) * 64 + ch * 8) = v;
+}
+
+int vit_kv_panels(const void* qkv_hi, const void* qkv_lo, int ld, int D, void* kv, size_t kv_stride, int Npad, int B, int H, int N,
+                  hipStream_t s) {
+    if (D != H * 64 || Npad % 64 || Npad < N || N <= 0 || B <= 0 || ld % 8 || ld < 3 * D || !qkv_hi || !qkv_lo || !kv ||
+        kv_stride < (size_t)B * H * Npad * 64 || kv_stride % 8)
+        return PNP_ERR_ARG;
+    const size_t total = (size_t)4 * B * H * Npad * 8;
+    hipLaunchKernelGGL(kv_panels_kernel, dim3((unsigned)((total + 255) / 256)), dim3(256), 0, s, (const bf16*)qkv_hi,
+                       (const bf16*)qkv_lo, ld, D, (bf16*)kv, kv_stride, Npad, B, H, N);
+    return hipGetLastError() == hipSuccess ? PNP_OK : PNP_ERR_HIP;
+}
+
+int vit_attention_x3(const void* q_hi, const void* q_lo, int ld_q, int D, const void* kv, size_t kv_stride, int Npad, void* ctx_hi,
+                     void* ctx_lo, int B, int H, int N, float scale, hipStream_t s) {
+    if (D != H * 64 || !q_hi || !q_lo || !kv || !ctx_hi || !ctx_lo || N <= 0 || B <= 0 || Npad % 64 || Npad < N || ld_q % 8 ||
+        ld_q < D || kv_stride < (size_t)B * H * Npad * 64 || kv_stride % 8)
+        return PNP_ERR_ARG;
     const int nqw = (N + 31) / 32;
     int max_wpb = nqw > 24 ? 12 : 8;
 #ifdef PNP_DEV
     if (getenv("PNP_ATTN_WPB")) max_wpb = atoi(getenv("PNP_ATTN_WPB"));
 #endif
     const int nblk = (nqw + max_wpb - 1) / max_wpb, wpb = (nqw + nblk - 1) / nblk;
-    const bf16 *qh = (const bf16*)qkv_hi, *ql = (const bf16*)qkv_lo;
-    hipLaunchKernelGGL(vit_attn32_x3_kernel, dim3(nblk, H, B), dim3(wpb * 64), 0, s, qh, ql, ld_qk, D, qh + 2 * D, ql + 2 * D, ld_qk,
-                       (bf16*)ctx_hi, (bf16*)ctx_lo, N, scale, nqw);
+    hipLaunchKernelGGL(vit_attn32_x3_kernel, dim3(nblk, H, B), dim3(wpb * 64), 0, s, (const bf16*)q_hi, (const bf16*)q_lo, ld_q, D,
+                       (const bf16*)kv, kv_stride, Npad, (bf16*)ctx_hi, (bf16*)ctx_lo, N, scale, nqw);
     return hipGetLastError() == hipSuccess ? PNP_OK : PNP_ERR_HIP;
 }
 
diff --git a/pnp-ovss_amd/pnp_ovss/hip.py b/pnp-ovss_amd/pnp_ovss/hip.py
--- a/pnp-ovss_amd/pnp_ovss/hip.py
+++ b/pnp-ovss_amd/pnp_ovss/hip.py
@@ -78,6 +78,9 @@
         "pnp_op_gemm_tokcols": (i32, [i32, vp, i32, vp, i32, i32, i32, i32, vp, vp, i32, i32, i32, vp]),
         "pnp_op_vit_attention": (i32, [i32, vp, i32, i32, vp, i32, i32, vp, i32, i32, i32, f32, vp]),
         "pnp_op_vit_attention_x3": (i32, [vp, vp, i32, i32, vp, vp, i32, i32, i32, f32, vp]),
+        "pnp_op_vit_attention_x3_panels": (i32, [vp, vp, i32, i32, vp, i64, i32, vp, vp, i32, i32, i32, f32, vp]),
+        "pnp_op_vit_kv_panels": (i32, [vp, vp, i32, i32, vp, i64, i32, i32, i32, i32, vp]),
+        "pnp_op_gemm_x3_kv": (i32, [vp, vp, i32, vp, vp, i32, i32, i32, i32, vp, vp, vp, i32, vp, i64, i32, i32, vp]),
         "pnp_preprocess_images": (i32, [vp, vp, i32, i32, i32, vp, vp, C.POINTER(C.c_float), C.POINTER(C.c_float), vp, vp]),
         "pnp_op_layernorm": (i32, [vp, vp, vp, f32, i32, i32, vp, vp]),
         "pnp_op_cast": (i32, [i32, vp, vp, i64, vp]),
@@ -108,7 +111,7 @@
             "pnp_cross_kv", "pnp_profile_read_stage", "pnp_op_split", "pnp_op_gemm_x3", "pnp_op_gemm_x3a",
             "pnp_xattn_grad_layer", "pnp_compute_gradcam_layer", "pnp_drop_loop_layer", "pnp_allocated_bytes",
             "pnp_op_vit_attention_x3", "pnp_jpeg_decode", "pnp_op_sort_pairs", "pnp_op_scan_i32", "pnp_set_tuning",
-            "pnp_streamk_status"]
+            "pnp_streamk_status", "pnp_op_vit_attention_x3_panels", "pnp_op_vit_kv_panels", "pnp_op_gemm_x3_kv"]
 
 
 class _DevView:
```

Result: no change. 216.1 (median of 6 runs) (+0.3%).
